# ChainBreak/denoising_diffusion_deep_fake

Measured on AMD Instinct MI355X. Metric: training images/sec (256x256 U-Net, bs=16/GPU), higher is better.
Workload: dtype f32; 1 GPU; d3f train_denoiser step: noise blend -> Unet(resnet34) fwd -> (MSE+1-SSIM)/2 -> bwd -> Adam, 256x256 synthetic face crops, bs=16/GPU, random-init weights, train-mode BatchNorm; image_size=256, batch_per_gpu=16, global_batch=16, parallelism=dp1, graph_step=False, adam_overlap_tail=False, adam_overlap_tail_steps=0, ranks_seen=1, csrc_digest=56899a78a27ce7a0

## Files before the change

denoising_diffusion_deep_fake_amd/_lib.py:

```python
import ctypes as C
import os
import re
from pathlib import Path

_HERE = Path(__file__).resolve().parent
LIB_PATH = Path(os.environ["D3F_LIB"]) if os.environ.get("D3F_LIB") else _HERE / "csrc" / "libd3f_hip.so"
HEADER_PATH = _HERE.parent / "include" / "d3f_hip.h"

F32, BF16, F32X3 = 0, 1, 2


class D3FError(RuntimeError):
    pass


class ConvDesc(C.Structure):
    _fields_ = [(n, C.c_int32) for n in
                ("B", "H", "W", "C0", "C1", "upsample0", "Cout", "KH", "KW", "stride", "pad", "CinReal")]


class BnDesc(C.Structure):
    _fields_ = [("dtype", C.c_int32), ("C", C.c_int32), ("Cpad", C.c_int32), ("rows", C.c_int64),
                ("apply", C.c_int32), ("relu", C.c_int32), ("res", C.c_int32), ("mask", C.c_int32),
                ("fwd_rows", C.c_int32), ("fused_rows", C.c_int32), ("allow_fused", C.c_int32), ("plan_nets", C.c_int32)]


class BnPlan(C.Structure):
    _fields_ = [("fwd_fused", C.c_int32), ("bwd_fused", C.c_int32), ("reduce_blocks", C.c_int32), ("bwd_rows", C.c_int32),
                ("rows_per_block", C.c_int64), ("stat_floats", C.c_uint64), ("part_floats", C.c_uint64)]


BN_COEF_ROWS = 7

_p, _i, _i64, _f, _sz, _dbl = C.c_void_p, C.c_int, C.c_int64, C.c_float, C.c_size_t, C.c_double
_u64, _u32p = C.c_uint64, C.POINTER(C.c_uint32)
_desc = C.POINTER(ConvDesc)
_bnd, _bnp = C.POINTER(BnDesc), C.POINTER(BnPlan)

PROTOTYPES = {
    "d3f_version": (_i, []),
    "d3f_last_error": (C.c_char_p, []),
    "d3f_source_digest": (C.c_char_p, []),
    "d3f_profile_enable": (_i, [_i]),
    "d3f_profile_classes": (_i, [_i]),
    "d3f_profile_collect": (_i, [C.POINTER(C.c_double), C.POINTER(C.c_int64), C.POINTER(C.c_double)]),
    "d3f_unet_create": (_i, [C.c_char_p, _i, _i, _i, _i, _i, _i, C.POINTER(_p)]),
    "d3f_unet_destroy": (_i, [_p]),
    "d3f_unet_create_nets": (_i, [C.c_char_p, _i, _i, _i, _i, _i, _i, _i, _i, C.POINTER(_p)]),
    "d3f_unet_nets": (_i, [_p]),
    "d3f_unet_net_workspace_stride": (_sz, [_p]),
    "d3f_unet_pair_pack_weights": (_i, [_p, C.POINTER(_p), _p, _p]),
    "d3f_unet_pair_forward": (_i, [_p, C.POINTER(_p), C.POINTER(_p), C.POINTER(_p), C.POINTER(_p), _p, _p]),
    "d3f_unet_pair_backward": (_i, [_p, C.POINTER(_p), C.POINTER(_p), C.POINTER(_p), _p, _i, _i, _i, _p]),
    "d3f_unet_num_params": (_i, [_p]),
    "d3f_unet_param_info": (_i, [_p, _i, C.c_char_p, _i, C.POINTER(C.c_int32), C.POINTER(_i), C.POINTER(_i64)]),
    "d3f_unet_param_floats": (_i64, [_p]),
    "d3f_unet_num_bn": (_i, [_p]),
    "d3f_unet_bn_info": (_i, [_p, _i, C.c_char_p, _i, C.POINTER(_i), C.POINTER(_i64), C.POINTER(_i64)]),
    "d3f_unet_bnstat_floats": (_i64, [_p]),
    "d3f_unet_workspace_bytes": (_sz, [_p]),
    "d3f_unet_forward_flops": (_dbl, [_p]),
    "d3f_unet_backward_flops": (_dbl, [_p]),
    "d3f_unet_pack_weights": (_i, [_p, _p, _p, _p]),
    "d3f_unet_forward": (_i, [_p, _p, _p, _p, _p, _p, _i, _p]),
    "d3f_unet_forward_graph": (_i, [_p, _p, _p, _p, _p, _p, _p]),
    "d3f_noise_blend_fixed": (_i, [_p, _p, _p, _p, _i, _i64, _p]),
    "d3f_l1_per_image_workspace_bytes": (_sz, [_i]),
    "d3f_l1_per_image": (_i, [_p, _p, _p, _p, _i, _i64, _p]),
    "d3f_affine_warp": (_i, [_p, _p, _p, _i, _i, _i, _i, _p]),
    "d3f_u8rgb_normalise": (_i, [_p, _p, _i, _i, _i, C.POINTER(_f), C.POINTER(_f), _p]),
    "d3f_unet_predict_u8": (_i, [_p, _p, _p, _p, _p, C.POINTER(_f), C.POINTER(_f), _p, _i, _p]),
    "d3f_unet_predict_frames_u8": (_i, [_p, _p, _p, _p, _i, _i, _i, _i, _i, _i, _p, C.POINTER(_f), C.POINTER(_f), _p, _i, _p]),
    "d3f_crop_resize_cubic_u8": (_i, [_p, _i, _i, _i, _i, _i, _i, _i, _p, _i, _i, _i64, _p]),
    "d3f_unet_num_segments": (_i, [_p]),
    "d3f_unet_plan_counts": (_i, [_p, C.POINTER(C.c_int32), C.POINTER(C.c_int32), C.POINTER(C.c_int32)]),
    "d3f_unet_segment_range": (_i, [_p, _i, C.POINTER(_i64), C.POINTER(_i64)]),
    "d3f_unet_backward": (_i, [_p, _p, _p, _p, _p, _i, _i, _p]),
    "d3f_unet_backward_nojoin": (_i, [_p, _p, _p, _p, _p, _i, _i, _p]),
    "d3f_unet_side_stream": (_i, [_p, C.POINTER(_p)]),
    "d3f_unet_backward_join": (_i, [_p, _p]),
    "d3f_adam_coefficients": (_i, [_f, _f, _f, _f, _i, _f, C.POINTER(_f)]),
    "d3f_unet_train_step": (_i, [_p, _p, _f, _f, _f, _p, _i, _p]),
    "d3f_unet_set_bn_sync": (_i, [_p, _p, _p, _i]),
    "d3f_unet_export": (_i, [_p, C.c_char_p, _p, _p, _p]),
    "d3f_unet_export_shape": (_i, [_p, C.c_char_p, C.POINTER(C.c_int32)]),
    "d3f_conv_upsample_folded": (_i, [_i, _p]),
    "d3f_conv_upsample_summed": (_i, [_i, _p]),
    "d3f_conv_packed_bytes": (_sz, [_i, _desc, _i]),
    "d3f_conv_pack_weights": (_i, [_i, _desc, _p, _p, _p, _p]),
    "d3f_conv_workspace_bytes": (_sz, [_i, _desc, _i]),
    "d3f_conv_stats_floats": (_sz, [_i, _desc, _i, C.POINTER(_i)]),
    "d3f_conv_forward": (_i, [_i, _desc, _p, _p, _p, _p, _p, _p, _p]),
    "d3f_conv_winograd_applies": (_i, [_i, _desc]),
    "d3f_conv_winograd_filter_bytes": (_sz, [_desc]),
    "d3f_conv_winograd_stats_floats": (_sz, [_desc, C.POINTER(_i)]),
    "d3f_conv_winograd_pack": (_i, [_desc, _p, _p, _p]),
    "d3f_conv_winograd_forward": (_i, [_desc, _p, _p, _p, _p, _p, _p, _p, _i, _p]),
    "d3f_conv_backward_data": (_i, [_i, _desc, _p, _p, _p, _p, _i, _i, _p, _p]),
    "d3f_conv_backward_weight_workspace_bytes": (_sz, [_i, _desc]),
    "d3f_conv_backward_weight": (_i, [_i, _desc, _p, _p, _p, _p, _p, _p]),
    "d3f_bn_finalize": (_i, [_p, _i, _i, _i64, _p, _p, _p, _p, _p, _p]),
    "d3f_bn_apply": (_i, [_i, _p, _p, _i, _i64, _p, _i, _p, _p]),
    "d3f_bn_backward_workspace_bytes": (_sz, [_i, _i, _i64]),
    "d3f_bn_backward": (_i, [_i, _p, _p, _p, _p, _p, _i, _i64, _p, _p, _p, _p, _p, _p]),
    "d3f_bn_layer_plan": (_i, [_bnd, _bnp]),
    "d3f_bn_layer_forward": (_i, [_bnd, _p, _p, _p, _p, _p, _p, _p, _p, _p, _p, _p]),
    "d3f_bn_layer_backward": (_i, [_bnd, _p, _p, _p, _p, _p, _p, _p, _p, _i, _p, _p, _p]),
    "d3f_unet_bn_layer": (_i, [_p, _i, _bnd, _bnp]),
    "d3f_maxpool3x3s2_forward": (_i, [_i, _p, _p, _p, _i, _i, _i, _i, _p]),
    "d3f_maxpool3x3s2_backward": (_i, [_i, _p, _p, _p, _i, _i, _i, _i, _i, _p]),
    "d3f_upsample2x_backward": (_i, [_i, _p, _p, _i, _i, _i, _i, _p]),
    "d3f_nchw_to_nhwc": (_i, [_i, _p, _p, _i, _i, _i, _i, _i, _p]),
    "d3f_nhwc_to_nchw": (_i, [_i, _p, _p, _i, _i, _i, _i, _i, _p]),
    "d3f_noise_blend": (_i, [_p, _p, _p, _f, _p, _p, _i, _i64, _p]),
    "d3f_mse_ssim_loss_workspace_bytes": (_sz, [_i, _i, _i]),
    "d3f_mse_ssim_loss": (_i, [_p, _p, _f, _f, _p, _p, _p, _i, _i, _i, _p]),
    "d3f_adam_step": (_i, [_p, _p, _p, _p, _i64, _f, _f, _f, _f, _i, _f, _p]),
    "d3f_ema_lerp": (_i, [_p, _p, _i64, _f, _p]),
    "d3f_philox4x32_10": (_i, [_u32p, _u32p, _u32p]),
    "d3f_noise_blend_rng": (_i, [_p, _u64, _u64, _f, _p, _p, _i, _i64, _p]),
    "d3f_noise_blend_fixed_rng": (_i, [_p, _u64, _u64, _p, _p, _i, _i64, _p]),
    "d3f_noise_draw": (_i, [_u64, _u64, _p, _p, _i, _i64, _p]),
    "d3f_affine_warp_rng": (_i, [_p, _p, _u64, _u64, _i, C.POINTER(_f), _i, _i, _i, _i, _p]),
    "d3f_affine_theta_draw": (_i, [_u64, _u64, _i, C.POINTER(_f), _p, _p, _i, _i, _i, _p]),
}

ALLREDUCE_FN = C.CFUNCTYPE(C.c_int, C.c_void_p, C.c_void_p, C.c_int64, C.c_void_p)

_lib = None


def header_symbols():
    text = HEADER_PATH.read_text()
    text = re.sub(r"/\*.*?\*/", "", text, flags=re.S)
    return sorted(set(re.findall(r"\b(d3f_[a-z0-9_]+)\s*\(", text)))


def sources_present():
    return HEADER_PATH.exists() and any((_HERE / "csrc").glob("*.hip"))


def source_digest():
    import hashlib
    h = hashlib.sha256()
    files = sorted((_HERE / "csrc").glob("*.hip")) + sorted((_HERE / "csrc").glob("*.h")) + [HEADER_PATH]
    for f in files:
        h.update(f.name.encode())
        h.update(f.read_bytes())
    return h.hexdigest()[:16]


def lib():
    global _lib
    if _lib is not None:
        return _lib
    if not LIB_PATH.exists():
        raise D3FError(
            f"{LIB_PATH} is missing: build it with `python -c 'import __graft_entry__ as g; g.build()'` "
            f"or `make -C {LIB_PATH.parent}` (hipcc, gfx950). There is no CPU fallback.")
    handle = C.CDLL(str(LIB_PATH))
    for name, (res, args) in PROTOTYPES.items():
        if os.environ.get("D3F_LIB") and not hasattr(handle, name):
            continue
        fn = getattr(handle, name)
        fn.restype = res
        fn.argtypes = args
    if not os.environ.get("D3F_LIB") and sources_present():
        built, here = handle.d3f_source_digest().decode(), source_digest()
        if built != here:
            raise D3FError(
                f"{LIB_PATH} was built from other sources (digest {built}) than the ones next to it ({here}): "
                f"rebuild it with `make -C {LIB_PATH.parent}`, or name a variant build explicitly through D3F_LIB")
    _lib = handle
    return _lib


def built_digest():
    handle = lib()
    return handle.d3f_source_digest().decode() if hasattr(handle, "d3f_source_digest") else None


def check(rc):
    if rc != 0:
        raise D3FError(lib().d3f_last_error().decode("utf-8", "replace"))


def stream_ptr():
    import torch
    return C.c_void_p(torch.cuda.current_stream().cuda_stream)


def ptr(t):
    if t is None:
        return None
    return C.c_void_p(t.data_ptr())


def ptr2(a, b):
    return (C.c_void_p * 2)(a.data_ptr(), b.data_ptr())
```

denoising_diffusion_deep_fake_amd/csrc/batchnorm.hip:

```cpp
#include "common.h"
#include "pointwise.h"
#include "vec16.h"

#include <algorithm>
#include <type_traits>

namespace d3f {

constexpr float BN_EPS = 1e-5f, BN_MOMENTUM = 0.1f;

constexpr int BNF_SC = 32;
constexpr int BNF_MAX_ROWS = 1024;
#ifndef BNF_FWD_U_F32
#define BNF_FWD_U_F32 4
#endif
#ifndef BNF_BWD_U
#define BNF_BWD_U 2
#endif

__device__ __forceinline__ float2 bn_fwd_coef(double s1, double s2, double count, int c, const float* __restrict__ gamma,
                                              const float* __restrict__ beta, float eps, float momentum, bool store,
                                              float* __restrict__ running_mean, float* __restrict__ running_var,
                                              float* __restrict__ mean_o, float* __restrict__ invstd_o,
                                              float* __restrict__ scale_o, float* __restrict__ shift_o) {
// ... 317 lines not shown
    const float4 v0 = *reinterpret_cast<const float4*>(base + (long)r * ld * 2);
    const float4 v1 = *reinterpret_cast<const float4*>(base + (long)(r + 16) * ld * 2);
    const float4 v2 = *reinterpret_cast<const float4*>(base + (long)(r + 32) * ld * 2);
    const float4 v3 = *reinterpret_cast<const float4*>(base + (long)(r + 48) * ld * 2);
    if (!hooked) { behind_first_loads(); hooked = true; }
    a0 += (double)v0.x; a1 += (double)v0.y; a2 += (double)v0.z; a3 += (double)v0.w;
    a0 += (double)v1.x; a1 += (double)v1.y; a2 += (double)v1.z; a3 += (double)v1.w;
    a0 += (double)v2.x; a1 += (double)v2.y; a2 += (double)v2.z; a3 += (double)v2.w;
    a0 += (double)v3.x; a1 += (double)v3.y; a2 += (double)v3.z; a3 += (double)v3.w;
  }
  if (!hooked) behind_first_loads();
  for (; r < rows; r += 16) {
    const float4 v = *reinterpret_cast<const float4*>(base + (long)r * ld * 2);
    a0 += (double)v.x; a1 += (double)v.y; a2 += (double)v.z; a3 += (double)v.w;
  }
  red[rl][q * 4 + 0] = a0;
  red[rl][q * 4 + 1] = a1;
  red[rl][q * 4 + 2] = a2;
  red[rl][q * 4 + 3] = a3;
  __syncthreads();
  if (tid < 64) {
    double s = 0.0;
#pragma unroll
    for (int k = 0; k < 16; ++k) s += red[k][tid];
    tot[tid] = s;
  }
  __syncthreads();
}

template <typename T, bool HAS2>
__global__ __launch_bounds__(256) void bn_finalize_apply_kernel(
    const float* __restrict__ stats, int stat_rows, int C, int Cpad, double count,
    const float* __restrict__ gamma, const float* __restrict__ beta, float eps, float momentum,
    float* __restrict__ running_mean, float* __restrict__ running_var, float* __restrict__ mean_o,
    float* __restrict__ invstd_o, float* __restrict__ scale_o, float* __restrict__ shift_o,
    const T* __restrict__ y, const T* __restrict__ res, const T* __restrict__ yr,
    const float* __restrict__ scale_r, const float* __restrict__ shift_r, int relu, T* __restrict__ out,
    long rows, long rows_per_block, NetSplit ns) {
  chain_priority();
  if (blockIdx.z != 0) {
    net_shift(stats, ns.ws); net_shift(gamma, ns.par); net_shift(beta, ns.par);
    net_shift(running_mean, ns.bn); net_shift(running_var, ns.bn);
    net_shift(mean_o, ns.ws); net_shift(invstd_o, ns.ws); net_shift(scale_o, ns.ws); net_shift(shift_o, ns.ws);
    net_shift(y, ns.ws); net_shift(res, ns.ws); net_shift(yr, ns.ws); net_shift(scale_r, ns.ws); net_shift(shift_r, ns.ws);
    net_shift(out, ns.ws);
  }
  __shared__ double red[16][64];
  __shared__ double tot[64];
  __shared__ float cf[2][BNF_SC];
  typedef typename Raw4<T>::type raw_t;
  constexpr int U = sizeof(T) == 4 ? BNF_FWD_U_F32 : 8;
  const int tid = threadIdx.x, c0 = blockIdx.y * BNF_SC;
  const int v = tid & 7, rr = tid >> 3, cc = c0 + v * 4;
  const long r0 = (long)blockIdx.x * rows_per_block;
  long r1 = r0 + rows_per_block;
  if (r1 > rows) r1 = rows;
  const T* __restrict__ second = res != nullptr ? res : yr;
  raw_t a[U], b[U], an[U], bn[U];
  auto load = [&](raw_t (&ya)[U], raw_t (&yb)[U], long r) {
#pragma unroll
    for (int u = 0; u < U; ++u) {
      const long row = r + 32 * u < r1 ? r + 32 * u : r1 - 1;
      ya[u] = ldraw(y + row * C + cc);
      if (HAS2) yb[u] = ldraw(second + row * C + cc);
    }
  };
  slab_reduce(stats, stat_rows, Cpad, c0, red, tot, [&]() { load(a, b, r0 + rr); });
  if (tid < BNF_SC) {
    const float2 f = bn_fwd_coef(tot[2 * tid], tot[2 * tid + 1], count, c0 + tid, gamma, beta, eps, momentum,
                                 blockIdx.x == 0, running_mean, running_var, mean_o, invstd_o, scale_o, shift_o);
    cf[0][tid] = f.x;
    cf[1][tid] = f.y;
  }
  __syncthreads();
  float sc[4], sf[4], scr[4] = {0.f, 0.f, 0.f, 0.f}, sfr[4] = {0.f, 0.f, 0.f, 0.f};
#pragma unroll
  for (int k = 0; k < 4; ++k) {
    sc[k] = cf[0][v * 4 + k];
    sf[k] = cf[1][v * 4 + k];
    if (HAS2 && res == nullptr) {
      scr[k] = scale_r[cc + k];
      sfr[k] = shift_r[cc + k];
    }
  }
  for (long r = r0 + rr; r < r1; r += 32 * U) {
    if (r + 32 * U < r1) load(an, bn, r + 32 * U);
#pragma unroll
    for (int u = 0; u < U; ++u) {
      const long row = r + 32 * u;
      if (row >= r1) continue;
      const float4 ya = cvt4(a[u]);
      float x[4] = {ya.x, ya.y, ya.z, ya.w};
#pragma unroll
      for (int k = 0; k < 4; ++k) x[k] = x[k] * sc[k] + sf[k];
      if (HAS2) {
        const float4 yb = cvt4(b[u]);
        if (res != nullptr) {
          x[0] += yb.x; x[1] += yb.y; x[2] += yb.z; x[3] += yb.w;
        } else {
          const float t[4] = {yb.x, yb.y, yb.z, yb.w};
#pragma unroll
          for (int k = 0; k < 4; ++k) x[k] += t[k] * scr[k] + sfr[k];
        }
      }
      if (relu) {
#pragma unroll
        for (int k = 0; k < 4; ++k) x[k] = fmaxf(x[k], 0.f);
      }
      st4<T>(out + row * C + cc, make_float4(x[0], x[1], x[2], x[3]));
    }
#pragma unroll
    for (int u = 0; u < U; ++u) {
      a[u] = an[u];
      if (HAS2) b[u] = bn[u];
    }
  }
}

static long rows_per_block_for(long rows, int slabs, int dtype, int plan_nets) {
  const long wgs = (dtype == D3F_F32 ? 256 : 512) / plan_nets_for(plan_nets, 64);
  long rb = std::max(1L, wgs / slabs);
  long rpb = (rows + rb - 1) / rb;
  rpb = (rpb + 31) / 32 * 32;
  return std::max(32L, rpb);
}

struct BnResidualOps {
  const void *res = nullptr, *yr = nullptr;
  const float *scale_r = nullptr, *shift_r = nullptr;
};
static BnResidualOps residual_ops(const BnLayer& L, const BnBufs& b) {
  if (L.res == BN_RES_TENSOR) return {b.res, nullptr, nullptr, nullptr};
  if (L.res == BN_RES_LAYER) return {nullptr, b.res, bn_coef(b.res_coef, L.C, BN_SCALE), bn_coef(b.res_coef, L.C, BN_SHIFT)};
  return {};
}

static int bn_finalize_apply_launch(const BnLayer& L, const BnBufs& b, hipStream_t stream, const NetSplit* ns) {
  if (L.rows == 0) return 0;
  const NetSplit nv = net_split_or_single(ns);
  const dim3 grid((unsigned)((L.rows + L.rows_per_block - 1) / L.rows_per_block), (unsigned)(L.C / BNF_SC),
                  (unsigned)nv.nets);
  const BnResidualOps r = residual_ops(L, b);
  by_dtype(L.dtype, [&](auto* typed) {
    typedef std::remove_pointer_t<decltype(typed)> T;
    auto go = [&](auto kernel) {
      hipLaunchKernelGGL(kernel, grid, dim3(256), 0, stream, b.stats, L.fwd_rows, L.C, L.Cpad, (double)L.rows, b.gamma,
                         b.beta, BN_EPS, BN_MOMENTUM, b.running_mean, b.running_var, bn_coef(b.coef, L.C, BN_MEAN),
                         bn_coef(b.coef, L.C, BN_INVSTD), bn_coef(b.coef, L.C, BN_SCALE), bn_coef(b.coef, L.C, BN_SHIFT),
                         (const T*)b.y, (const T*)r.res, (const T*)r.yr, r.scale_r, r.shift_r, L.relu ? 1 : 0, (T*)b.a,
                         L.rows, L.rows_per_block, nv);
    };
    if (L.res != BN_RES_NONE) go(bn_finalize_apply_kernel<T, true>);
    else go(bn_finalize_apply_kernel<T, false>);
  });
  D3F_HIP(hipGetLastError());
  return 0;
}

template <typename T, bool FROM_A, bool RD_DRES>
__global__ __launch_bounds__(256) void bn_bwd_finalize_apply_kernel(
    const float* __restrict__ partial, int nblocks, int C, double count, const float* __restrict__ gamma,
    const float* __restrict__ mean, const float* __restrict__ invstd, float* __restrict__ dgamma,
    float* __restrict__ dbeta, float* __restrict__ coef, const T* __restrict__ dA,
    const T* __restrict__ a, const T* __restrict__ y, T* __restrict__ dy, T* __restrict__ dres,
    long rows, long rows_per_block, const float* __restrict__ mask_scale,
    const float* __restrict__ mask_shift, NetSplit ns) {
  chain_priority();
  if (blockIdx.z != 0) {
    net_shift(partial, ns.ws); net_shift(gamma, ns.par); net_shift(mean, ns.ws); net_shift(invstd, ns.ws);
    net_shift(dgamma, ns.grad); net_shift(dbeta, ns.grad); net_shift(coef, ns.ws);
    net_shift(dA, ns.ws); net_shift(a, ns.ws); net_shift(y, ns.ws); net_shift(dy, ns.ws); net_shift(dres, ns.ws);
    net_shift(mask_scale, ns.ws); net_shift(mask_shift, ns.ws);
  }
  __shared__ double red[16][64];
  __shared__ double tot[64];
  __shared__ float cf[3][BNF_SC];
  typedef typename Raw4<T>::type raw_t;
  constexpr int U = BNF_BWD_U;
  const int tid = threadIdx.x, c0 = blockIdx.y * BNF_SC;
  const int v = tid & 7, rr = tid >> 3, cc = c0 + v * 4;
  const long r0 = (long)blockIdx.x * rows_per_block;
  long r1 = r0 + rows_per_block;
  if (r1 > rows) r1 = rows;
  raw_t g4[U], y4[U], a4[U], d4[U], g4n[U], y4n[U], a4n[U], d4n[U];
  auto load = [&](raw_t (&gg)[U], raw_t (&yy)[U], raw_t (&aa)[U], raw_t (&dd)[U], long r) {
#pragma unroll
    for (int u = 0; u < U; ++u) {
      const long row = r + 32 * u < r1 ? r + 32 * u : r1 - 1;
      gg[u] = ldraw(dA + row * C + cc);
      yy[u] = ldraw(y + row * C + cc);
      if (FROM_A) aa[u] = ldraw(a + row * C + cc);
      if (RD_DRES) dd[u] = ldraw(dres + row * C + cc);
    }
  };
  slab_reduce(partial, nblocks, C, c0, red, tot, [&]() { load(g4, y4, a4, d4, r0 + rr); });
  if (tid < BNF_SC) {
    const float3 k = bn_bwd_coef(tot[2 * tid], tot[2 * tid + 1], count, c0 + tid, C, gamma, invstd, blockIdx.x == 0,
                                 dgamma, dbeta, coef);
    cf[0][tid] = k.x;
    cf[1][tid] = k.y;
    cf[2][tid] = k.z;
  }
  __syncthreads();
  float k0[4], k1[4], k2[4], mu[4], is[4], msc[4] = {0.f, 0.f, 0.f, 0.f}, msf[4] = {0.f, 0.f, 0.f, 0.f};
#pragma unroll
  for (int k = 0; k < 4; ++k) {
    k0[k] = cf[0][v * 4 + k];
    k1[k] = cf[1][v * 4 + k];
    k2[k] = cf[2][v * 4 + k];
    mu[k] = mean[cc + k];
    is[k] = invstd[cc + k];
    if (!FROM_A && mask_scale != nullptr) {
      msc[k] = mask_scale[cc + k];
      msf[k] = mask_shift[cc + k];
    }
  }
  for (long r = r0 + rr; r < r1; r += 32 * U) {
    if (r + 32 * U < r1) load(g4n, y4n, a4n, d4n, r + 32 * U);
#pragma unroll
    for (int u = 0; u < U; ++u) {
      const long row = r + 32 * u;
      if (row >= r1) continue;
      const float4 gv = cvt4(g4[u]), yv = cvt4(y4[u]);
      float g[4] = {gv.x, gv.y, gv.z, gv.w};
      const float yy[4] = {yv.x, yv.y, yv.z, yv.w};
      if (FROM_A) {
        const float4 av = cvt4(a4[u]);
        const float aa[4] = {av.x, av.y, av.z, av.w};
#pragma unroll
        for (int k = 0; k < 4; ++k) g[k] = aa[k] > 0.f ? g[k] : 0.f;
      } else if (mask_scale != nullptr) {
#pragma unroll
        for (int k = 0; k < 4; ++k) g[k] = (yy[k] * msc[k] + msf[k]) > 0.f ? g[k] : 0.f;
      }
      float o[4];
#pragma unroll
      for (int k = 0; k < 4; ++k) {
        const float xhat = (yy[k] - mu[k]) * is[k];
        o[k] = k0[k] * (g[k] - k1[k] - xhat * k2[k]);
      }
      st4<T>(dy + row * C + cc, make_float4(o[0], o[1], o[2], o[3]));
      if (dres != nullptr) {
        if (RD_DRES) {
          const float4 dv = cvt4(d4[u]);
          g[0] += dv.x; g[1] += dv.y; g[2] += dv.z; g[3] += dv.w;
        }
        st4<T>(dres + row * C + cc, make_float4(g[0], g[1], g[2], g[3]));
      }
    }
#pragma unroll
    for (int u = 0; u < U; ++u) {
      g4[u] = g4n[u];
      y4[u] = y4n[u];
      if (FROM_A) a4[u] = a4n[u];
      if (RD_DRES) d4[u] = d4n[u];
    }
  }
}

struct BnBwdOps {
  const float *mean, *invstd;
  float* k;
  const void* a;
  const float *mask_scale, *mask_shift;
};
static BnBwdOps bwd_ops(const BnLayer& L, const BnBufs& b) {
  const bool from_y = L.mask == BN_MASK_FROM_Y;
  return {bn_coef(b.coef, L.C, BN_MEAN), bn_coef(b.coef, L.C, BN_INVSTD), b.k != nullptr ? b.k : bn_coef(b.coef, L.C, BN_K),
          L.mask == BN_MASK_FROM_A ? b.a : nullptr, from_y ? bn_coef(b.coef, L.C, BN_SCALE) : nullptr,
          from_y ? bn_coef(b.coef, L.C, BN_SHIFT) : nullptr};
}

static int bn_bwd_finalize_apply_launch(const BnLayer& L, const BnBufs& b, const BnBwdOps& o, hipStream_t stream,
                                        const NetSplit* ns) {
  if (L.rows == 0) return 0;
  const NetSplit nv = net_split_or_single(ns);
  const dim3 grid((unsigned)((L.rows + L.rows_per_block - 1) / L.rows_per_block), (unsigned)(L.C / BNF_SC),
                  (unsigned)nv.nets);
  const bool from_a = o.mask_scale == nullptr && o.a != nullptr;
  const bool rd_dres = b.dres != nullptr && b.dres_acc;
  by_dtype(L.dtype, [&](auto* typed) {
    typedef std::remove_pointer_t<decltype(typed)> T;
    auto go = [&](auto kernel) {
      hipLaunchKernelGGL(kernel, grid, dim3(256), 0, stream, b.stats, L.bwd_rows, L.C, (double)L.rows, b.gamma, o.mean,
                         o.invstd, b.dgamma, b.dbeta, o.k, (const T*)b.dA, (const T*)o.a, (const T*)b.y, (T*)b.dy,
                         (T*)b.dres, L.rows, L.rows_per_block, o.mask_scale, o.mask_shift, nv);
    };
    if (from_a && rd_dres) go(bn_bwd_finalize_apply_kernel<T, true, true>);
    else if (from_a) go(bn_bwd_finalize_apply_kernel<T, true, false>);
    else if (rd_dres) go(bn_bwd_finalize_apply_kernel<T, false, true>);
    else go(bn_bwd_finalize_apply_kernel<T, false, false>);
  });
  D3F_HIP(hipGetLastError());
  return 0;
}

void bn_layer_plan(BnLayer& L) {
  static const bool no_fused = getenv("D3F_NO_BN_FUSED_FINALIZE") != nullptr;
  auto fused_ok = [&](int rows) {
    return L.allow_fused && !no_fused && (L.dtype == D3F_F32 || L.dtype == D3F_BF16) && L.C % BNF_SC == 0 && rows >= 1 &&
           rows <= BNF_MAX_ROWS;
  };
  const long min_rows = std::max(16L, 4L * (256 / std::max(1, std::min(256, L.C / (L.dtype == D3F_F32 ? 4 : 8)))));
  L.reduce_blocks = (int)std::clamp((L.rows + min_rows - 1) / min_rows, 1L, 1024L);
  L.bwd_rows = L.fused_rows > 0 ? L.fused_rows : L.reduce_blocks;
  L.fwd_fused = L.apply && fused_ok(L.fwd_rows);
  L.bwd_fused = fused_ok(L.bwd_rows);
  L.rows_per_block = L.fwd_fused || L.bwd_fused ? rows_per_block_for(L.rows, L.C / BNF_SC, L.dtype, L.plan_nets) : 0;
  L.stat_floats = (size_t)L.fwd_rows * L.Cpad * 2;
  L.part_floats = (size_t)std::max(L.reduce_blocks, L.fused_rows) * L.C * 2;
}

int bn_layer_finalize(const BnLayer& L, const BnBufs& b, long count, hipStream_t stream, const NetSplit* ns) {
  const NetSplit nv = net_split_or_single(ns);
  hipLaunchKernelGGL(bn_finalize_kernel, dim3(L.C, 1, nv.nets), dim3(256), 0, stream, b.stats, L.fwd_rows, L.C, L.Cpad,
                     (double)count, b.gamma, b.beta, BN_EPS, BN_MOMENTUM, b.running_mean, b.running_var,
                     bn_coef(b.coef, L.C, BN_MEAN), bn_coef(b.coef, L.C, BN_INVSTD), bn_coef(b.coef, L.C, BN_SCALE),
                     bn_coef(b.coef, L.C, BN_SHIFT), nv);
  D3F_HIP(hipGetLastError());
  return 0;
}

int bn_layer_apply(const BnLayer& L, const BnBufs& b, hipStream_t stream, const NetSplit* ns) {
  const int ve = L.dtype == D3F_F32 ? 4 : 8;
  D3F_CHECK(L.C % ve == 0 && (256 * ve) % L.C == 0, "bn_apply: C=%d must divide %d", L.C, 256 * ve);
  const long nvec = L.rows * L.C / ve;
  if (nvec == 0) return 0;
  const NetSplit nv = net_split_or_single(ns);
  const BnResidualOps r = residual_ops(L, b);
  by_dtype(L.dtype, [&](auto* typed) {
    typedef std::remove_pointer_t<decltype(typed)> T;
    hipLaunchKernelGGL(bn_apply_kernel<T>, dim3(grid_for(nvec), 1, nv.nets), dim3(256), 0, stream, (const T*)b.y,
                       bn_coef(b.coef, L.C, BN_SCALE), bn_coef(b.coef, L.C, BN_SHIFT), (const T*)r.res, (const T*)r.yr,
                       r.scale_r, r.shift_r, L.relu ? 1 : 0, (T*)b.a, nvec, L.C, nv.ws);
  });
  D3F_HIP(hipGetLastError());
  return 0;
}

int bn_layer_forward(const BnLayer& L, const BnBufs& b, const BnSync* sync, hipStream_t stream, const NetSplit* ns) {
  long count = L.rows;
  if (sync != nullptr) {
    if (int rc = sync->fn(sync->ctx, b.stats, (int64_t)L.fwd_rows * L.Cpad * 2, (void*)stream))
      return set_error(rc, "BatchNorm statistics all-reduce failed in the forward pass (%s)", L.name.c_str());
    count *= sync->world;
  } else if (L.fwd_fused) {
    return bn_finalize_apply_launch(L, b, stream, ns);
  }
  if (int rc = bn_layer_finalize(L, b, count, stream, ns)) return rc;
  return L.apply ? bn_layer_apply(L, b, stream, ns) : 0;
}

int bn_layer_backward(const BnLayer& L, const BnBufs& b, const BnSync* sync, hipStream_t stream, const NetSplit* ns) {
  const int C = L.C, ve = L.dtype == D3F_F32 ? 4 : 8, vc = C / ve;
  const NetSplit nv = net_split_or_single(ns);
  const BnBwdOps o = bwd_ops(L, b);
  if (L.fused_rows == 0) {
    D3F_CHECK(C % ve == 0 && vc >= 1 && vc <= 256 && (256 % vc) == 0, "bn_bwd_reduce: unsupported channel count %d", C);
    by_dtype(L.dtype, [&](auto* typed) {
      typedef std::remove_pointer_t<decltype(typed)> T;
      hipLaunchKernelGGL(bn_bwd_reduce_kernel<T>, dim3(L.reduce_blocks, 1, nv.nets), dim3(256), 0, stream,
                         (const T*)b.dA, (const T*)o.a, (const T*)b.y, o.mean, o.invstd, b.stats, L.rows, C, o.mask_scale,
                         o.mask_shift, nv.ws);
    });
    D3F_HIP(hipGetLastError());
  }
  auto finalize = [&](long count, float* dgamma, float* dbeta) -> int {
    hipLaunchKernelGGL(bn_bwd_finalize_kernel, dim3(C, 1, nv.nets), dim3(256), 0, stream, b.stats, L.bwd_rows, C,
                       (double)count, b.gamma, o.invstd, dgamma, dbeta, o.k, nv);
    D3F_HIP(hipGetLastError());
    return 0;
  };
  if (sync != nullptr) {
    if (int rc = finalize(L.rows, b.dgamma, b.dbeta)) return rc;
    if (int rc = sync->fn(sync->ctx, b.stats, (int64_t)L.bwd_rows * C * 2, (void*)stream))
      return set_error(rc, "BatchNorm statistics all-reduce failed in the backward pass (%s)", L.name.c_str());
    if (int rc = finalize(L.rows * sync->world, nullptr, nullptr)) return rc;
  } else if (L.bwd_fused) {
    return bn_bwd_finalize_apply_launch(L, b, o, stream, ns);
  } else if (int rc = finalize(L.rows, b.dgamma, b.dbeta)) {
    return rc;
  }
  D3F_CHECK(C % ve == 0 && (256 * ve) % C == 0, "bn_bwd_apply: C=%d must divide %d", C, 256 * ve);
  const long nvec = L.rows * C / ve;
  if (nvec == 0) return 0;
  by_dtype(L.dtype, [&](auto* typed) {
    typedef std::remove_pointer_t<decltype(typed)> T;
    hipLaunchKernelGGL(bn_bwd_apply_kernel<T>, dim3(grid_for(nvec), 1, nv.nets), dim3(256), 0, stream, (const T*)b.dA,
                       (const T*)o.a, (const T*)b.y, o.mean, o.invstd, o.k, (T*)b.dy, (T*)b.dres, b.dres_acc, nvec, C,
                       o.mask_scale, o.mask_shift, nv.ws);
  });
  D3F_HIP(hipGetLastError());
  return 0;
}

}
```

denoising_diffusion_deep_fake_amd/csrc/c_api.hip:

```cpp
#include "../../include/d3f_hip.h"

#include <cstdarg>
#include <cstdio>
#include <cstring>
#include <new>
#include <vector>

#include "engine.h"
#include "philox.h"

namespace d3f {
static thread_local char g_err[1024] = "";
int set_error(int code, const char* fmt, ...) {
  va_list ap;
  va_start(ap, fmt);
  vsnprintf(g_err, sizeof(g_err), fmt, ap);
  va_end(ap);
  return code;
}
}

namespace d3f {
struct ProfRec {
  hipEvent_t a, b;
// ... 368 lines not shown
  if (int rc = plan(L, D3F_F32, d, PLAN_FWD)) return rc;
  D3F_CHECK(L.wu != 0,
            "conv_winograd: needs 3x3 / stride 1 / pad 1, one source, H and W multiples of 16, channels a multiple of 16, "
            "filters a multiple of 64 (got %dx%d k%d s%d p%d C0=%d C1=%d up=%d Cout=%d)",
            d->H, d->W, d->KH, d->stride, d->pad, d->C0, d->C1, d->upsample0, d->Cout);
  return 0;
}
int d3f_conv_winograd_applies(int dtype, const d3f_conv_desc* d) {
  ConvLayer L;
  return (d != nullptr && plan(L, dtype, d, PLAN_FWD) == 0 && L.wino) ? 1 : 0;
}
size_t d3f_conv_winograd_filter_bytes(const d3f_conv_desc* d) {
  ConvLayer L;
  return (d == nullptr || plan(L, D3F_F32, d, PLAN_FWD) != 0) ? 0 : L.wu;
}
size_t d3f_conv_winograd_stats_floats(const d3f_conv_desc* d, int* tiles) {
  ConvLayer L;
  if (d == nullptr || plan(L, D3F_F32, d, PLAN_FWD) != 0 || L.wu == 0) return 0;
  if (tiles) *tiles = L.wino_rows;
  return (size_t)L.wino_rows * L.CoutPad * 2;
}
int d3f_conv_winograd_pack(const d3f_conv_desc* d, const float* w, void* u, void* stream) {
  ConvLayer L;
  if (int rc = wino_plan(L, d)) return rc;
  D3F_CHECK(w && u && d->CinReal == d->C0, "conv_winograd_pack: null argument or padded input channels");
  return conv_winograd_pack_launch(w, reinterpret_cast<float*>(u), d->Cout, d->C0, (hipStream_t)stream);
}
int d3f_conv_winograd_forward(const d3f_conv_desc* d, const void* src0, const void* u, void* y, float* stats,
                              const float* scale, const float* shift, const void* residual, int relu, void* stream) {
  ConvLayer L;
  if (int rc = wino_plan(L, d)) return rc;
  if (d->B == 0) return 0;
  D3F_CHECK(src0 && u && y && ((scale == nullptr) == (shift == nullptr)), "conv_winograd_forward: null argument");
  D3F_CHECK(scale != nullptr || (residual == nullptr && relu == 0),
            "conv_winograd_forward: residual / ReLU belong to the eval epilogue (scale and shift)");
  ConvFwdBufs b;
  b.src0 = src0; b.w = u; b.out = y;
  if (scale != nullptr) {
    b.scale = scale; b.shift = shift; b.res = residual; b.relu = relu ? 1 : 0;
  } else {
    b.stats = stats;
  }
  return conv_layer_forward(L, b, true, (hipStream_t)stream);
}
int d3f_conv_backward_data(int dtype, const d3f_conv_desc* d, const void* dy, const void* w_dgrad,
                           void* dx0, void* dx1, int acc0, int acc1, void* workspace, void* stream) {
  ConvLayer L;
  const int sum2 = d != nullptr && d->upsample0 == 2 ? PLAN_SUM2 : 0;
  if (int rc = plan(L, dtype, d, PLAN_DGRAD | sum2 | (workspace ? PLAN_SPLITK : 0))) return rc;
  if (d->B == 0) return 0;
  D3F_CHECK(dy && w_dgrad && dx0 && (d->C1 == 0 || dx1), "conv_backward_data: null argument");
  ConvDgradBufs b;
  b.dy = dy; b.w = w_dgrad; b.dx0 = dx0; b.dx1 = dx1; b.acc0 = acc0; b.acc1 = acc1;
  b.w_skip = L.upfold ? reinterpret_cast<const char*>(w_dgrad) + L.wd4 : nullptr;
  b.slabs = reinterpret_cast<float*>(workspace);
  return conv_layer_dgrad(L, b, (hipStream_t)stream);
}
size_t d3f_conv_backward_weight_workspace_bytes(int dtype, const d3f_conv_desc* d) {
  ConvLayer L;
  return plan(L, dtype, d, PLAN_WGRAD) != 0 ? 0 : L.wslab_bytes;
}
int d3f_conv_backward_weight(int dtype, const d3f_conv_desc* d, const void* dy, const void* src0,
                             const void* src1, void* workspace, float* dw, void* stream) {
  ConvLayer L;
  if (int rc = plan(L, dtype, d, PLAN_WGRAD)) return rc;
  if (d->B == 0) {
    D3F_CHECK(dw, "conv_backward_weight: null argument");
    D3F_HIP(hipMemsetAsync(dw, 0, (size_t)d->Cout * d->CinReal * d->KH * d->KW * sizeof(float), (hipStream_t)stream));
    return 0;
  }
  D3F_CHECK(dy && src0 && workspace && dw && (d->C1 == 0 || src1), "conv_backward_weight: null argument");
  return wgrad_layer_launch(L.wl, dy, src0, src1, reinterpret_cast<float*>(workspace), dw, d->Cout, d->CinReal, dtype,
                            (hipStream_t)stream);
}

static BnLayer bn_layer(int dtype, int C, int64_t rows, int fwd_rows = 0) {
  BnLayer L;
  L.C = C; L.Cpad = (int)round_up(C, 16); L.rows = (long)rows; L.dtype = sdt(dtype); L.fwd_rows = fwd_rows;
  L.allow_fused = false;
  bn_layer_plan(L);
  return L;
}
int d3f_bn_finalize(const float* stats, int tiles, int C, int64_t count, const float* gamma,
                    const float* beta, float* running_mean, float* running_var, float* coef, void* stream) {
  D3F_CHECK(stats && gamma && beta && coef && C > 0 && tiles > 0 && count > 0, "bn_finalize: argument");
  const BnLayer L = bn_layer(D3F_F32, C, count, tiles);
  BnBufs b;
  b.stats = const_cast<float*>(stats);
  b.gamma = gamma; b.beta = beta; b.running_mean = running_mean; b.running_var = running_var; b.coef = coef;
  return bn_layer_finalize(L, b, (long)count, (hipStream_t)stream);
}
int d3f_bn_apply(int dtype, const void* y, const float* coef, int C, int64_t rows, const void* residual,
                 int relu, void* out, void* stream) {
  D3F_CHECK(y && coef && out, "bn_apply: null argument");
  BnLayer L = bn_layer(dtype, C, rows);
  L.relu = relu != 0;
  L.res = residual ? BN_RES_TENSOR : BN_RES_NONE;
  BnBufs b;
  b.coef = const_cast<float*>(coef);
  b.y = y; b.res = residual; b.a = out;
  return bn_layer_apply(L, b, (hipStream_t)stream);
}
size_t d3f_bn_backward_workspace_bytes(int dtype, int C, int64_t rows) {
  return ((size_t)bn_layer(dtype, C, rows).reduce_blocks * C * 2 + 3 * (size_t)C) * sizeof(float) + 256;
}
int d3f_bn_backward(int dtype, const void* dA, const void* a_or_null, const void* y, const float* coef,
                    const float* gamma, int C, int64_t rows, void* dy, void* dres, float* dgamma,
                    float* dbeta, void* workspace, void* stream) {
  D3F_CHECK(dA && y && coef && gamma && dy && dgamma && dbeta && workspace, "bn_backward: null argument");
  BnLayer L = bn_layer(dtype, C, rows);
  L.mask = a_or_null ? BN_MASK_FROM_A : BN_MASK_NONE;
  BnBufs b;
  b.stats = reinterpret_cast<float*>(workspace);
  b.k = b.stats + (size_t)round_up((long)L.reduce_blocks * C * 2, 4);
  b.coef = const_cast<float*>(coef);
  b.gamma = gamma; b.y = y; b.a = const_cast<void*>(a_or_null);
  b.dA = dA; b.dy = dy; b.dres = dres; b.dgamma = dgamma; b.dbeta = dbeta;
  return bn_layer_backward(L, b, nullptr, (hipStream_t)stream);
}

static_assert(D3F_BN_COEF_ROWS == BN_COEF_ROWS, "d3f_hip.h states the coefficient block's rows");
static int bn_plan(BnLayer& L, const d3f_bn_desc* d) {
  D3F_CHECK(d != nullptr, "bn_layer: null descriptor");
  D3F_CHECK(d->dtype == D3F_F32 || d->dtype == D3F_BF16 || d->dtype == D3F_F32X3, "bn_layer: dtype %d", d->dtype);
  D3F_CHECK(d->C > 0 && d->Cpad >= d->C && d->rows >= 0, "bn_layer: C=%d Cpad=%d rows=%lld", d->C, d->Cpad,
            (long long)d->rows);
  D3F_CHECK(d->res >= BN_RES_NONE && d->res <= BN_RES_LAYER && d->mask >= BN_MASK_NONE && d->mask <= BN_MASK_FROM_A,
            "bn_layer: res=%d mask=%d", d->res, d->mask);
  D3F_CHECK(d->fwd_rows >= 0 && d->fused_rows >= 0, "bn_layer: fwd_rows=%d fused_rows=%d", d->fwd_rows, d->fused_rows);
  D3F_CHECK(d->plan_nets == 1 || d->plan_nets == 2, "bn_layer: plan_nets=%d", d->plan_nets);
  L.name = "bn_layer";
  L.C = d->C; L.Cpad = d->Cpad; L.rows = (long)d->rows; L.dtype = sdt(d->dtype); L.plan_nets = d->plan_nets;
  L.apply = d->apply != 0; L.relu = d->relu != 0;
  L.res = (BnResidual)d->res; L.mask = (BnMask)d->mask;
  L.fwd_rows = d->fwd_rows; L.fused_rows = d->fused_rows; L.allow_fused = d->allow_fused != 0;
  bn_layer_plan(L);
  return 0;
}
static void bn_plan_out(const BnLayer& L, d3f_bn_plan* p) {
  p->fwd_fused = L.fwd_fused; p->bwd_fused = L.bwd_fused; p->reduce_blocks = L.reduce_blocks; p->bwd_rows = L.bwd_rows;
  p->rows_per_block = L.rows_per_block; p->stat_floats = L.stat_floats; p->part_floats = L.part_floats;
}
static bool bn_split_channels_ok(const BnLayer& L) {
  const int ve = L.dtype == D3F_F32 ? 4 : 8;
  return L.C % ve == 0 && (256 * ve) % L.C == 0;
}
int d3f_bn_layer_plan(const d3f_bn_desc* d, d3f_bn_plan* plan) {
  D3F_CHECK(plan != nullptr, "bn_layer_plan: null argument");
  BnLayer L;
  if (int rc = bn_plan(L, d)) return rc;
  bn_plan_out(L, plan);
  return 0;
}
int d3f_bn_layer_forward(const d3f_bn_desc* d, float* stats, const float* gamma, const float* beta, float* running_mean,
                         float* running_var, float* coef, const void* y, const void* res, const float* res_coef, void* a,
                         void* stream) {
  BnLayer L;
  if (int rc = bn_plan(L, d)) return rc;
  if (L.rows == 0) return 0;
  D3F_CHECK(L.fwd_rows >= 1, "bn_layer_forward: the forward pass reads fwd_rows >= 1 partial rows (fwd_rows=%d)", L.fwd_rows);
  D3F_CHECK(stats && gamma && beta && coef && y, "bn_layer_forward: null argument");
  D3F_CHECK((running_mean == nullptr) == (running_var == nullptr), "bn_layer_forward: one running statistic without the other");
  if (L.apply) {
    D3F_CHECK(a != nullptr, "bn_layer_forward: apply needs the output tensor");
    D3F_CHECK(L.res == BN_RES_NONE || res != nullptr, "bn_layer_forward: res=%d needs the residual tensor", (int)L.res);
    D3F_CHECK(L.res != BN_RES_LAYER || res_coef != nullptr, "bn_layer_forward: res=2 needs res_coef, the other layer's coefficient block");
  }
  if (L.fwd_fused)
    D3F_CHECK(L.Cpad % 2 == 0, "bn_layer_forward: the fused form needs an even Cpad (Cpad=%d)", L.Cpad);
  else if (L.apply)
    D3F_CHECK(bn_split_channels_ok(L), "bn_layer_forward: the split form needs C to divide %d (C=%d)",
              256 * (L.dtype == D3F_F32 ? 4 : 8), L.C);
  BnBufs b;
  b.stats = stats; b.gamma = gamma; b.beta = beta; b.running_mean = running_mean; b.running_var = running_var;
  b.coef = coef; b.y = y; b.a = a; b.res = res; b.res_coef = res_coef;
  return bn_layer_forward(L, b, nullptr, (hipStream_t)stream);
}
int d3f_bn_layer_backward(const d3f_bn_desc* d, float* partial, const float* gamma, float* coef, const void* y,
                          const void* a, const void* dA, void* dy, void* dres, int dres_acc, float* dgamma, float* dbeta,
                          void* stream) {
  BnLayer L;
  if (int rc = bn_plan(L, d)) return rc;
  if (L.rows == 0) return 0;
  D3F_CHECK(partial != nullptr, "bn_layer_backward: null partial rows (fused_rows=%d: %s)", L.fused_rows,
            L.fused_rows > 0 ? "the caller's sums" : "scratch of part_floats floats");
  D3F_CHECK(gamma && coef && y && dA && dy, "bn_layer_backward: null argument");
  D3F_CHECK(L.mask != BN_MASK_FROM_A || a != nullptr, "bn_layer_backward: mask=2 needs the activation a");
  D3F_CHECK((dgamma == nullptr) == (dbeta == nullptr), "bn_layer_backward: dgamma without dbeta or the reverse");
  if (L.fused_rows == 0 || !L.bwd_fused)
    D3F_CHECK(bn_split_channels_ok(L), "bn_layer_backward: the split kernels need C to divide %d (C=%d)",
              256 * (L.dtype == D3F_F32 ? 4 : 8), L.C);
  BnBufs b;
  b.stats = partial; b.gamma = gamma; b.coef = coef; b.y = y;
  b.a = const_cast<void*>(a);
  b.dA = dA; b.dy = dy; b.dres = dres; b.dres_acc = dres != nullptr && dres_acc ? 1 : 0;
  b.dgamma = dgamma; b.dbeta = dbeta;
  return bn_layer_backward(L, b, nullptr, (hipStream_t)stream);
}
int d3f_unet_bn_layer(d3f_unet_t h, int i, d3f_bn_desc* d, d3f_bn_plan* plan) {
  D3F_CHECK(h && d && plan && i >= 0 && i < (int)h->e.bns.size(), "bn_layer: index %d", i);
  int k = -1;
  for (const Unit& u : h->e.units) {
    if (!u.bn || ++k != i) continue;
    const BnLayer& L = u.norm;
    d->dtype = L.dtype; d->C = L.C; d->Cpad = L.Cpad; d->rows = L.rows; d->apply = L.apply; d->relu = L.relu;
    d->res = L.res; d->mask = L.mask; d->fwd_rows = L.fwd_rows; d->fused_rows = L.fused_rows;
    d->allow_fused = L.allow_fused; d->plan_nets = L.plan_nets;
    bn_plan_out(L, plan);
    return 0;
  }
  return set_error(-1, "bn_layer: index %d", i);
}

int d3f_maxpool3x3s2_forward(int dtype, const void* in, void* out, uint8_t* idx, int B, int H, int W,
                             int C, void* stream) {
  D3F_CHECK(in && out && idx, "maxpool: null argument");
  return maxpool3x3s2_fwd_launch(sdt(dtype), in, out, idx, B, H, W, C, (hipStream_t)stream);
}
int d3f_maxpool3x3s2_backward(int dtype, const void* dout, const uint8_t* idx, void* din, int accumulate,
                              int B, int H, int W, int C, void* stream) {
  D3F_CHECK(dout && idx && din, "maxpool: null argument");
  return maxpool3x3s2_bwd_launch(sdt(dtype), dout, idx, din, accumulate, B, H, W, C, (hipStream_t)stream);
}
int d3f_upsample2x_backward(int dtype, const void* dfull, void* dlow, int B, int Hlow, int Wlow, int C,
                            void* stream) {
  D3F_CHECK(dfull && dlow, "upsample2x_backward: null argument");
  return sum2x2_launch(sdt(dtype), dfull, dlow, B, Hlow, Wlow, C, (hipStream_t)stream);
}
int d3f_u8rgb_normalise(const uint8_t* in_hwc, float* out_nchw, int B, int H, int W, const float mean[3],
                        const float std[3], void* stream) {
  if (B == 0) return 0;
  D3F_CHECK(in_hwc && out_nchw && mean && std, "u8rgb_normalise: null argument");
  D3F_CHECK(B > 0 && H > 0 && W > 0, "u8rgb_normalise: bad shape");
  D3F_CHECK(std[0] != 0.f && std[1] != 0.f && std[2] != 0.f, "u8rgb_normalise: zero std");
  return u8rgb_to_nchw_launch(in_hwc, out_nchw, B, (long)H * W, mean, std, (hipStream_t)stream);
}

int d3f_crop_resize_cubic_u8(const uint8_t* src, int B, int src_h, int src_w, int x1, int y1, int cw, int ch, uint8_t* dst,
                             int H, int W, int64_t dst_row_stride_bytes, void* stream) {
  D3F_CHECK(src && dst, "crop_resize_cubic_u8: null argument");
  return crop_resize_cubic_u8_launch(src, B, src_h, src_w, x1, y1, cw, ch, dst, H, W, (long)dst_row_stride_bytes,
                                     (hipStream_t)stream);
}

int d3f_affine_warp(const float* in, const float* theta, float* out, int B, int C, int H, int W, void* stream) {
  if (B == 0) return 0;
  D3F_CHECK(in && theta && out && in != out, "affine_warp: null or aliased argument");
  D3F_CHECK(B >= 0 && C > 0 && H > 0 && W > 0, "affine_warp: bad shape");
  return affine_warp_launch(in, theta, out, B, C, H, W, (hipStream_t)stream);
}

int d3f_affine_warp_rng(const float* in, float* out, uint64_t seed, uint64_t offset, int kind, const float params[5],
                        int B, int C, int H, int W, void* stream) {
  if (B == 0) return 0;
  D3F_CHECK(in && out && params && in != out, "affine_warp_rng: null or aliased argument");
  D3F_CHECK(B >= 0 && C > 0 && H > 0 && W > 0, "affine_warp_rng: bad shape");
  AffineRngParams q;
  if (int rc = affine_rng_params(kind, params, H, W, q)) return rc;
  return affine_warp_rng_launch(in, out, seed, offset, q, B, C, H, W, (hipStream_t)stream);
}
int d3f_affine_theta_draw(uint64_t seed, uint64_t offset, int kind, const float params[5], float* theta, uint8_t* apply,
                          int B, int H, int W, void* stream) {
  if (B == 0) return 0;
  D3F_CHECK(params && theta && apply, "affine_theta_draw: null argument");
  D3F_CHECK(B >= 0, "affine_theta_draw: bad shape");
  AffineRngParams q;
  if (int rc = affine_rng_params(kind, params, H, W, q)) return rc;
  return affine_theta_draw_launch(seed, offset, q, theta, apply, B, (hipStream_t)stream);
}

int d3f_nchw_to_nhwc(int dtype, const float* in, void* out, int B, int C, int H, int W, int Cpad, void* stream) {
  D3F_CHECK(in && out && Cpad >= C, "nchw_to_nhwc: argument");
  return nchw_to_nhwc_launch(sdt(dtype), in, out, B, C, H, W, Cpad, (hipStream_t)stream);
}
int d3f_nhwc_to_nchw(int dtype, const void* in, float* out, int B, int C, int H, int W, int Cpad, void* stream) {
  D3F_CHECK(in && out && Cpad >= C, "nhwc_to_nchw: argument");
  return nhwc_to_nchw_launch(sdt(dtype), in, out, B, C, H, W, Cpad, (hipStream_t)stream);
}

int d3f_noise_blend(const float* x, const float* noise, const float* y_uniform, float lam, float* out,
                    float* r_out_or_null, int B, int64_t per_image, void* stream) {
  if (B == 0 || per_image == 0) return 0;
  D3F_CHECK(x && noise && y_uniform && out, "noise_blend: null argument");
  return noise_blend_launch(x, noise, y_uniform, lam, out, r_out_or_null, B, (long)per_image,
                            (hipStream_t)stream);
}
int d3f_noise_blend_fixed(const float* x, const float* noise, const float* r, float* out, int B, int64_t per_image,
                          void* stream) {
  if (B == 0 || per_image == 0) return 0;
  D3F_CHECK(x && noise && r && out, "noise_blend_fixed: null argument");
  return noise_blend_fixed_launch(x, noise, r, out, B, (long)per_image, (hipStream_t)stream);
}
int d3f_philox4x32_10(const uint32_t counter[4], const uint32_t key[2], uint32_t out[4]) {
  D3F_CHECK(counter && key && out, "philox4x32_10: null argument");
  const Philox4 p = philox4x32_10(counter[0], counter[1], counter[2], counter[3], key[0], key[1]);
  for (int i = 0; i < 4; ++i) out[i] = p.x[i];
  return 0;
}
int d3f_noise_blend_rng(const float* x, uint64_t seed, uint64_t offset, float lam, float* out, float* r_out_or_null,
                        int B, int64_t per_image, void* stream) {
  if (B == 0 || per_image == 0) return 0;
  D3F_CHECK(x && out && x != out, "noise_blend_rng: null or aliased argument");
  D3F_CHECK(B > 0 && per_image > 0, "noise_blend_rng: bad shape");
  return noise_blend_rng_launch(x, seed, offset, lam, out, r_out_or_null, B, (long)per_image, (hipStream_t)stream);
}
int d3f_noise_blend_fixed_rng(const float* x, uint64_t seed, uint64_t offset, const float* r, float* out, int B,
                              int64_t per_image, void* stream) {
  if (B == 0 || per_image == 0) return 0;
  D3F_CHECK(x && r && out && x != out, "noise_blend_fixed_rng: null or aliased argument");
  D3F_CHECK(B > 0 && per_image > 0, "noise_blend_fixed_rng: bad shape");
  return noise_blend_fixed_rng_launch(x, seed, offset, r, out, B, (long)per_image, (hipStream_t)stream);
}
int d3f_noise_draw(uint64_t seed, uint64_t offset, float* noise_or_null, float* y_or_null, int B, int64_t per_image,
                   void* stream) {
  if (B == 0) return 0;
  D3F_CHECK(B > 0 && per_image >= 0, "noise_draw: bad shape");
  return noise_draw_launch(seed, offset, noise_or_null, y_or_null, B, (long)per_image, (hipStream_t)stream);
}
size_t d3f_l1_per_image_workspace_bytes(int B) { return l1_per_image_workspace_bytes(B); }
int d3f_l1_per_image(const float* prediction, const float* target, float* out, void* workspace, int B,
                     int64_t per_image, void* stream) {
  if (B == 0) return 0;
  D3F_CHECK(prediction && target && out && workspace, "l1_per_image: null argument");
  return l1_per_image_launch(prediction, target, out, workspace, B, (long)per_image, (hipStream_t)stream);
}
size_t d3f_mse_ssim_loss_workspace_bytes(int B, int H, int W) {
  return loss_workspace_floats(B, H, W) * sizeof(float);
}
int d3f_mse_ssim_loss(const float* pred, const float* target, float input_min, float input_max,
// ... 18 lines not shown
```

denoising_diffusion_deep_fake_amd/csrc/engine.h:

```cpp
#pragma once
#include <string>
#include <vector>

#include "common.h"
#include "pointwise.h"

namespace d3f {

struct TensorD {
  size_t off = 0;
  int H = 0, W = 0, C = 0;
  long elems(int B) const { return (long)B * H * W * C; }
};

struct ParamInfo {
  std::string name;
  int shape[4];
  int ndim;
  long offset;
  long numel;
};

struct BnInfo {
  std::string prefix;
  int C;
  long rm_off, rv_off;
};

struct Unit : ConvLayer {
  std::string conv_name;
  int in0 = -1, in1 = -1, y = -1, a = -1;
  bool bn = true, bias = false;
  BnLayer norm;
  int res_tensor = -1, res_unit = -1;
  long w_off = -1, bias_off = -1, g_off = -1, b_off = -1, rm_off = -1, rv_off = -1;
  size_t wf_off = 0, wd_off = 0;
  size_t coef_off = 0;
  int segment = 0;
  size_t dy_off = 0;
  size_t wfc_off = 0, wd4_off = 0, wds_off = 0;
  size_t wu_off = 0;
  size_t wslab_off = 0;
};

enum BwdKind { BW_HEAD, BW_UNIT, BW_SUM2X2, BW_POOL };
struct BwdOp {
  BwdKind kind;
  int unit = -1;
  int dA = -1;
  int fuse_for_unit = -1;
  int fused_rows = 0;
  bool mask = true;
  int dres = -1;
  bool dres_acc = false;
  int dst0 = -1, dst1 = -1;
  bool acc0 = false, acc1 = false;
  bool dst0_is_full_scratch = false;
  int C = 0, Hl = 0, Wl = 0;
  int segment = 0;
};

struct NetIO {
  long params = 0, bnstats = 0, grads = 0, x = 0, out = 0, dout = 0;
};

class UnetEngine {
 public:
  ~UnetEngine();
  int build(const char* encoder, int in_channels, int classes, int B, int H, int W, int dtype, int nets = 1,
            int plan_nets = 1);

  int pack_weights(const float* params, void* ws, hipStream_t s, const NetIO* io = nullptr) const;
  int forward(const float* params, float* bnstats, const float* x, float* out, void* ws, int training,
              hipStream_t s, const NetIO* io = nullptr) const;
  int backward(const float* params, const float* dout, float* grads, void* ws, int seg_begin,
               int seg_end, hipStream_t s, int join = 1, const NetIO* io = nullptr) const;
  int backward_join(hipStream_t s) const;
  hipStream_t side_stream() const;
  int predict_u8(const float* params, float* bnstats, const uint8_t* bgr_in, uint8_t* bgr_out,
                 const float mean[3], const float stdv[3], void* ws, int use_graph, hipStream_t s) const;
  int predict_frames_u8(const float* params, float* bnstats, const uint8_t* raw_in, int src_h, int src_w, int x1, int y1,
                        int cw, int ch, uint8_t* pair_out, const float mean[3], const float stdv[3], void* ws,
                        int use_graph, hipStream_t s) const;
  int forward_graph(const float* params, float* bnstats, const float* x, float* out, void* ws, hipStream_t s) const;
  struct StepArgs {
    float* params; float* bnstats; float* grads; float* exp_avg; float* exp_avg_sq;
    const float* image; const float* noise; const float* y_uniform;
    float* noisy; float* pred; float* gpred; float* loss_out; float* loss_ws;
    const float* adam_coef;
    float lam, lo, hi;
  };
  int train_step(const StepArgs& a, void* ws, int use_graph, hipStream_t s) const;
  typedef int (*AllReduceFn)(void* ctx, float* data, int64_t count, void* stream);
  bool bn_sync_installed() const { return bn_sync_.fn != nullptr; }
  void set_bn_sync(AllReduceFn fn, void* ctx, int world) { bn_sync_ = BnSync{fn, ctx, world > 0 ? world : 1}; }
  int export_tensor(const char* name, const void* ws, float* out_nchw, hipStream_t s) const;
  int export_shape(const char* name, int32_t dims[3]) const;

  std::vector<ParamInfo> params;
  std::vector<BnInfo> bns;
  long param_floats = 0, bnstat_floats = 0;
  size_t workspace_bytes = 0;
  int num_segments = 4;
  long seg_grad_begin[8] = {0}, seg_grad_end[8] = {0};
  int B = 0, H = 0, W = 0, dtype = 0, in_channels = 3, classes = 3;
  int nets = 1, plan_nets = 1;
  size_t net_ws_stride = 0;
  int cdtype = 0;
  double fwd_flops = 0, bwd_flops = 0;
  std::vector<Unit> units;

 private:
  int esize() const { return dtype == D3F_F32 ? 4 : 2; }
  int wsize() const { return cdtype == D3F_F32X3 ? 6 : esize(); }
  int ve() const { return dtype == D3F_F32 ? 4 : 8; }
  const TensorD* find_export(const char* name) const;
  int new_tensor(int H_, int W_, int C_);
  int new_grad(int tensor_id);
  size_t alloc(size_t bytes);
  int add_unit(const std::string& conv_name, const std::string& bn_name, int in0, int in1, int up0,
               int Cout, int k, int stride, int pad, bool bn, bool bias, bool relu, bool apply,
               int segment);

  std::vector<TensorD> tensors;
  std::vector<TensorD> gtensors;
  std::vector<int> grad_of;
  std::vector<bool> grad_init;
  std::vector<BwdOp> bwd_ops;
  std::vector<int> fwd_order_;
  mutable hipStream_t side_ = nullptr;
  mutable std::vector<hipEvent_t> ev_dy_;
  mutable hipEvent_t ev_join_ = nullptr;
  mutable hipEvent_t ev_seg_ = nullptr;
  mutable bool side_dirty_ = false;
  int ensure_streams() const;
  mutable hipEvent_t ev_pack_in_ = nullptr, ev_pack_done_ = nullptr, ev_pack_mid_ = nullptr;
  mutable bool pack_pending_ = false, pack_mid_pending_ = false;
  int first_mid_unit_ = -1;
  int first_late_unit_ = -1;
  int forward_body(const float* params, float* bnstats, float* out, char* ws, int training, hipStream_t s,
                   const NetSplit* ns = nullptr) const;
  bool make_split(const NetIO* io, long in_delta, NetSplit* ns) const;
  int predict_u8_launches(const float* params, float* bnstats, const uint8_t* bgr_in, uint8_t* bgr_out,
                          const float mean255[3], const float std255[3], char* ws, hipStream_t s) const;
  int predict_frames_u8_launches(const float* params, float* bnstats, const uint8_t* raw_in, const int geo[6],
                                 uint8_t* pair_out, const float mean255[3], const float std255[3], char* ws,
                                 hipStream_t s) const;
  struct GraphKey {
    const void* ptr[5];
    float cst[6];
    int geo[6];
  };
  struct GraphSlot {
    hipGraphExec_t exec = nullptr;
    GraphKey key = {};
  };
  template <typename F>
  int graph_replay(GraphSlot& slot, const GraphKey& key, hipStream_t s, F&& launches) const;
  int wait_for_packed_weights(hipStream_t s) const;
  mutable hipStream_t gstream_ = nullptr;
  mutable GraphSlot g_predict_, g_eval_, g_frames_;
  BnSync bn_sync_{nullptr, nullptr, 1};
  const BnSync* bn_sync() const { return bn_sync_.fn != nullptr ? &bn_sync_ : nullptr; }
  int train_step_launches(const StepArgs& a, void* ws, hipStream_t s) const;
  mutable hipGraphExec_t g_step_ = nullptr;
  mutable StepArgs g_step_key_{};
  mutable const void* g_step_ws_ = nullptr;
  mutable hipEvent_t ev_gin_ = nullptr, ev_gout_ = nullptr;
  size_t head_nchw_off = 0;
  size_t ws_top = 0;
  int t_x = -1, t_pool = -1, head = -1, conv1 = -1;
  size_t pool_idx_off = 0, stats_off = 0, bnpart_off = 0, dz_off = 0, dfull_off = 0,
         bsum_off = 0, splitk_off = 0;
  size_t stats_bytes = 0, bnpart_bytes = 0, dy_bytes = 0, dz_bytes = 0, dfull_bytes = 0, splitk_bytes = 0;
};

int channel_sum_nchw_launch(const float* x, int B, int C, long HW, float* partial, float* out,
                            hipStream_t stream, const NetSplit* ns = nullptr);

}
```

denoising_diffusion_deep_fake_amd/csrc/engine.hip:

```cpp
#include "engine.h"
#include <vector>

#include <cstdio>
#include <cstdlib>
#include <cstring>

namespace d3f {

constexpr int CS_PP = 16;
__global__ __launch_bounds__(256) void channel_sum_partial_kernel(const float* __restrict__ x, int C, long HW,
                                                                  float* __restrict__ partial, int nb, long net_in,
                                                                  long net_ws) {
  __shared__ float red[256];
  const int seg = blockIdx.x, c = blockIdx.y, b = (int)blockIdx.z % nb;
  if ((int)blockIdx.z >= nb) {
    net_shift(x, net_in); net_shift(partial, net_ws);
  }
  const float* __restrict__ plane = x + ((long)b * C + c) * HW;
  const long per = (HW + CS_PP - 1) / CS_PP, lo = (long)seg * per, hi = lo + per < HW ? lo + per : HW;
  float s = 0.f;
  if ((HW & 3) == 0 && (per & 3) == 0) {
    for (long i = lo + 4 * threadIdx.x; i < hi; i += 4 * 256) {
      const float4 v = *reinterpret_cast<const float4*>(plane + i);
      s += (v.x + v.y) + (v.z + v.w);
// ... 253 lines not shown
        if (u.in1 >= 0) op.dst1 = grad_dst(u.in1, &op.acc1);
      } else {
        op.dst0 = grad_dst(u.in0, &op.acc0);
      }
    }
    bwd_ops.push_back(op);
    if (u.need_dgrad && u.up0 && !u.upfold && !u.dgrad.sum2) {
      BwdOp s;
      s.kind = BW_SUM2X2; s.unit = ui; s.C = u.C0; s.Hl = u.Hv / 2; s.Wl = u.Wv / 2; s.segment = u.segment;
      bool acc;
      s.dst0 = grad_dst(u.in0, &acc);
      D3F_CHECK(!acc, "plan: up-sampled tensor has two consumers");
      bwd_ops.push_back(s);
    }
    return 0;
  };
  {
    BwdOp h;
    h.kind = BW_HEAD; h.unit = head; h.segment = 0;
    h.dst0 = grad_dst(units[head].in0, &h.acc0);
    bwd_ops.push_back(h);
  }
  for (int i = 4; i >= 0; --i) {
    const DBlk& d = dec_blocks[i];
    if (int rc = emit_unit(d.u2, grad_of[units[d.u2].a], true, -1, false)) return rc;
    if (int rc = emit_unit(d.u1, grad_of[units[d.u1].a], true, -1, false)) return rc;
  }
  for (int bi = (int)enc_blocks.size() - 1; bi >= 0; --bi) {
    const Blk& b = enc_blocks[bi];
    const Unit& u2 = units[b.u2];
    D3F_CHECK(grad_of[u2.a] >= 0, "plan: block output without gradient");
    int dres;
    bool dres_acc = false;
    if (b.ud >= 0) dres = -2;
    else dres = grad_dst(u2.res_tensor, &dres_acc);
    if (int rc = emit_unit(b.u2, grad_of[u2.a], true, dres, dres_acc)) return rc;
    if (int rc = emit_unit(b.u1, grad_of[units[b.u1].a], true, -1, false)) return rc;
    if (b.ud >= 0)
      if (int rc = emit_unit(b.ud, -2, false, -1, false)) return rc;
  }
  {
    BwdOp p;
    p.kind = BW_POOL; p.segment = 3;
    p.dA = grad_of[t_pool];
    D3F_CHECK(p.dA >= 0, "plan: pool output without gradient");
    p.dst0 = grad_dst(f1, &p.acc0);
    bwd_ops.push_back(p);
  }
  if (int rc = emit_unit(conv1, grad_of[f1], true, -1, false)) return rc;

  static const bool no_fused_reduce = getenv("D3F_NO_FUSED_BN_REDUCE") != nullptr;
  if (!no_fused_reduce) {
    auto writes = [&](const BwdOp& o, int gid) {
      if (o.kind == BW_UNIT || o.kind == BW_HEAD) {
        if (units[o.unit].need_dgrad && !o.dst0_is_full_scratch && o.dst0 == gid) return true;
        if (o.dst1 == gid) return true;
        if (o.kind == BW_UNIT && o.dres == gid) return true;
      }
      return (o.kind == BW_SUM2X2 || o.kind == BW_POOL) && o.dst0 == gid;
    };
    for (size_t j = 0; j + 1 < bwd_ops.size(); ++j) {
      BwdOp& pj = bwd_ops[j];
      if (!(pj.kind == BW_UNIT || pj.kind == BW_HEAD)) continue;
      const Unit& up = units[pj.unit];
      const ConvParams& pd = up.upfold ? up.dgrad_lo : up.dgrad;
      if (!up.need_dgrad || pd.par || pj.dst0_is_full_scratch || (pj.dst1 >= 0 && !up.upfold) || pj.dst0 < 0) continue;
      BwdOp& ck = bwd_ops[j + 1];
      if (ck.kind != BW_UNIT || ck.dA != pj.dst0) continue;
      bool last = true;
      for (size_t k = j + 1; k < bwd_ops.size(); ++k) last = last && !writes(bwd_ops[k], pj.dst0);
      const Unit& uc = units[ck.unit];
      if (!last || !(uc.bn && ck.mask)) continue;
      D3F_CHECK(pd.Cout == uc.Cout && pd.M == (pd.sum2 ? 4 : 1) * B * uc.Ho * uc.Wo && pd.out_c0 == pd.Cout,
                "plan: fused BatchNorm reduce shape mismatch (%s -> %s)", up.conv_name.c_str(), uc.conv_name.c_str());
      pj.fuse_for_unit = ck.unit;
      ck.fused_rows = pd.splitk > 1 ? pd.stat_rows : pd.tiles_m;
    }
  }

  for (const BwdOp& op : bwd_ops) {
    if (op.kind != BW_UNIT) continue;
    Unit& u = units[op.unit];
    u.norm.res = u.res_tensor >= 0 ? BN_RES_TENSOR : u.res_unit >= 0 ? BN_RES_LAYER : BN_RES_NONE;
    u.norm.mask = !op.mask ? BN_MASK_NONE : u.norm.res == BN_RES_NONE ? BN_MASK_FROM_Y : BN_MASK_FROM_A;
    u.norm.fused_rows = op.fused_rows;
  }
  for (Unit& u : units) {
    if (!u.bn) continue;
    bn_layer_plan(u.norm);
    stats_bytes = std::max(stats_bytes, u.norm.stat_floats * sizeof(float));
    bnpart_bytes = std::max(bnpart_bytes, u.norm.part_floats * sizeof(float));
  }

  stats_off = alloc(stats_bytes);
  bnpart_off = alloc(bnpart_bytes);
  dz_off = alloc(dz_bytes);
  dfull_off = alloc(dfull_bytes);
  bsum_off = alloc(channel_sum_partial_floats(B, classes) * sizeof(float));
  splitk_off = alloc(splitk_bytes);
  head_nchw_off = alloc((size_t)B * classes * H * W * sizeof(float));
  net_ws_stride = nets > 1 ? (size_t)round_up((long)ws_top, 4096) : 0;
  workspace_bytes = nets > 1 ? net_ws_stride * nets : ws_top;

  long layer3_start = -1, layer4_start = -1, dec_start = -1;
  for (const auto& p : params) {
    if (layer3_start < 0 && p.name.rfind("encoder.layer3.", 0) == 0) layer3_start = p.offset;
    if (layer4_start < 0 && p.name.rfind("encoder.layer4.", 0) == 0) layer4_start = p.offset;
    if (dec_start < 0 && p.name.rfind("decoder.", 0) == 0) dec_start = p.offset;
  }
  num_segments = 4;
  seg_grad_begin[0] = dec_start;     seg_grad_end[0] = param_floats;
  seg_grad_begin[1] = layer4_start;  seg_grad_end[1] = dec_start;
  seg_grad_begin[2] = layer3_start;  seg_grad_end[2] = layer4_start;
  seg_grad_begin[3] = 0;             seg_grad_end[3] = layer3_start;
  fwd_order_.clear();
  fwd_order_.push_back(conv1);
  fwd_order_.push_back(-1);
  for (const auto& b : enc_blocks) {
    fwd_order_.push_back(b.u1);
    if (b.ud >= 0) fwd_order_.push_back(b.ud);
    fwd_order_.push_back(b.u2);
  }
  for (const auto& d : dec_blocks) {
    fwd_order_.push_back(d.u1);
    fwd_order_.push_back(d.u2);
  }
  fwd_order_.push_back(head);
  return 0;
}

static int shared_side_stream(hipStream_t* out) {
  constexpr int MAXDEV = 64;
  static hipStream_t streams[MAXDEV] = {};
  int dev = 0;
  D3F_HIP(hipGetDevice(&dev));
  D3F_CHECK(dev >= 0 && dev < MAXDEV, "side stream: device index %d", dev);
  if (streams[dev] == nullptr) {
    int least = 0, greatest = 0;
    D3F_HIP(hipDeviceGetStreamPriorityRange(&least, &greatest));
    D3F_HIP(hipStreamCreateWithPriority(&streams[dev], hipStreamNonBlocking, least));
  }
  *out = streams[dev];
  return 0;
}

int UnetEngine::ensure_streams() const {
  if (side_ != nullptr) return 0;
  if (int rc = shared_side_stream(&side_)) return rc;
  D3F_HIP(hipEventCreateWithFlags(&ev_join_, hipEventDisableTiming));
  D3F_HIP(hipEventCreateWithFlags(&ev_seg_, hipEventDisableTiming));
  D3F_HIP(hipEventCreateWithFlags(&ev_pack_in_, hipEventDisableTiming));
  D3F_HIP(hipEventCreateWithFlags(&ev_pack_done_, hipEventDisableTiming));
  D3F_HIP(hipEventCreateWithFlags(&ev_pack_mid_, hipEventDisableTiming));
  return 0;
}

bool UnetEngine::make_split(const NetIO* io, long in_delta, NetSplit* ns) const {
  if (nets <= 1) return false;
  ns->nets = nets;
  ns->ws = (long)net_ws_stride;
  ns->par = io->params;
  ns->grad = io->grads;
  ns->bn = io->bnstats;
  ns->in = in_delta;
  ns->out = io->out;
  return true;
}

int UnetEngine::pack_weights(const float* params0_, void* ws0_, hipStream_t s, const NetIO* io) const {
  D3F_CHECK((int)units.size() <= PACK_MAX_LAYERS, "pack_weights: %d layers exceed the table", (int)units.size());
  D3F_CHECK(nets == 1 || io != nullptr, "pack_weights: a pair engine needs the second network's offsets");
  static const bool sync_pack = getenv("D3F_NO_ASYNC_PACK") != nullptr;
  const bool async = !sync_pack && first_late_unit_ > 0;
  const int mid = async ? first_mid_unit_ : -1;
  auto params_of = [&](int n) { return reinterpret_cast<const float*>(reinterpret_cast<const char*>(params0_) + (n ? io->params : 0)); };
  auto ws_of = [&](int n) { return reinterpret_cast<char*>(ws0_) + (size_t)n * net_ws_stride; };
  auto part_of = [&](int ui) { return ui >= first_late_unit_ ? 2 : (mid > 0 && ui >= mid) ? 1 : 0; };
  for (int part = 0; part < 3; ++part) {
    if (part == 1 && mid <= 0) continue;
    PackTable t;
    t.n = 0;
    uint32_t blocks = 0;
    for (int ui = 0; ui < (int)units.size(); ++ui) {
      const Unit& u = units[ui];
      if (first_late_unit_ > 0 && part_of(ui) != part) continue;
      if (first_late_unit_ <= 0 && part != 0) continue;
      if (u.upfold) continue;
      const int nb = conv_pack_entry(u, u.w_off, u.wf_off, u.wd_off, true, u.need_dgrad, blocks, t.e[t.n++]);
      if (nb < 0) return nb;
      blocks += (uint32_t)nb;
    }
    hipStream_t ps = s;
    if (part >= 1 && async) {
      if (int rc = ensure_streams()) return rc;
      if (part == 1 || mid <= 0) {
        D3F_HIP(hipEventRecord(ev_pack_in_, s));
        D3F_HIP(hipStreamWaitEvent(side_, ev_pack_in_, 0));
      }
      ps = side_;
    }
    for (int n = 0; n < nets; ++n) {
      const float* params_ = params_of(n);
      char* ws = ws_of(n);
      if (t.n > 0)
        if (int rc = pack_all_launch(cdtype, params_, ws, t, (int)blocks, ps)) return rc;
      for (int ui = 0; ui < (int)units.size(); ++ui) {
        const Unit& u = units[ui];
        if (!u.wino) continue;
        if (first_late_unit_ > 0 ? part_of(ui) != part : part != 0) continue;
        if (int rc = conv_winograd_pack_launch(params_ + u.w_off, reinterpret_cast<float*>(ws + u.wu_off), u.Cout, u.Cin, ps))
          return rc;
      }
    }
    if (part == 1 && async) {
      D3F_HIP(hipEventRecord(ev_pack_mid_, side_));
      pack_mid_pending_ = true;
    }
    if (part == 2 || (first_late_unit_ <= 0 && part == 0)) {
      for (int n = 0; n < nets; ++n) {
        const float* params_ = params_of(n);
        char* ws = ws_of(n);
        for (const Unit& u : units)
          if (u.upfold)
            if (int rc = pack_up_launch(cdtype, params_ + u.w_off, u.Cout, u.C0, u.C1, ws + u.wfc_off, u.CoutPad,
                                        u.need_dgrad ? ws + u.wd4_off : nullptr, u.C0Rows,
                                        (u.need_dgrad && u.C1 > 0) ? ws + u.wds_off : nullptr, u.C1Rows, ps))
              return rc;
      }
    }
    if (part == 2 && async) {
      D3F_HIP(hipEventRecord(ev_pack_done_, side_));
      pack_pending_ = true;
    }
  }
  return 0;
}

int UnetEngine::forward(const float* params_, float* bnstats, const float* x, float* out, void* ws_,
                        int training, hipStream_t s, const NetIO* io) const {
  char* ws = reinterpret_cast<char*>(ws_);
  D3F_CHECK(nets == 1 || (io != nullptr && training), "unet: the pair engine runs train-mode passes and needs the second "
            "network's offsets");
  NetSplit split{};
  const NetSplit* ns = make_split(io, io ? io->x : 0, &split) ? &split : nullptr;
  if (int rc = nchw_to_nhwc_launch(dtype, x, ws + tensors[t_x].off, B, in_channels, H, W, tensors[t_x].C, s, ns))
    return rc;
  return forward_body(params_, bnstats, out, ws, training, s, ns);
}

int UnetEngine::forward_body(const float* params_, float* bnstats, float* out, char* ws, int training,
                             hipStream_t s, const NetSplit* ns) const {
  auto T = [&](int tid) { return ws + tensors[tid].off; };
  auto coef = [&](const Unit& u) { return reinterpret_cast<float*>(ws + u.coef_off); };
  D3F_CHECK(ns == nullptr || (training && bn_sync() == nullptr), "unet: the pair engine runs train-mode passes with "
            "per-GPU BatchNorm statistics");
  if (!training) {
    BnEvalTable t;
    t.n = 0;
    for (const Unit& u : units)
      if (u.bn) {
        D3F_CHECK(t.n < PACK_MAX_LAYERS && u.coef_off % 16 == 0, "eval coefficients: table overflow");
        BnEvalEntry& e = t.e[t.n++];
        e.g_off = (uint32_t)u.g_off; e.b_off = (uint32_t)u.b_off;
        e.rm_off = (uint32_t)u.rm_off; e.rv_off = (uint32_t)u.rv_off;
        e.coef_off16 = (uint32_t)(u.coef_off >> 4);
        e.C = u.Cout;
      }
    if (int rc = bn_eval_coeff_all_launch(params_, bnstats, ws, t, s)) return rc;
  }
  for (int ui : fwd_order_) {
    if (ui < 0) {
      const TensorD& f1 = tensors[units[conv1].a];
      if (int rc = maxpool3x3s2_fwd_launch(dtype, T(units[conv1].a), T(t_pool),
                                           reinterpret_cast<uint8_t*>(ws + pool_idx_off), B, f1.H, f1.W,
                                           f1.C, s, ns))
        return rc;
      continue;
    }
    const Unit& u = units[ui];
    if (pack_mid_pending_ && ui >= first_mid_unit_) {
      D3F_HIP(hipStreamWaitEvent(s, ev_pack_mid_, 0));
      pack_mid_pending_ = false;
    }
    if (pack_pending_ && ui >= first_late_unit_) {
      D3F_HIP(hipStreamWaitEvent(s, ev_pack_done_, 0));
      pack_pending_ = false;
    }
    ConvFwdBufs b;
    b.src0 = T(u.in0);
    b.src1 = u.in1 >= 0 ? T(u.in1) : nullptr;
    b.w = ws + (u.wino ? u.wu_off : u.upfold ? u.wfc_off : u.wf_off);
    b.slabs = reinterpret_cast<float*>(ws + splitk_off);
    if (!u.bn) {
      b.out = out;
      b.bias = params_ + u.bias_off;
      if (int rc = conv_layer_forward(u, b, false, s, ns)) return rc;
      continue;
    }
    const Unit* ds = u.res_unit >= 0 ? &units[u.res_unit] : nullptr;
    if (training) {
      b.out = T(u.y);
      b.stats = reinterpret_cast<float*>(ws + stats_off);
      if (int rc = conv_layer_forward(u, b, u.wino, s, ns)) return rc;
      BnBufs n;
      n.stats = b.stats;
      n.gamma = params_ + u.g_off; n.beta = params_ + u.b_off;
      n.running_mean = bnstats + u.rm_off; n.running_var = bnstats + u.rv_off;
      n.coef = coef(u);
      n.y = T(u.y); n.a = u.a >= 0 ? T(u.a) : nullptr;
      n.res = u.res_tensor >= 0 ? T(u.res_tensor) : (ds ? T(ds->y) : nullptr);
      n.res_coef = ds ? coef(*ds) : nullptr;
      if (int rc = bn_layer_forward(u.norm, n, bn_sync(), s, ns)) return rc;
    } else {
      b.scale = bn_coef(coef(u), u.Cout, BN_SCALE);
      b.shift = bn_coef(coef(u), u.Cout, BN_SHIFT);
      b.relu = u.norm.relu ? 1 : 0;
      if (u.norm.apply) {
        b.out = T(u.a);
        b.res = u.res_tensor >= 0 ? T(u.res_tensor) : (ds ? T(ds->y) : nullptr);
      } else {
        b.out = T(u.y);
      }
      if (int rc = conv_layer_forward(u, b, u.wino, s, ns)) return rc;
    }
  }
  return 0;
}

int UnetEngine::predict_u8_launches(const float* params_, float* bnstats, const uint8_t* bgr_in, uint8_t* bgr_out,
                                    const float mean255[3], const float std255[3], char* ws, hipStream_t s) const {
  if (int rc = u8bgr_to_nhwc_launch(dtype, bgr_in, ws + tensors[t_x].off, (long)B * H * W, tensors[t_x].C, mean255,
                                    std255, s))
    return rc;
  float* head_out = reinterpret_cast<float*>(ws + head_nchw_off);
  if (int rc = forward_body(params_, bnstats, head_out, ws, 0, s)) return rc;
  return nchw_to_u8bgr_launch(head_out, bgr_out, B, H, W, 3L * W, mean255, std255, s);
}

int UnetEngine::predict_u8(const float* params_, float* bnstats, const uint8_t* bgr_in, uint8_t* bgr_out,
                           const float mean[3], const float stdv[3], void* ws_, int use_graph,
                           hipStream_t s) const {
  D3F_CHECK(in_channels == 3 && classes == 3, "predict_u8: 3-channel frames only (in %d, out %d)", in_channels, classes);
  char* ws = reinterpret_cast<char*>(ws_);
  float m255[3], s255[3];
  for (int c = 0; c < 3; ++c) {
    m255[c] = mean[c] * 255.0f;
    s255[c] = stdv[c] * 255.0f;
  }
  if (!use_graph) return predict_u8_launches(params_, bnstats, bgr_in, bgr_out, m255, s255, ws, s);
  const GraphKey key = {{params_, bnstats, bgr_in, bgr_out, ws_}, {m255[0], m255[1], m255[2], s255[0], s255[1], s255[2]}, {}};
  return graph_replay(g_predict_, key, s, [&](hipStream_t gs) {
    return predict_u8_launches(params_, bnstats, bgr_in, bgr_out, m255, s255, ws, gs);
  });
}

int UnetEngine::predict_frames_u8_launches(const float* params_, float* bnstats, const uint8_t* raw_in, const int geo[6],
                                           uint8_t* pair_out, const float mean255[3], const float std255[3], char* ws,
                                           hipStream_t s) const {
  if (int rc = crop_resize_cubic_u8_nhwc_launch(dtype, raw_in, B, geo[0], geo[1], geo[2], geo[3], geo[4], geo[5], pair_out,
                                                H, W, 6L * W, ws + tensors[t_x].off, tensors[t_x].C, mean255, std255, s))
    return rc;
  float* head_out = reinterpret_cast<float*>(ws + head_nchw_off);
  if (int rc = forward_body(params_, bnstats, head_out, ws, 0, s)) return rc;
  return nchw_to_u8bgr_launch(head_out, pair_out + 3L * W, B, H, W, 6L * W, mean255, std255, s);
}

int UnetEngine::predict_frames_u8(const float* params_, float* bnstats, const uint8_t* raw_in, int src_h, int src_w, int x1,
                                  int y1, int cw, int ch, uint8_t* pair_out, const float mean[3], const float stdv[3],
                                  void* ws_, int use_graph, hipStream_t s) const {
  D3F_CHECK(in_channels == 3 && classes == 3, "predict_frames_u8: 3-channel frames only (in %d, out %d)", in_channels,
            classes);
  char* ws = reinterpret_cast<char*>(ws_);
  float m255[3], s255[3];
  for (int c = 0; c < 3; ++c) {
    m255[c] = mean[c] * 255.0f;
    s255[c] = stdv[c] * 255.0f;
  }
  if (int rc = crop_resize_cubic_check(B, src_h, src_w, x1, y1, cw, ch, H, W, 6L * W)) return rc;
  const int geo[6] = {src_h, src_w, x1, y1, cw, ch};
  if (!use_graph) return predict_frames_u8_launches(params_, bnstats, raw_in, geo, pair_out, m255, s255, ws, s);
  const GraphKey key = {{params_, bnstats, raw_in, pair_out, ws_},
                        {m255[0], m255[1], m255[2], s255[0], s255[1], s255[2]},
                        {src_h, src_w, x1, y1, cw, ch}};
  return graph_replay(g_frames_, key, s, [&](hipStream_t gs) {
    return predict_frames_u8_launches(params_, bnstats, raw_in, geo, pair_out, m255, s255, ws, gs);
  });
}

int UnetEngine::forward_graph(const float* params_, float* bnstats, const float* x, float* out, void* ws_,
                              hipStream_t s) const {
  const GraphKey key = {{params_, bnstats, x, out, ws_}, {}, {}};
  return graph_replay(g_eval_, key, s, [&](hipStream_t gs) { return forward(params_, bnstats, x, out, ws_, 0, gs); });
}

int UnetEngine::train_step_launches(const StepArgs& a, void* ws_, hipStream_t s) const {
  const long per_image = (long)in_channels * H * W;
  if (int rc = pack_weights(a.params, ws_, s)) return rc;
  if (int rc = noise_blend_launch(a.image, a.noise, a.y_uniform, a.lam, a.noisy, nullptr, B, per_image, s)) return rc;
  if (int rc = forward(a.params, a.bnstats, a.noisy, a.pred, ws_, 1, s)) return rc;
  if (int rc = mse_ssim_loss_launch(a.pred, a.image, a.lo, a.hi, a.loss_out, a.gpred, a.loss_ws, B, H, W, s)) return rc;
  if (int rc = backward(a.params, a.gpred, a.grads, ws_, 0, num_segments, s, 1)) return rc;
  return adam_step_dev_launch(a.params, a.grads, a.exp_avg, a.exp_avg_sq, param_floats, a.adam_coef, s);
}

int UnetEngine::train_step(const StepArgs& a, void* ws_, int use_graph, hipStream_t s) const {
  D3F_CHECK(in_channels == 3 && classes == 3, "train_step: the (MSE + 1 - SSIM) / 2 objective is defined on 3-channel images");
  if (!use_graph) return train_step_launches(a, ws_, s);
  if (int rc = wait_for_packed_weights(s)) return rc;
  if (int rc = ensure_streams()) return rc;
  if (gstream_ == nullptr) {
    D3F_HIP(hipStreamCreateWithFlags(&gstream_, hipStreamNonBlocking));
    D3F_HIP(hipEventCreateWithFlags(&ev_gin_, hipEventDisableTiming));
    D3F_HIP(hipEventCreateWithFlags(&ev_gout_, hipEventDisableTiming));
  }
  const bool same = g_step_ != nullptr && g_step_ws_ == ws_ && memcmp(&a, &g_step_key_, sizeof(StepArgs)) == 0;
  if (!same) {
    if (g_step_) {
      (void)hipGraphExecDestroy(g_step_);
      g_step_ = nullptr;
    }
    hipGraph_t graph = nullptr;
    D3F_HIP(hipStreamBeginCapture(gstream_, hipStreamCaptureModeThreadLocal));
    const int rc = train_step_launches(a, ws_, gstream_);
    const hipError_t e = hipStreamEndCapture(gstream_, &graph);
    pack_pending_ = pack_mid_pending_ = false;
    side_dirty_ = false;
    if (rc != 0) {
      if (graph) (void)hipGraphDestroy(graph);
      return rc;
    }
    D3F_HIP(e);
    const hipError_t ei = hipGraphInstantiate(&g_step_, graph, nullptr, nullptr, 0);
    (void)hipGraphDestroy(graph);
    D3F_HIP(ei);
    g_step_key_ = a;
    g_step_ws_ = ws_;
  }
  D3F_HIP(hipGraphLaunch(g_step_, s));
  return 0;
}

int UnetEngine::wait_for_packed_weights(hipStream_t s) const {
  if (pack_mid_pending_) {
    D3F_HIP(hipStreamWaitEvent(s, ev_pack_mid_, 0));
    pack_mid_pending_ = false;
  }
  if (pack_pending_) {
    D3F_HIP(hipStreamWaitEvent(s, ev_pack_done_, 0));
    pack_pending_ = false;
  }
  return 0;
}

template <typename F>
int UnetEngine::graph_replay(GraphSlot& slot, const GraphKey& key, hipStream_t s, F&& launches) const {
  if (int rc = wait_for_packed_weights(s)) return rc;
  if (gstream_ == nullptr) {
    D3F_HIP(hipStreamCreateWithFlags(&gstream_, hipStreamNonBlocking));
    D3F_HIP(hipEventCreateWithFlags(&ev_gin_, hipEventDisableTiming));
    D3F_HIP(hipEventCreateWithFlags(&ev_gout_, hipEventDisableTiming));
  }
  static_assert(sizeof(GraphKey) == 5 * sizeof(void*) + 6 * sizeof(float) + 6 * sizeof(int), "GraphKey is compared bytewise");
  const bool same = slot.exec != nullptr && memcmp(&key, &slot.key, sizeof(GraphKey)) == 0;
  if (!same) {
    if (slot.exec) {
      (void)hipGraphExecDestroy(slot.exec);
      slot.exec = nullptr;
    }
    hipGraph_t graph = nullptr;
    D3F_HIP(hipStreamBeginCapture(gstream_, hipStreamCaptureModeThreadLocal));
    const int rc = launches(gstream_);
    const hipError_t e = hipStreamEndCapture(gstream_, &graph);
    if (rc != 0) {
      if (graph) (void)hipGraphDestroy(graph);
      return rc;
    }
    D3F_HIP(e);
    const hipError_t ei = hipGraphInstantiate(&slot.exec, graph, nullptr, nullptr, 0);
    (void)hipGraphDestroy(graph);
    D3F_HIP(ei);
    slot.key = key;
  }
  D3F_HIP(hipEventRecord(ev_gin_, s));
  D3F_HIP(hipStreamWaitEvent(gstream_, ev_gin_, 0));
  D3F_HIP(hipGraphLaunch(slot.exec, gstream_));
  D3F_HIP(hipEventRecord(ev_gout_, gstream_));
  D3F_HIP(hipStreamWaitEvent(s, ev_gout_, 0));
  return 0;
}

UnetEngine::~UnetEngine() {
  if (g_predict_.exec) (void)hipGraphExecDestroy(g_predict_.exec);
  if (g_eval_.exec) (void)hipGraphExecDestroy(g_eval_.exec);
  if (g_frames_.exec) (void)hipGraphExecDestroy(g_frames_.exec);
  if (g_step_) (void)hipGraphExecDestroy(g_step_);
  if (ev_gin_) (void)hipEventDestroy(ev_gin_);
  if (ev_gout_) (void)hipEventDestroy(ev_gout_);
  if (gstream_) (void)hipStreamDestroy(gstream_);
  for (hipEvent_t e : ev_dy_)
    if (e) (void)hipEventDestroy(e);
  if (ev_join_) (void)hipEventDestroy(ev_join_);
  if (ev_seg_) (void)hipEventDestroy(ev_seg_);
  if (ev_pack_in_) (void)hipEventDestroy(ev_pack_in_);
  if (ev_pack_done_) (void)hipEventDestroy(ev_pack_done_);
  if (ev_pack_mid_) (void)hipEventDestroy(ev_pack_mid_);
}

static bool serial_backward() {
  static const bool serial = getenv("D3F_SERIAL_BACKWARD") != nullptr;
  return serial;
}

hipStream_t UnetEngine::side_stream() const {
  if (serial_backward() || ensure_streams() != 0) return nullptr;
  return side_;
}

int UnetEngine::backward_join(hipStream_t s) const {
  if (side_ != nullptr && side_dirty_) {
    D3F_HIP(hipEventRecord(ev_join_, side_));
    D3F_HIP(hipStreamWaitEvent(s, ev_join_, 0));
    side_dirty_ = false;
  }
  return 0;
}

int UnetEngine::backward(const float* params_, const float* dout, float* grads, void* ws_,
                         int seg_begin, int seg_end, hipStream_t s, int join, const NetIO* io) const {
  char* ws = reinterpret_cast<char*>(ws_);
  D3F_CHECK(nets == 1 || (io != nullptr && bn_sync() == nullptr), "unet: the pair engine needs the second network's "
            "offsets and runs with per-GPU BatchNorm statistics");
  NetSplit split{};
  const NetSplit* ns = make_split(io, io ? io->dout : 0, &split) ? &split : nullptr;
  auto T = [&](int tid) { return ws + tensors[tid].off; };
  auto G = [&](int gid) { return gid == -2 ? ws + dz_off : ws + gtensors[gid].off; };
  auto coef = [&](const Unit& u) { return reinterpret_cast<float*>(ws + u.coef_off); };
  const bool serial = serial_backward();
#ifdef D3F_PROFILING
  static const char* abl = getenv("D3F_ABLATE_BACKWARD");
  const bool skip_w = abl && strchr(abl, 'w'), skip_d = abl && strchr(abl, 'd'), skip_b = abl && strchr(abl, 'b');
  const bool skip_r = abl && strchr(abl, 'r');
#else
  constexpr bool skip_w = false, skip_d = false, skip_b = false, skip_r = false;
#endif
  if (!serial)
    if (int rc = ensure_streams()) return rc;
  hipStream_t ws_stream = serial ? s : side_;
  size_t next_event = 0;
  bool side_used = false;
  constexpr int defer = 3;
  std::vector<int> pending;
  int pending_segment = -1;
  bool head_bias_pending = false;
  auto flush_pending = [&]() -> int {
    if (pending.empty()) return 0;
    if (!serial) {
      if (next_event == ev_dy_.size()) {
        hipEvent_t e = nullptr;
        D3F_HIP(hipEventCreateWithFlags(&e, hipEventDisableTiming));
        ev_dy_.push_back(e);
      }
      D3F_HIP(hipEventRecord(ev_dy_[next_event], s));
      D3F_HIP(hipStreamWaitEvent(side_, ev_dy_[next_event], 0));
      ++next_event;
      side_used = true;
    }
    if (head_bias_pending) {
      const Unit& uh = units[head];
      if (int rc = channel_sum_nchw_launch(dout, B, uh.Cout, (long)uh.Ho * uh.Wo, reinterpret_cast<float*>(ws + bsum_off),
                                           grads + uh.bias_off, ws_stream, ns))
        return rc;
      head_bias_pending = false;
    }
    for (int ui : pending) {
      const Unit& u = units[ui];
      WgradReduceBatch red;
      if (int rc = wgrad_layer_launch_deferred(u.wl, ws + u.dy_off, T(u.in0), u.in1 >= 0 ? T(u.in1) : nullptr,
                                               reinterpret_cast<float*>(ws + u.wslab_off), grads + u.w_off, u.Cout,
                                               u.CinReal, cdtype, red, ws_stream, ns))
        return rc;
      if (!skip_r)
        if (int rc = wgrad_reduce_batch_launch(red, ws_stream)) return rc;
    }
    pending.clear();
    return 0;
  };
  for (const BwdOp& op : bwd_ops) {
    if (op.segment < seg_begin || op.segment >= seg_end) continue;
    if (op.segment != pending_segment) {
      if (int rc = flush_pending()) return rc;
      pending_segment = op.segment;
    }
    if (op.kind == BW_SUM2X2) {
      if (int rc = sum2x2_launch(dtype, ws + dfull_off, G(op.dst0), B, op.Hl, op.Wl, op.C, s, ns)) return rc;
      continue;
    }
    if (op.kind == BW_POOL) {
      const TensorD& f1 = tensors[units[conv1].a];
      if (int rc = maxpool3x3s2_bwd_launch(dtype, G(op.dA), reinterpret_cast<uint8_t*>(ws + pool_idx_off),
                                           G(op.dst0), op.acc0 ? 1 : 0, B, f1.H, f1.W, f1.C, s, ns))
        return rc;
      continue;
    }
    const Unit& u = units[op.unit];
    char* dy = ws + u.dy_off;
    if (op.kind == BW_HEAD) {
      if (int rc = nchw_to_nhwc_launch(dtype, dout, dy, B, u.Cout, u.Ho, u.Wo, u.CoutD, s, ns)) return rc;
      if (skip_w) {
        if (int rc = channel_sum_nchw_launch(dout, B, u.Cout, (long)u.Ho * u.Wo,
                                             reinterpret_cast<float*>(ws + bsum_off), grads + u.bias_off, s, ns))
          return rc;
      } else {
        head_bias_pending = true;
      }
    } else if (!skip_b) {
      BnBufs n;
      n.stats = reinterpret_cast<float*>(ws + bnpart_off);
      n.gamma = params_ + u.g_off;
      n.coef = coef(u);
      n.y = T(u.y); n.a = u.a >= 0 ? T(u.a) : nullptr;
      n.dA = G(op.dA); n.dy = dy;
      n.dres = op.dres == -1 ? nullptr : G(op.dres); n.dres_acc = op.dres_acc ? 1 : 0;
      n.dgamma = grads + u.g_off; n.dbeta = grads + u.b_off;
      if (int rc = bn_layer_backward(u.norm, n, bn_sync(), s, ns)) return rc;
    }
    if (!skip_w) {
      pending.push_back(op.unit);
      if ((int)pending.size() >= defer)
        if (int rc = flush_pending()) return rc;
    }
    if (u.need_dgrad && !skip_d) {
      ConvDgradBufs d;
      d.dy = dy;
      d.w = ws + (u.upfold ? u.wd4_off : u.wd_off);
      d.w_skip = ws + u.wds_off;
      if (op.dst0_is_full_scratch) {
        d.dx0 = ws + dfull_off;
      } else {
        d.dx0 = G(op.dst0);
        d.acc0 = op.acc0 ? 1 : 0;
      }
      d.dx1 = op.dst1 >= 0 ? G(op.dst1) : nullptr;
      d.acc1 = op.acc1 ? 1 : 0;
      d.slabs = reinterpret_cast<float*>(ws + splitk_off);
      if (op.fuse_for_unit >= 0) {
        const Unit& uc = units[op.fuse_for_unit];
        d.bn_y = T(uc.y);
        d.bn_coef = bn_coef(coef(uc), uc.Cout, BN_MEAN);
        d.bn_partial = reinterpret_cast<float*>(ws + bnpart_off);
        d.bn_a = uc.norm.mask == BN_MASK_FROM_A ? T(uc.a) : nullptr;
      }
      if (int rc = conv_layer_dgrad(u, d, s, ns)) return rc;
    }
  }
  if (int rc = flush_pending()) return rc;
  if (!serial && side_used) side_dirty_ = true;
  if (!serial && !join) {
    D3F_HIP(hipEventRecord(ev_seg_, s));
    D3F_HIP(hipStreamWaitEvent(side_, ev_seg_, 0));
    side_dirty_ = true;
  } else if (!serial) {
    if (int rc = backward_join(s)) return rc;
  }
  return 0;
}

const TensorD* UnetEngine::find_export(const char* name) const {
  const std::string n(name);
  const size_t colon = n.rfind(':');
  if (colon == std::string::npos) return nullptr;
  const std::string un = n.substr(0, colon), kind = n.substr(colon + 1);
  if (kind != "y" && kind != "a" && kind != "da") return nullptr;
  for (const Unit& u : units) {
    if (u.conv_name != un) continue;
    const int tid = kind == "y" ? u.y : u.a;
    if (tid < 0) return nullptr;
    if (kind == "da") return grad_of[tid] >= 0 ? &gtensors[grad_of[tid]] : nullptr;
    return &tensors[tid];
  }
  return nullptr;
}

int UnetEngine::export_tensor(const char* name, const void* ws_, float* out_nchw, hipStream_t s) const {
  const TensorD* t = find_export(name);
  D3F_CHECK(t != nullptr, "export: no tensor named '%s' (expected '<conv name>:y|a|da')", name);
  return nhwc_to_nchw_launch(dtype, reinterpret_cast<const char*>(ws_) + t->off, out_nchw, B, t->C, t->H, t->W, t->C, s);
}

int UnetEngine::export_shape(const char* name, int32_t dims[3]) const {
  const TensorD* t = find_export(name);
  D3F_CHECK(t != nullptr, "export: no tensor named '%s' (expected '<conv name>:y|a|da')", name);
  dims[0] = t->C; dims[1] = t->H; dims[2] = t->W;
  return 0;
}

}
```

denoising_diffusion_deep_fake_amd/csrc/loss.hip:

```cpp
#include "pointwise.h"
#include "philox.h"

namespace d3f {

constexpr int SS_T = 32;
constexpr int SS_K = 11;
constexpr int SS_IN = SS_T + SS_K - 1;
constexpr int SS_LD = SS_IN + 1;

struct GaussK {
  float g[SS_K];
};

static GaussK make_gauss() {
  GaussK k;
  float s = 0.f;
  for (int i = 0; i < SS_K; ++i) {
    const float d = (float)i - (float)(SS_K - 1) / 2.f;
    k.g[i] = expf(-(d * d) / (2.f * 1.5f * 1.5f));
    s += k.g[i];
  }
  for (int i = 0; i < SS_K; ++i) k.g[i] /= s;
  return k;
}

__device__ __forceinline__ float norm01(float v, float lo, float range) {
  const float t = (v - lo) / range;
  return fminf(fmaxf(t, 0.f), 1.f);
}

__global__ __launch_bounds__(256) void ssim_fwd_kernel(const float* __restrict__ pred,
                                                       const float* __restrict__ target, float lo,
                                                       float range, GaussK gk, int H, int W,
                                                       float* __restrict__ dA, float* __restrict__ dB,
                                                       float* __restrict__ dC,
                                                       float* __restrict__ partial) {
  chain_priority();
  __shared__ float tx[SS_IN * SS_LD], ty[SS_IN * SS_LD];
  __shared__ float vv[5][SS_T * SS_LD];
  __shared__ float wsum[4];
  const int Hv = H - (SS_K - 1), Wv = W - (SS_K - 1);
  const int plane = blockIdx.z;
  const int oy0 = blockIdx.y * SS_T, ox0 = blockIdx.x * SS_T;
  const float* __restrict__ px = pred + (long)plane * H * W;
  const float* __restrict__ py = target + (long)plane * H * W;
  const int tid = threadIdx.x;
  for (int e = tid; e < SS_IN * SS_IN; e += 256) {
    const int r = e / SS_IN, c = e - r * SS_IN;
    const int iy = oy0 + r, ix = ox0 + c;
    float a = 0.f, b = 0.f;
    if (iy < H && ix < W) {
      a = norm01(px[(long)iy * W + ix], lo, range);
      b = norm01(py[(long)iy * W + ix], lo, range);
    }
    tx[r * SS_LD + c] = a;
    ty[r * SS_LD + c] = b;
  }
  __syncthreads();
  constexpr int RB = 8;
  if (tid < SS_IN * (SS_T / RB)) {
    const int c = tid % SS_IN, r0 = (tid / SS_IN) * RB;
    float a[RB + SS_K - 1], b[RB + SS_K - 1], aa[RB + SS_K - 1], bb[RB + SS_K - 1], ab[RB + SS_K - 1];
#pragma unroll
    for (int i = 0; i < RB + SS_K - 1; ++i) {
      a[i] = tx[(r0 + i) * SS_LD + c];
      b[i] = ty[(r0 + i) * SS_LD + c];
      aa[i] = a[i] * a[i];
      bb[i] = b[i] * b[i];
      ab[i] = a[i] * b[i];
    }
#pragma unroll
    for (int r = 0; r < RB; ++r) {
      float s0 = 0.f, s1 = 0.f, s2 = 0.f, s3 = 0.f, s4 = 0.f;
#pragma unroll
      for (int i = 0; i < SS_K; ++i) {
        const float g = gk.g[i];
        s0 += g * a[r + i];
        s1 += g * b[r + i];
        s2 += g * aa[r + i];
        s3 += g * bb[r + i];
        s4 += g * ab[r + i];
      }
      vv[0][(r0 + r) * SS_LD + c] = s0;
      vv[1][(r0 + r) * SS_LD + c] = s1;
      vv[2][(r0 + r) * SS_LD + c] = s2;
      vv[3][(r0 + r) * SS_LD + c] = s3;
      vv[4][(r0 + r) * SS_LD + c] = s4;
    }
  }
  __syncthreads();
  const float c1 = 0.01f * 0.01f, c2 = 0.03f * 0.03f;
  float local = 0.f;
  constexpr int CBk = 4;
  const int rr = tid / (SS_T / CBk), cq = (tid % (SS_T / CBk)) * CBk;
  float win[5][CBk + SS_K - 1];
#pragma unroll
  for (int q = 0; q < 5; ++q)
#pragma unroll
    for (int j = 0; j < CBk + SS_K - 1; ++j) win[q][j] = vv[q][rr * SS_LD + cq + j];
#pragma unroll
  for (int cc = 0; cc < CBk; ++cc) {
    const int r = rr, c = cq + cc;
    const int oy = oy0 + r, ox = ox0 + c;
    if (oy >= Hv || ox >= Wv) continue;
    float m[5];
#pragma unroll
    for (int q = 0; q < 5; ++q) {
      float s = 0.f;
#pragma unroll
      for (int j = 0; j < SS_K; ++j) s += gk.g[j] * win[q][cc + j];
      m[q] = s;
    }
    const float mux = m[0], muy = m[1];
    const float sxx = m[2] - mux * mux, syy = m[3] - muy * muy, sxy = m[4] - mux * muy;
    const float a1 = 2.f * mux * muy + c1, b1 = mux * mux + muy * muy + c1;
    const float a2 = 2.f * sxy + c2, b2 = sxx + syy + c2;
    const float l = a1 / b1, cs = a2 / b2;
    const float ss = l * cs;
    local += ss;
    const long o = ((long)plane * Hv + oy) * Wv + ox;
    const float dl_dmux = 2.f * (muy - l * mux) / b1;
    const float dcs_dmux = (2.f * mux * cs - 2.f * muy) / b2;
    dA[o] = cs * dl_dmux + l * dcs_dmux;
    dB[o] = -l * cs / b2;
    dC[o] = 2.f * l / b2;
  }
#pragma unroll
  for (int o = 32; o > 0; o >>= 1) local += __shfl_xor(local, o);
  if ((tid & 63) == 0) wsum[tid >> 6] = local;
  __syncthreads();
  if (tid == 0)
    partial[((long)blockIdx.z * gridDim.y + blockIdx.y) * gridDim.x + blockIdx.x] =
        (wsum[0] + wsum[1]) + (wsum[2] + wsum[3]);
}

__global__ __launch_bounds__(256) void ssim_mse_bwd_kernel(
    const float* __restrict__ pred, const float* __restrict__ target, float lo, float range, GaussK gk,
    int H, int W, const float* __restrict__ dA, const float* __restrict__ dB,
    const float* __restrict__ dC, float ssim_coef, float mse_coef, float* __restrict__ grad,
    float* __restrict__ partial_mse) {
  chain_priority();
  __shared__ float t3[3][SS_IN * SS_LD];
  __shared__ float vv[3][SS_T * SS_LD];
  __shared__ float wsum[4];
  const int Hv = H - (SS_K - 1), Wv = W - (SS_K - 1);
  const int plane = blockIdx.z;
  const int py0 = blockIdx.y * SS_T, px0 = blockIdx.x * SS_T;
  const int tid = threadIdx.x;
  for (int e = tid; e < SS_IN * SS_IN; e += 256) {
    const int r = e / SS_IN, c = e - r * SS_IN;
    const int oy = py0 - (SS_K - 1) + r, ox = px0 - (SS_K - 1) + c;
    float a = 0.f, b = 0.f, d = 0.f;
    if (oy >= 0 && oy < Hv && ox >= 0 && ox < Wv) {
      const long o = ((long)plane * Hv + oy) * Wv + ox;
      a = dA[o];
      b = dB[o];
      d = dC[o];
    }
    t3[0][r * SS_LD + c] = a;
    t3[1][r * SS_LD + c] = b;
    t3[2][r * SS_LD + c] = d;
  }
  __syncthreads();
  constexpr int RB = 8;
  if (tid < SS_IN * (SS_T / RB)) {
    const int c = tid % SS_IN, r0 = (tid / SS_IN) * RB;
    float v0[RB + SS_K - 1], v1[RB + SS_K - 1], v2[RB + SS_K - 1];
#pragma unroll
    for (int i = 0; i < RB + SS_K - 1; ++i) {
      v0[i] = t3[0][(r0 + i) * SS_LD + c];
      v1[i] = t3[1][(r0 + i) * SS_LD + c];
      v2[i] = t3[2][(r0 + i) * SS_LD + c];
    }
#pragma unroll
    for (int r = 0; r < RB; ++r) {
      float s0 = 0.f, s1 = 0.f, s2 = 0.f;
#pragma unroll
      for (int i = 0; i < SS_K; ++i) {
        const float g = gk.g[SS_K - 1 - i];
        s0 += g * v0[r + i];
        s1 += g * v1[r + i];
        s2 += g * v2[r + i];
      }
      vv[0][(r0 + r) * SS_LD + c] = s0;
      vv[1][(r0 + r) * SS_LD + c] = s1;
      vv[2][(r0 + r) * SS_LD + c] = s2;
    }
  }
  __syncthreads();
  const float inv_range = 1.f / range;
  float local = 0.f;
  constexpr int CBk = 4;
  const int rr = tid / (SS_T / CBk), cq = (tid % (SS_T / CBk)) * CBk;
  float win[3][CBk + SS_K - 1];
#pragma unroll
  for (int q = 0; q < 3; ++q)
#pragma unroll
    for (int j = 0; j < CBk + SS_K - 1; ++j) win[q][j] = vv[q][rr * SS_LD + cq + j];
#pragma unroll
  for (int cc = 0; cc < CBk; ++cc) {
    const int r = rr, c = cq + cc;
    const int iy = py0 + r, ix = px0 + c;
    if (iy >= H || ix >= W) continue;
    float ga = 0.f, gb = 0.f, gc = 0.f;
#pragma unroll
    for (int j = 0; j < SS_K; ++j) {
      const float g = gk.g[SS_K - 1 - j];
      ga += g * win[0][cc + j];
      gb += g * win[1][cc + j];
      gc += g * win[2][cc + j];
    }
    const long p = (long)plane * H * W + (long)iy * W + ix;
    const float pv = pred[p], tv = target[p];
    const float rawx = (pv - lo) / range;
    const float xh = fminf(fmaxf(rawx, 0.f), 1.f);
    const float yh = norm01(tv, lo, range);
    float gx = ga + 2.f * xh * gb + yh * gc;
    gx = (rawx >= 0.f && rawx <= 1.f) ? gx * inv_range : 0.f;
    const float diff = pv - tv;
    local += diff * diff;
    grad[p] = ssim_coef * gx + mse_coef * diff;
  }
#pragma unroll
  for (int o = 32; o > 0; o >>= 1) local += __shfl_xor(local, o);
  if ((tid & 63) == 0) wsum[tid >> 6] = local;
  __syncthreads();
  if (tid == 0)
    partial_mse[((long)blockIdx.z * gridDim.y + blockIdx.y) * gridDim.x + blockIdx.x] =
        (wsum[0] + wsum[1]) + (wsum[2] + wsum[3]);
}

__global__ __launch_bounds__(256) void loss_finalize_kernel(const float* __restrict__ part_ss, int n_ss,
                                                            const float* __restrict__ part_mse,
                                                            int n_mse, double n_ssim_elems,
                                                            double n_elems, float* __restrict__ out) {
  chain_priority();
  __shared__ double red[2][256];
  double a = 0.0, b = 0.0;
  for (int i = threadIdx.x; i < n_ss; i += 256) a += (double)part_ss[i];
  for (int i = threadIdx.x; i < n_mse; i += 256) b += (double)part_mse[i];
  red[0][threadIdx.x] = a;
  red[1][threadIdx.x] = b;
  __syncthreads();
  for (int s = 128; s > 0; s >>= 1) {
    if (threadIdx.x < s) {
      red[0][threadIdx.x] += red[0][threadIdx.x + s];
      red[1][threadIdx.x] += red[1][threadIdx.x + s];
    }
    __syncthreads();
  }
  if (threadIdx.x == 0) {
    const float ssim = (float)(red[0][0] / n_ssim_elems);
    const float mse = (float)(red[1][0] / n_elems);
    out[0] = (mse + (1.0f - ssim)) / 2.0f;
    out[1] = mse;
    out[2] = ssim;
  }
}

static inline int tiles(int n) { return (n + SS_T - 1) / SS_T; }

size_t loss_workspace_floats(int B, int H, int W) {
  if (H < SS_K || W < SS_K) return 0;
  const long planes = (long)B * 3;
  const long maps = 3 * planes * (H - SS_K + 1) * (W - SS_K + 1);
  const long p1 = planes * tiles(H - SS_K + 1) * tiles(W - SS_K + 1);
  const long p2 = planes * tiles(H) * tiles(W);
  return (size_t)(maps + p1 + p2 + 16);
}

int mse_ssim_loss_launch(const float* pred, const float* target, float in_min, float in_max,
                         float* loss_out, float* grad_pred, float* workspace, int B, int H, int W,
                         hipStream_t stream) {
  D3F_CHECK(H >= SS_K && W >= SS_K, "loss: image %dx%d smaller than the 11x11 SSIM window", H, W);
  D3F_CHECK(in_max > in_min, "loss: input range");
  static const GaussK gk = make_gauss();
  const int Hv = H - SS_K + 1, Wv = W - SS_K + 1;
  const long planes = (long)B * 3;
  const long map = planes * Hv * Wv;
  float* dA = workspace;
  float* dB = dA + map;
  float* dC = dB + map;
  float* part_ss = dC + map;
  const int n_ss = (int)(planes * tiles(Hv) * tiles(Wv));
  float* part_mse = part_ss + n_ss;
  const int n_mse = (int)(planes * tiles(H) * tiles(W));
  const float range = in_max - in_min;
  hipLaunchKernelGGL(ssim_fwd_kernel, dim3(tiles(Wv), tiles(Hv), (unsigned)planes), dim3(256), 0, stream,
                     pred, target, in_min, range, gk, H, W, dA, dB, dC, part_ss);
  D3F_HIP(hipGetLastError());
  const double n_elems = (double)planes * H * W;
  const double n_ssim = (double)planes * Hv * Wv;
  const float ssim_coef = (float)(-0.5 / n_ssim);
  const float mse_coef = (float)(1.0 / n_elems);
  hipLaunchKernelGGL(ssim_mse_bwd_kernel, dim3(tiles(W), tiles(H), (unsigned)planes), dim3(256), 0,
                     stream, pred, target, in_min, range, gk, H, W, dA, dB, dC, ssim_coef, mse_coef,
                     grad_pred, part_mse);
  D3F_HIP(hipGetLastError());
  hipLaunchKernelGGL(loss_finalize_kernel, dim3(1), dim3(256), 0, stream, part_ss, n_ss, part_mse, n_mse,
                     n_ssim, n_elems, loss_out);
  D3F_HIP(hipGetLastError());
  return 0;
}

struct BlendCoef {
  float r, sa, sb;
};
__device__ __forceinline__ BlendCoef blend_coef(float y, float c, float one_minus_c, float inv_lam) {
  const float t = __fadd_rn(__fmul_rn(y, one_minus_c), c);
  const float r = inv_lam > 0.f ? __fmul_rn(inv_lam, (float)log((double)__fdiv_rn(1.0f, t))) : y;
  return BlendCoef{r, __fsqrt_rn(__fsub_rn(1.0f, r)), __fsqrt_rn(r)};
}
__device__ __forceinline__ float4 blend4(const BlendCoef k, const float4 a, const float4 n) {
  float4 o;
  o.x = __fadd_rn(__fmul_rn(k.sa, a.x), __fmul_rn(k.sb, n.x));
  o.y = __fadd_rn(__fmul_rn(k.sa, a.y), __fmul_rn(k.sb, n.y));
  o.z = __fadd_rn(__fmul_rn(k.sa, a.z), __fmul_rn(k.sb, n.z));
  o.w = __fadd_rn(__fmul_rn(k.sa, a.w), __fmul_rn(k.sb, n.w));
  return o;
}

__global__ __launch_bounds__(256) void noise_blend_kernel(const float* __restrict__ x,
                                                          const float* __restrict__ noise,
                                                          const float* __restrict__ y_uniform,
                                                          float c, float one_minus_c, float inv_lam,
                                                          float* __restrict__ out,
                                                          float* __restrict__ r_out, long per_image) {
  const int b = blockIdx.y;
  const BlendCoef k = blend_coef(y_uniform[b], c, one_minus_c, inv_lam);
  if (r_out != nullptr && blockIdx.x == 0 && threadIdx.x == 0) r_out[b] = k.r;
  const long nvec = per_image / 4;
  const float4* __restrict__ xv = reinterpret_cast<const float4*>(x + (long)b * per_image);
  const float4* __restrict__ nv = reinterpret_cast<const float4*>(noise + (long)b * per_image);
  float4* __restrict__ ov = reinterpret_cast<float4*>(out + (long)b * per_image);
  for (long i = (long)blockIdx.x * 256 + threadIdx.x; i < nvec; i += (long)gridDim.x * 256) ov[i] = blend4(k, xv[i], nv[i]);
}

int noise_blend_launch(const float* x, const float* noise, const float* y_uniform, float lam,
                       float* out, float* r_out, int B, long per_image, hipStream_t stream) {
  D3F_CHECK(per_image % 4 == 0, "noise_blend: per-image element count %ld not a multiple of 4", per_image);
  D3F_CHECK(lam > 0.f, "noise_blend: lambda must be positive");
  if (B == 0 || per_image == 0) return 0;
  const double c = 1.0 / exp((double)lam);
  long bx = (per_image / 4 + 255) / 256;
  if (bx > 256) bx = 256;
  hipLaunchKernelGGL(noise_blend_kernel, dim3((unsigned)bx, (unsigned)B), dim3(256), 0, stream, x, noise,
                     y_uniform, (float)c, (float)(1.0 - c), (float)(1.0 / (double)lam), out, r_out,
                     per_image);
  D3F_HIP(hipGetLastError());
  return 0;
}

int noise_blend_fixed_launch(const float* x, const float* noise, const float* r, float* out, int B, long per_image,
                             hipStream_t stream) {
  D3F_CHECK(per_image % 4 == 0, "noise_blend: per-image element count %ld not a multiple of 4", per_image);
  if (B == 0 || per_image == 0) return 0;
  long bx = (per_image / 4 + 255) / 256;
  if (bx > 256) bx = 256;
  hipLaunchKernelGGL(noise_blend_kernel, dim3((unsigned)bx, (unsigned)B), dim3(256), 0, stream, x, noise, r, 0.f, 0.f,
                     -1.f, out, (float*)nullptr, per_image);
  D3F_HIP(hipGetLastError());
  return 0;
}

__global__ __launch_bounds__(256) void noise_blend_rng_kernel(const float* __restrict__ x, uint64_t seed, uint64_t offset,
                                                              const float* __restrict__ y_or_r, float c,
                                                              float one_minus_c, float inv_lam, float* __restrict__ out,
                                                              float* __restrict__ r_out, long per_image) {
  chain_priority();
  const int b = blockIdx.y;
  const BlendCoef k = blend_coef(y_or_r != nullptr ? y_or_r[b] : rng_y(seed, offset, b), c, one_minus_c, inv_lam);
  if (r_out != nullptr && blockIdx.x == 0 && threadIdx.x == 0) r_out[b] = k.r;
  const long nvec = per_image / 4;
  const float4* __restrict__ xv = reinterpret_cast<const float4*>(x + (long)b * per_image);
// ... 100 lines not shown
```

denoising_diffusion_deep_fake_amd/csrc/pointwise.h:

```cpp
#pragma once
#include <string>

#include "common.h"

namespace d3f {

constexpr int PACK_MAX_LAYERS = 64;

enum BnCoefRow { BN_MEAN, BN_INVSTD, BN_SCALE, BN_SHIFT, BN_K, BN_COEF_ROWS = BN_K + 3 };
inline float* bn_coef(float* block, int C, BnCoefRow row) { return block + (long)row * C; }
inline const float* bn_coef(const float* block, int C, BnCoefRow row) { return block + (long)row * C; }

struct BnEvalEntry {
  uint32_t g_off, b_off, rm_off, rv_off;
  uint32_t coef_off16;
  int32_t C;
};
struct BnEvalTable {
  int n;
  BnEvalEntry e[PACK_MAX_LAYERS];
};
int bn_eval_coeff_all_launch(const float* params, const float* bnstats, void* ws, const BnEvalTable& t,
                             hipStream_t stream);

enum BnResidual { BN_RES_NONE, BN_RES_TENSOR, BN_RES_LAYER };
enum BnMask { BN_MASK_NONE, BN_MASK_FROM_Y, BN_MASK_FROM_A };
struct BnLayer {
  std::string name;
  int C = 0, Cpad = 0;
  long rows = 0;
  int dtype = D3F_F32;
  int plan_nets = 1;
  bool apply = true, relu = true;
  BnResidual res = BN_RES_NONE;
  BnMask mask = BN_MASK_NONE;
  int fwd_rows = 0;
  int fused_rows = 0;
  bool allow_fused = false;
  bool fwd_fused = false, bwd_fused = false;
  int reduce_blocks = 0;
  int bwd_rows = 0;
  long rows_per_block = 0;
  size_t stat_floats = 0;
  size_t part_floats = 0;
};
void bn_layer_plan(BnLayer& L);
struct BnBufs {
  float* stats = nullptr;
  const float *gamma = nullptr, *beta = nullptr;
  float *running_mean = nullptr, *running_var = nullptr;
  float* coef = nullptr;
  float* k = nullptr;
  const void* y = nullptr;
  void* a = nullptr;
  const void* res = nullptr;
  const float* res_coef = nullptr;
  const void* dA = nullptr;
  void* dy = nullptr;
  void* dres = nullptr;
  int dres_acc = 0;
  float *dgamma = nullptr, *dbeta = nullptr;
};
struct BnSync {
  int (*fn)(void* ctx, float* data, int64_t count, void* stream);
  void* ctx;
  int world;
};
int bn_layer_forward(const BnLayer& L, const BnBufs& b, const BnSync* sync, hipStream_t stream,
                     const NetSplit* ns = nullptr);
int bn_layer_backward(const BnLayer& L, const BnBufs& b, const BnSync* sync, hipStream_t stream,
                      const NetSplit* ns = nullptr);
int bn_layer_finalize(const BnLayer& L, const BnBufs& b, long count, hipStream_t stream, const NetSplit* ns = nullptr);
int bn_layer_apply(const BnLayer& L, const BnBufs& b, hipStream_t stream, const NetSplit* ns = nullptr);

int maxpool3x3s2_fwd_launch(int dtype, const void* in, void* out, uint8_t* idx, int B, int H, int W,
                            int C, hipStream_t stream, const NetSplit* ns = nullptr);
int maxpool3x3s2_bwd_launch(int dtype, const void* dout, const uint8_t* idx, void* din, int accumulate,
                            int B, int H, int W, int C, hipStream_t stream, const NetSplit* ns = nullptr);
int sum2x2_launch(int dtype, const void* dfull, void* dlow, int B, int Hl, int Wl, int C,
                  hipStream_t stream, const NetSplit* ns = nullptr);
int nchw_to_nhwc_launch(int dtype, const float* in, void* out, int B, int C, int H, int W, int Cpad,
                        hipStream_t stream, const NetSplit* ns = nullptr);
int nhwc_to_nchw_launch(int dtype, const void* in, float* out, int B, int C, int H, int W, int Cpad,
                        hipStream_t stream);

int u8bgr_to_nhwc_launch(int dtype, const uint8_t* in, void* out, long npix, int Cpad, const float mean255[3],
                         const float std255[3], hipStream_t stream);
int nchw_to_u8bgr_launch(const float* in, uint8_t* out, int B, int H, int W, long out_row_stride, const float mean255[3],
                         const float std255[3], hipStream_t stream);

int crop_resize_cubic_check(int B, int src_h, int src_w, int x1, int y1, int cw, int ch, int H, int W, long dst_row_stride);
int crop_resize_cubic_u8_launch(const uint8_t* src, int B, int src_h, int src_w, int x1, int y1, int cw, int ch,
                                uint8_t* dst, int H, int W, long dst_row_stride, hipStream_t stream);
int crop_resize_cubic_u8_nhwc_launch(int dtype, const uint8_t* src, int B, int src_h, int src_w, int x1, int y1, int cw,
                                     int ch, uint8_t* dst, int H, int W, long dst_row_stride, void* act, int Cpad,
                                     const float mean255[3], const float std255[3], hipStream_t stream);

int u8rgb_to_nchw_launch(const uint8_t* in, float* out, int B, long HW, const float mean[3], const float stdv[3],
                         hipStream_t stream);

int affine_warp_launch(const float* in, const float* theta, float* out, int B, int C, int H, int W,
                       hipStream_t stream);
struct AffineRngParams {
  int kind;
  float angle_unit;
  float deg2rad;
  float scale_lo, scale_span;
  float shift_x, shift_y;
  float p;
  float h_over_w, w_over_h;
};
int affine_rng_params(int kind, const float params[5], int H, int W, AffineRngParams& q);
int affine_warp_rng_launch(const float* in, float* out, uint64_t seed, uint64_t offset, const AffineRngParams& q, int B,
                           int C, int H, int W, hipStream_t stream);
int affine_theta_draw_launch(uint64_t seed, uint64_t offset, const AffineRngParams& q, float* theta, uint8_t* apply, int B,
                             hipStream_t stream);

int pack_up_launch(int dtype, const float* w, int Cout, int C0, int C1, void* wfc, int CoutPad, void* wd4,
                   int C0Rows, void* wds, int C1Rows, hipStream_t stream);

constexpr int PACK_NT = 32;
constexpr int PACK_LDS_ROW = 288;
struct PackEntry {
  uint32_t w_off;
  uint32_t wf_off16, wd_off16;
  uint32_t block0;
  uint16_t Cout, CinReal, Cin, taps, CoutPad, Kpad, CinRows, CoutD, KpadD, has_d, CT, ctiles;
  uint16_t conv_stride;
  uint16_t has_f;
  uint16_t taps_shr, ct_log2;
  uint32_t taps_mul;
};
struct PackTable {
  int n;
  PackEntry e[PACK_MAX_LAYERS];
};
static_assert(sizeof(PackEntry) == 52, "PackTable travels as a kernel argument: keep its entries small");
int pack_all_launch(int dtype, const float* params, void* ws, const PackTable& t, int blocks,
                    hipStream_t stream);

int noise_blend_launch(const float* x, const float* noise, const float* y_uniform, float lam,
                       float* out, float* r_out, int B, long per_image, hipStream_t stream);
int noise_blend_fixed_launch(const float* x, const float* noise, const float* r, float* out, int B, long per_image,
                             hipStream_t stream);
int noise_blend_rng_launch(const float* x, uint64_t seed, uint64_t offset, float lam, float* out, float* r_out, int B,
                           long per_image, hipStream_t stream);
int noise_blend_fixed_rng_launch(const float* x, uint64_t seed, uint64_t offset, const float* r, float* out, int B,
                                 long per_image, hipStream_t stream);
int noise_draw_launch(uint64_t seed, uint64_t offset, float* noise, float* y, int B, long per_image,
                      hipStream_t stream);
size_t l1_per_image_workspace_bytes(int B);
int l1_per_image_launch(const float* pred, const float* target, float* out, void* workspace, int B, long per_image,
                        hipStream_t stream);
size_t loss_workspace_floats(int B, int H, int W);
int mse_ssim_loss_launch(const float* pred, const float* target, float in_min, float in_max,
                         float* loss_out , float* grad_pred, float* workspace,
                         int B, int H, int W, hipStream_t stream);
int adam_step_launch(float* p, const float* g, float* m, float* v, long n, float lr, float beta1,
                     float beta2, float eps, int step, float grad_scale, hipStream_t stream);
void adam_coefficients(float lr, float beta1, float beta2, float eps, int step, float grad_scale, float coef[8]);
int adam_step_dev_launch(float* p, const float* g, float* m, float* v, long n, const float* coef_dev,
                         hipStream_t stream);
int ema_lerp_launch(float* ema, const float* online, long n, float weight, hipStream_t stream);

}
```

denoising_diffusion_deep_fake_amd/ops.py:

```python
import ctypes as C

import torch

from . import _lib
from ._lib import ConvDesc, check, ptr, stream_ptr

F32, BF16, F32X3 = _lib.F32, _lib.BF16, _lib.F32X3


def _tdtype(dtype):
    return torch.bfloat16 if dtype == BF16 else torch.float32


def _dev(t):
    if t.device.type != "cuda":
        raise _lib.D3FError("libd3f_hip ops need tensors on the HIP device (no CPU fallback)")
    return t.device


def make_desc(B, H, W, C0, C1, Cout, k, stride, pad, upsample0=False, cin_real=None):
    return ConvDesc(B, H, W, C0, C1, 1 if upsample0 else 0, Cout, k, k, stride, pad,
                    cin_real if cin_real is not None else C0 + C1)


# ... 7 lines not shown
    check(_lib.lib().d3f_nchw_to_nhwc(dtype, ptr(x.contiguous().float()), ptr(out), B, Cc, H, W, cpad, stream_ptr()))
    return out


def nhwc_to_nchw(x, c, dtype=F32):
    B, H, W, cpad = x.shape
    out = torch.empty((B, c, H, W), dtype=torch.float32, device=_dev(x))
    check(_lib.lib().d3f_nhwc_to_nchw(dtype, ptr(x.contiguous()), ptr(out), B, c, H, W, cpad, stream_ptr()))
    return out


def pack_weights(d, w, dtype=F32, dgrad=True):
    L = _lib.lib()
    dev = _dev(w)
    wf = torch.empty(L.d3f_conv_packed_bytes(dtype, C.byref(d), 0), dtype=torch.uint8, device=dev)
    wd = torch.empty(L.d3f_conv_packed_bytes(dtype, C.byref(d), 1), dtype=torch.uint8, device=dev) if dgrad else None
    check(L.d3f_conv_pack_weights(dtype, C.byref(d), ptr(w.contiguous().float()), ptr(wf), ptr(wd), stream_ptr()))
    return wf, wd


def _conv_ws(d, dtype, which, dev, splitk):
    if not splitk:
        return None
    n = _lib.lib().d3f_conv_workspace_bytes(dtype, C.byref(d), which)
    return torch.empty(max(n, 16), dtype=torch.uint8, device=dev)


def conv_forward(d, src0, src1, wf, dtype=F32, want_stats=True, splitk=False):
    L = _lib.lib()
    ho, wo = out_hw(d)
    y = torch.empty((d.B, ho, wo, d.Cout), dtype=_tdtype(dtype), device=_dev(src0))
    ws = _conv_ws(d, dtype, 0, y.device, splitk)
    tiles = C.c_int()
    n = L.d3f_conv_stats_floats(dtype, C.byref(d), int(splitk), C.byref(tiles))
    stats = torch.zeros(n, dtype=torch.float32, device=y.device) if want_stats else None
    check(L.d3f_conv_forward(dtype, C.byref(d), ptr(src0), ptr(src1), ptr(wf), ptr(y), ptr(stats), ptr(ws),
                             stream_ptr()))
    return y, stats, tiles.value


def conv_winograd_applies(d, dtype=F32):
    return bool(_lib.lib().d3f_conv_winograd_applies(dtype, C.byref(d)))


def conv_winograd_pack(d, w):
    L = _lib.lib()
    n = L.d3f_conv_winograd_filter_bytes(C.byref(d))
    if n == 0:
        raise _lib.D3FError("conv_winograd_pack: the layer does not fit the Winograd kernel")
    u = torch.empty(n, dtype=torch.uint8, device=_dev(w))
    check(L.d3f_conv_winograd_pack(C.byref(d), ptr(w.contiguous().float()), ptr(u), stream_ptr()))
    return u


def conv_winograd_forward(d, src0, u, want_stats=True, scale=None, shift=None, residual=None, relu=False):
    L = _lib.lib()
    y = torch.empty((d.B, d.H, d.W, d.Cout), dtype=torch.float32, device=_dev(src0))
    tiles = C.c_int()
    n = L.d3f_conv_winograd_stats_floats(C.byref(d), C.byref(tiles))
    stats = torch.zeros(n, dtype=torch.float32, device=y.device) if (want_stats and scale is None) else None
    check(L.d3f_conv_winograd_forward(C.byref(d), ptr(src0), ptr(u), ptr(y), ptr(stats), ptr(scale), ptr(shift),
                                      ptr(residual), int(relu), stream_ptr()))
    return y, stats, tiles.value


def conv_upsample_folded(d, dtype=F32):
    return bool(d.upsample0) and bool(_lib.lib().d3f_conv_upsample_folded(dtype, C.byref(d)))


def conv_backward_data(d, dy, wd, dtype=F32, dx0=None, dx1=None, acc0=False, acc1=False, splitk=False, summed=None):
    dev = _dev(dy)
    ws = _conv_ws(d, dtype, 1, dev, splitk)
    folded = bool(d.upsample0) and bool(_lib.lib().d3f_conv_upsample_folded(dtype, C.byref(d)))
    if bool(d.upsample0) and not folded and summed is not False and \
            bool(_lib.lib().d3f_conv_upsample_summed(dtype, C.byref(d))):
        d = ConvDesc(*[getattr(d, n) for n, _ in ConvDesc._fields_])
        d.upsample0 = 2
        folded = True
    low = (d.B, d.H // 2, d.W // 2, d.C0)
    if d.upsample0 and not folded:
        if acc0 or dx0 is not None:
            raise ValueError("conv_backward_data: an up-sampled source that is not folded takes no dx0 / acc0")
        full = torch.empty((d.B, d.H, d.W, d.C0), dtype=_tdtype(dtype), device=dev)
    elif dx0 is None:
        full = None
        dx0 = torch.empty(low if d.upsample0 else (d.B, d.H, d.W, d.C0), dtype=_tdtype(dtype), device=dev)
    else:
        full = None
    if dx1 is None and d.C1 > 0:
        dx1 = torch.empty((d.B, d.H, d.W, d.C1), dtype=_tdtype(dtype), device=dev)
    check(_lib.lib().d3f_conv_backward_data(dtype, C.byref(d), ptr(dy), ptr(wd), ptr(full if full is not None else dx0),
                                            ptr(dx1), int(acc0), int(acc1), ptr(ws), stream_ptr()))
    if full is not None:
        dx0 = upsample2x_backward(full, dtype)
    return dx0, dx1


def conv_backward_weight(d, dy, src0, src1, dtype=F32):
    L = _lib.lib()
    ws = torch.empty(L.d3f_conv_backward_weight_workspace_bytes(dtype, C.byref(d)), dtype=torch.uint8, device=_dev(dy))
    dw = torch.empty((d.Cout, d.CinReal, d.KH, d.KW), dtype=torch.float32, device=dy.device)
    check(L.d3f_conv_backward_weight(dtype, C.byref(d), ptr(dy), ptr(src0), ptr(src1), ptr(ws), ptr(dw), stream_ptr()))
    return dw


def bn_finalize(stats, tiles, Cc, count, gamma, beta, running_mean=None, running_var=None):
    coef = torch.empty(4 * Cc, dtype=torch.float32, device=_dev(stats))
    check(_lib.lib().d3f_bn_finalize(ptr(stats), tiles, Cc, count, ptr(gamma), ptr(beta), ptr(running_mean),
                                     ptr(running_var), ptr(coef), stream_ptr()))
    return coef


def bn_apply(y, coef, residual=None, relu=True, dtype=F32):
    Cc = y.shape[-1]
    out = torch.empty_like(y)
    check(_lib.lib().d3f_bn_apply(dtype, ptr(y), ptr(coef), Cc, y.numel() // Cc, ptr(residual), int(relu),
                                  ptr(out), stream_ptr()))
    return out


def bn_backward(dA, a, y, coef, gamma, want_dres=False, dtype=F32):
    L = _lib.lib()
    Cc = y.shape[-1]
    rows = y.numel() // Cc
    ws = torch.empty(L.d3f_bn_backward_workspace_bytes(dtype, Cc, rows), dtype=torch.uint8, device=_dev(y))
    dy = torch.empty_like(y)
    dres = torch.empty_like(y) if want_dres else None
    dgamma = torch.empty(Cc, dtype=torch.float32, device=y.device)
    dbeta = torch.empty(Cc, dtype=torch.float32, device=y.device)
    check(L.d3f_bn_backward(dtype, ptr(dA), ptr(a), ptr(y), ptr(coef), ptr(gamma), Cc, rows, ptr(dy), ptr(dres),
                            ptr(dgamma), ptr(dbeta), ptr(ws), stream_ptr()))
    return dy, dres, dgamma, dbeta


def bn_desc(C_, rows, dtype=F32, cpad=None, apply=True, relu=True, res=0, mask=0, fwd_rows=0, fused_rows=0,
            allow_fused=True, plan_nets=1):
    return _lib.BnDesc(dtype, C_, C_ if cpad is None else cpad, rows, int(apply), int(relu), res, mask, fwd_rows,
                       fused_rows, int(allow_fused), plan_nets)


def bn_layer_plan(d):
    p = _lib.BnPlan()
    check(_lib.lib().d3f_bn_layer_plan(C.byref(d), C.byref(p)))
    return p


def bn_layer_forward(d, stats, gamma, beta, coef, y, a=None, res=None, res_coef=None, running_mean=None,
                     running_var=None):
    check(_lib.lib().d3f_bn_layer_forward(C.byref(d), ptr(stats), ptr(gamma), ptr(beta), ptr(running_mean),
                                          ptr(running_var), ptr(coef), ptr(y), ptr(res), ptr(res_coef), ptr(a),
                                          stream_ptr()))


def bn_layer_backward(d, partial, gamma, coef, y, dA, dy, a=None, dres=None, dres_acc=False, dgamma=None, dbeta=None):
    check(_lib.lib().d3f_bn_layer_backward(C.byref(d), ptr(partial), ptr(gamma), ptr(coef), ptr(y), ptr(a), ptr(dA),
                                           ptr(dy), ptr(dres), int(dres_acc), ptr(dgamma), ptr(dbeta), stream_ptr()))


def maxpool_forward(x, dtype=F32):
    B, H, W, Cc = x.shape
    out = torch.empty((B, H // 2, W // 2, Cc), dtype=x.dtype, device=_dev(x))
    idx = torch.empty((B, H // 2, W // 2, Cc), dtype=torch.uint8, device=x.device)
    check(_lib.lib().d3f_maxpool3x3s2_forward(dtype, ptr(x), ptr(out), ptr(idx), B, H, W, Cc, stream_ptr()))
    return out, idx


def maxpool_backward(dout, idx, H, W, dtype=F32, din=None):
    B, _, _, Cc = dout.shape
    acc = din is not None
    if din is None:
        din = torch.empty((B, H, W, Cc), dtype=dout.dtype, device=_dev(dout))
    check(_lib.lib().d3f_maxpool3x3s2_backward(dtype, ptr(dout), ptr(idx), ptr(din), int(acc), B, H, W, Cc, stream_ptr()))
    return din


def upsample2x_backward(dfull, dtype=F32):
    B, H, W, Cc = dfull.shape
    out = torch.empty((B, H // 2, W // 2, Cc), dtype=dfull.dtype, device=_dev(dfull))
    check(_lib.lib().d3f_upsample2x_backward(dtype, ptr(dfull), ptr(out), B, H // 2, W // 2, Cc, stream_ptr()))
    return out


def affine_warp(x, theta):
    x = x.contiguous().float()
    B, Cc, H, W = x.shape
    theta = theta.to(device=_dev(x), dtype=torch.float32).contiguous()
    if theta.shape != (B, 2, 3):
        raise ValueError(f"theta must be [{B}, 2, 3], got {list(theta.shape)}")
    out = torch.empty_like(x)
    check(_lib.lib().d3f_affine_warp(ptr(x), ptr(theta), ptr(out), B, Cc, H, W, stream_ptr()))
    return out


def _affine_rng_params(kind, params):
    kinds = {"random_affine": 0, "shift_scale_rotate": 1}
    kind = kinds.get(kind, kind)
    if kind not in (0, 1):
        raise ValueError(f"kind must be one of {sorted(kinds)} (or 0 / 1), got {kind!r}")
    params = [float(v) for v in params]
    if len(params) != (5 if kind == 0 else 4):
        raise ValueError("params: (degrees, translate_x, translate_y, scale_lo, scale_hi) for random_affine, "
                         "(shift_limit, scale_limit, rotate_limit, p) for shift_scale_rotate")
    return kind, (C.c_float * 5)(*(params + [0.0] * (5 - len(params))))


def affine_warp_rng(x, seed, offset, kind, params):
    x = x.contiguous().float()
    B, Cc, H, W = x.shape
    kind, cparams = _affine_rng_params(kind, params)
    out = torch.empty_like(x)
    check(_lib.lib().d3f_affine_warp_rng(ptr(x), ptr(out), int(seed), int(offset), kind, cparams, B, Cc, H, W,
                                         stream_ptr()))
    return out


def affine_theta_draw(seed, offset, kind, params, B, H, W, device="cuda"):
    kind, cparams = _affine_rng_params(kind, params)
    theta = torch.empty((B, 2, 3), dtype=torch.float32, device=device)
    apply = torch.empty(B, dtype=torch.uint8, device=device)
    _dev(theta)
    check(_lib.lib().d3f_affine_theta_draw(int(seed), int(offset), kind, cparams, ptr(theta), ptr(apply), B, H, W,
                                           stream_ptr()))
    return theta, apply.bool()


def u8rgb_normalise(frames, mean, std):
    if frames.dtype != torch.uint8 or frames.dim() != 4 or frames.shape[-1] != 3:
        raise ValueError("u8rgb_normalise expects uint8 frames [B, H, W, 3] (RGB)")
    frames = frames.contiguous()
    B, H, W, _ = frames.shape
    out = torch.empty((B, 3, H, W), dtype=torch.float32, device=_dev(frames))
    m = (C.c_float * 3)(*[float(v) for v in mean])
    s = (C.c_float * 3)(*[float(v) for v in std])
    check(_lib.lib().d3f_u8rgb_normalise(ptr(frames), ptr(out), B, H, W, m, s, stream_ptr()))
    return out


def noise_blend(x, noise, y_uniform, lam, return_r=False):
    x = x.contiguous().float()
    out = torch.empty_like(x)
    B = x.shape[0]
    r = torch.empty(B, dtype=torch.float32, device=_dev(x)) if return_r else None
    check(_lib.lib().d3f_noise_blend(ptr(x), ptr(noise.contiguous().float()), ptr(y_uniform.contiguous().float()),
                                     float(lam), ptr(out), ptr(r), B, x.numel() // max(B, 1), stream_ptr()))
    return (out, r) if return_r else out


def noise_blend_fixed(x, noise, ratio):
    x = x.contiguous().float()
    B = x.shape[0]
    r = ratio if torch.is_tensor(ratio) else torch.ones(B, device=_dev(x)) * float(ratio)
    r = r.to(device=_dev(x), dtype=torch.float32).reshape(-1).contiguous()
    out = torch.empty_like(x)
    check(_lib.lib().d3f_noise_blend_fixed(ptr(x), ptr(noise.contiguous().float()), ptr(r), ptr(out), B,
                                           x.numel() // max(B, 1), stream_ptr()))
    return out


def noise_blend_rng(x, seed, offset, lam, return_r=False):
    x = x.contiguous().float()
    out = torch.empty_like(x)
    B = x.shape[0]
    r = torch.empty(B, dtype=torch.float32, device=_dev(x)) if return_r else None
    check(_lib.lib().d3f_noise_blend_rng(ptr(x), int(seed), int(offset), float(lam), ptr(out), ptr(r), B,
                                         x.numel() // max(B, 1), stream_ptr()))
    return (out, r) if return_r else out


def noise_blend_fixed_rng(x, seed, offset, ratio):
    x = x.contiguous().float()
    B = x.shape[0]
    r = ratio if torch.is_tensor(ratio) else torch.ones(B, device=_dev(x)) * float(ratio)
    r = r.to(device=_dev(x), dtype=torch.float32).reshape(-1).contiguous()
    out = torch.empty_like(x)
    check(_lib.lib().d3f_noise_blend_fixed_rng(ptr(x), int(seed), int(offset), ptr(r), ptr(out), B,
                                               x.numel() // max(B, 1), stream_ptr()))
    return out


def noise_draw(seed, offset, shape, device="cuda", noise=True, y=True):
    shape = tuple(int(v) for v in shape)
    B = shape[0]
    per_image = 1
    for v in shape[1:]:
        per_image *= v
    n = torch.empty(shape, dtype=torch.float32, device=device) if noise else None
    yy = torch.empty(B, dtype=torch.float32, device=device) if y else None
    _dev(n if n is not None else yy)
    check(_lib.lib().d3f_noise_draw(int(seed), int(offset), ptr(n), ptr(yy), B, per_image, stream_ptr()))
    return n, yy


def philox4x32_10(counter, key):
    c = (C.c_uint32 * 4)(*[int(v) & 0xFFFFFFFF for v in counter])
    k = (C.c_uint32 * 2)(*[int(v) & 0xFFFFFFFF for v in key])
    out = (C.c_uint32 * 4)()
    check(_lib.lib().d3f_philox4x32_10(c, k, out))
    return tuple(int(v) for v in out)


def l1_per_image(pred, target):
    L = _lib.lib()
    pred, target = pred.contiguous().float(), target.contiguous().float()
    B = pred.shape[0]
    ws = torch.empty(L.d3f_l1_per_image_workspace_bytes(B), dtype=torch.uint8, device=_dev(pred))
    out = torch.empty(B, dtype=torch.float32, device=pred.device)
# ... 57 lines not shown
```

include/d3f_hip.h:

```cpp
#ifndef D3F_HIP_H
#define D3F_HIP_H
#include <stddef.h>
#include <stdint.h>

#ifdef __cplusplus
extern "C" {
#endif

#define D3F_F32 0
#define D3F_BF16 1
#define D3F_F32X3 2

int d3f_version(void);
const char* d3f_last_error(void);
const char* d3f_source_digest(void);

int d3f_profile_enable(int max_launches);
int d3f_profile_classes(int mask);
int d3f_profile_collect(double ms[3], int64_t launches[3], double flops[3]);

typedef struct d3f_unet* d3f_unet_t;

int d3f_unet_create(const char* encoder_name, int in_channels, int classes, int B, int H, int W,
                    int dtype, d3f_unet_t* out);
int d3f_unet_destroy(d3f_unet_t h);

int d3f_unet_create_nets(const char* encoder_name, int in_channels, int classes, int B, int H, int W, int dtype,
                         int nets, int plan_nets, d3f_unet_t* out);
int d3f_unet_nets(d3f_unet_t h);
size_t d3f_unet_net_workspace_stride(d3f_unet_t h);
int d3f_unet_pair_pack_weights(d3f_unet_t h, const float* const params[2], void* workspace, void* stream);
int d3f_unet_pair_forward(d3f_unet_t h, const float* const params[2], float* const bnstats[2], const float* const x[2],
                          float* const out[2], void* workspace, void* stream);
int d3f_unet_pair_backward(d3f_unet_t h, const float* const params[2], const float* const grad_out[2],
                           float* const grads[2], void* workspace, int seg_begin, int seg_end, int join, void* stream);

int d3f_unet_num_params(d3f_unet_t h);
int d3f_unet_param_info(d3f_unet_t h, int i, char* name, int name_cap, int32_t shape[4], int* ndim,
                        int64_t* offset);
int64_t d3f_unet_param_floats(d3f_unet_t h);
int d3f_unet_num_bn(d3f_unet_t h);
int d3f_unet_bn_info(d3f_unet_t h, int i, char* prefix, int prefix_cap, int* C, int64_t* rm_offset,
                     int64_t* rv_offset);
int64_t d3f_unet_bnstat_floats(d3f_unet_t h);
size_t d3f_unet_workspace_bytes(d3f_unet_t h);
double d3f_unet_forward_flops(d3f_unet_t h);
double d3f_unet_backward_flops(d3f_unet_t h);

int d3f_unet_pack_weights(d3f_unet_t h, const float* params, void* workspace, void* stream);
int d3f_unet_forward(d3f_unet_t h, const float* params, float* bnstats, const float* x, float* out,
                     void* workspace, int training, void* stream);
int d3f_unet_forward_graph(d3f_unet_t h, const float* params, float* bnstats, const float* x, float* out,
                           void* workspace, void* stream);
int d3f_unet_predict_u8(d3f_unet_t h, const float* params, float* bnstats, const uint8_t* bgr_in, uint8_t* bgr_out,
                        const float mean[3], const float std[3], void* workspace, int use_graph, void* stream);
int d3f_unet_predict_frames_u8(d3f_unet_t h, const float* params, float* bnstats, const uint8_t* raw_in, int src_h,
                               int src_w, int x1, int y1, int cw, int ch, uint8_t* pair_out, const float mean[3],
                               const float std[3], void* workspace, int use_graph, void* stream);
int d3f_unet_num_segments(d3f_unet_t h);
int d3f_unet_plan_counts(d3f_unet_t h, int32_t fwd[16], int32_t dgrad[16], int32_t wgrad[16]);
int d3f_unet_segment_range(d3f_unet_t h, int segment, int64_t* begin, int64_t* end);
int d3f_unet_backward(d3f_unet_t h, const float* params, const float* grad_out, float* grads,
                      void* workspace, int seg_begin, int seg_end, void* stream);
int d3f_unet_backward_nojoin(d3f_unet_t h, const float* params, const float* grad_out, float* grads,
                             void* workspace, int seg_begin, int seg_end, void* stream);
int d3f_unet_side_stream(d3f_unet_t h, void** stream_out);
int d3f_unet_backward_join(d3f_unet_t h, void* stream);
typedef struct d3f_step_buffers {
  float* params; float* bnstats; float* grads; float* exp_avg; float* exp_avg_sq;
  const float* image;
  const float* noise;
  const float* y_uniform;
  float* noisy;
  float* pred;
  float* grad_pred;
  float* loss_out;
  void* loss_workspace;
  const float* adam_coef;
} d3f_step_buffers;
int d3f_adam_coefficients(float lr, float beta1, float beta2, float eps, int step, float grad_scale, float coef[8]);
int d3f_unet_train_step(d3f_unet_t h, const d3f_step_buffers* buffers, float lambda, float input_min, float input_max,
                        void* workspace, int use_graph, void* stream);
typedef int (*d3f_allreduce_fn)(void* ctx, float* data, int64_t count, void* stream);
int d3f_unet_set_bn_sync(d3f_unet_t h, d3f_allreduce_fn fn, void* ctx, int world_size);
int d3f_unet_export(d3f_unet_t h, const char* name, const void* workspace, float* out_nchw, void* stream);
int d3f_unet_export_shape(d3f_unet_t h, const char* name, int32_t dims[3]);

typedef struct d3f_conv_desc {
  int32_t B, H, W;
  int32_t C0, C1;
  int32_t upsample0;
  int32_t Cout, KH, KW, stride, pad;
  int32_t CinReal;
} d3f_conv_desc;

size_t d3f_conv_packed_bytes(int dtype, const d3f_conv_desc* d, int which);
int d3f_conv_pack_weights(int dtype, const d3f_conv_desc* d, const float* w, void* w_fwd, void* w_dgrad,
                          void* stream);
size_t d3f_conv_workspace_bytes(int dtype, const d3f_conv_desc* d, int which);
size_t d3f_conv_stats_floats(int dtype, const d3f_conv_desc* d, int with_workspace, int* tiles);
int d3f_conv_forward(int dtype, const d3f_conv_desc* d, const void* src0, const void* src1,
                     const void* w_fwd, void* y, float* stats, void* workspace, void* stream);
int d3f_conv_winograd_applies(int dtype, const d3f_conv_desc* d);
size_t d3f_conv_winograd_filter_bytes(const d3f_conv_desc* d);
size_t d3f_conv_winograd_stats_floats(const d3f_conv_desc* d, int* tiles);
int d3f_conv_winograd_pack(const d3f_conv_desc* d, const float* w, void* u, void* stream);
int d3f_conv_winograd_forward(const d3f_conv_desc* d, const void* src0, const void* u, void* y, float* stats,
                              const float* scale, const float* shift, const void* residual, int relu, void* stream);
int d3f_conv_upsample_folded(int dtype, const d3f_conv_desc* d);
int d3f_conv_upsample_summed(int dtype, const d3f_conv_desc* d);
int d3f_conv_backward_data(int dtype, const d3f_conv_desc* d, const void* dy, const void* w_dgrad,
                           void* dx0, void* dx1, int acc0, int acc1, void* workspace, void* stream);
size_t d3f_conv_backward_weight_workspace_bytes(int dtype, const d3f_conv_desc* d);
int d3f_conv_backward_weight(int dtype, const d3f_conv_desc* d, const void* dy, const void* src0,
                             const void* src1, void* workspace, float* dw, void* stream);

int d3f_bn_finalize(const float* stats, int tiles, int C, int64_t count, const float* gamma,
                    const float* beta, float* running_mean, float* running_var, float* coef, void* stream);
int d3f_bn_apply(int dtype, const void* y, const float* coef, int C, int64_t rows, const void* residual,
                 int relu, void* out, void* stream);
size_t d3f_bn_backward_workspace_bytes(int dtype, int C, int64_t rows);
int d3f_bn_backward(int dtype, const void* dA, const void* a_or_null, const void* y, const float* coef,
                    const float* gamma, int C, int64_t rows, void* dy, void* dres, float* dgamma,
                    float* dbeta, void* workspace, void* stream);

typedef struct d3f_bn_desc {
  int32_t dtype, C, Cpad;
  int64_t rows;
  int32_t apply, relu;
  int32_t res;
  int32_t mask;
  int32_t fwd_rows;
  int32_t fused_rows;
  int32_t allow_fused, plan_nets;
} d3f_bn_desc;
typedef struct d3f_bn_plan {
  int32_t fwd_fused, bwd_fused;
  int32_t reduce_blocks;
  int32_t bwd_rows;
  int64_t rows_per_block;
  uint64_t stat_floats;
  uint64_t part_floats;
} d3f_bn_plan;
#define D3F_BN_COEF_ROWS 7
int d3f_bn_layer_plan(const d3f_bn_desc* d, d3f_bn_plan* plan);
int d3f_bn_layer_forward(const d3f_bn_desc* d, float* stats, const float* gamma, const float* beta, float* running_mean,
                         float* running_var, float* coef, const void* y, const void* res, const float* res_coef, void* a,
                         void* stream);
int d3f_bn_layer_backward(const d3f_bn_desc* d, float* partial, const float* gamma, float* coef, const void* y,
                          const void* a, const void* dA, void* dy, void* dres, int dres_acc, float* dgamma, float* dbeta,
                          void* stream);
int d3f_unet_bn_layer(d3f_unet_t h, int i, d3f_bn_desc* d, d3f_bn_plan* plan);

int d3f_maxpool3x3s2_forward(int dtype, const void* in, void* out, uint8_t* idx, int B, int H, int W, int C, void* stream);
int d3f_maxpool3x3s2_backward(int dtype, const void* dout, const uint8_t* idx, void* din, int accumulate,
                              int B, int H, int W, int C, void* stream);
int d3f_upsample2x_backward(int dtype, const void* dfull, void* dlow, int B, int Hlow, int Wlow, int C, void* stream);
int d3f_nchw_to_nhwc(int dtype, const float* in, void* out, int B, int C, int H, int W, int Cpad, void* stream);
int d3f_nhwc_to_nchw(int dtype, const void* in, float* out, int B, int C, int H, int W, int Cpad, void* stream);
int d3f_u8rgb_normalise(const uint8_t* in_hwc, float* out_nchw, int B, int H, int W, const float mean[3],
                        const float std[3], void* stream);

int d3f_crop_resize_cubic_u8(const uint8_t* src, int B, int src_h, int src_w, int x1, int y1, int cw, int ch, uint8_t* dst,
                             int H, int W, int64_t dst_row_stride_bytes, void* stream);

int d3f_affine_warp(const float* in, const float* theta, float* out, int B, int C, int H, int W, void* stream);

int d3f_philox4x32_10(const uint32_t counter[4], const uint32_t key[2], uint32_t out[4]);

int d3f_affine_warp_rng(const float* in, float* out, uint64_t seed, uint64_t offset, int kind,
                        const float params[5], int B, int C, int H, int W, void* stream);
int d3f_affine_theta_draw(uint64_t seed, uint64_t offset, int kind, const float params[5],
                          float* theta, uint8_t* apply, int B, int H, int W, void* stream);

int d3f_noise_blend(const float* x, const float* noise, const float* y_uniform, float lam, float* out,
                    float* r_out_or_null, int B, int64_t per_image, void* stream);
int d3f_noise_blend_fixed(const float* x, const float* noise, const float* r, float* out, int B, int64_t per_image,
                          void* stream);
int d3f_noise_blend_rng(const float* x, uint64_t seed, uint64_t offset, float lam, float* out,
                        float* r_out_or_null, int B, int64_t per_image, void* stream);
int d3f_noise_blend_fixed_rng(const float* x, uint64_t seed, uint64_t offset, const float* r, float* out, int B,
                              int64_t per_image, void* stream);
int d3f_noise_draw(uint64_t seed, uint64_t offset, float* noise_or_null, float* y_or_null, int B, int64_t per_image,
                   void* stream);
size_t d3f_l1_per_image_workspace_bytes(int B);
int d3f_l1_per_image(const float* prediction, const float* target, float* out, void* workspace, int B,
                     int64_t per_image, void* stream);
size_t d3f_mse_ssim_loss_workspace_bytes(int B, int H, int W);
int d3f_mse_ssim_loss(const float* pred, const float* target, float input_min, float input_max,
                      float* loss_out, float* grad_pred, void* workspace, int B, int H, int W, void* stream);
int d3f_adam_step(float* params, const float* grads, float* exp_avg, float* exp_avg_sq, int64_t n,
                  float lr, float beta1, float beta2, float eps, int step, float grad_scale, void* stream);
int d3f_ema_lerp(float* ema, const float* online, int64_t n, float weight, void* stream);

#ifdef __cplusplus
}
#endif
#endif
```

Measured before the change: 2042 images/sec.

## Fuse stem BN apply with maxpool, split weight packing, vectorise SSIM backward

Adds a fused kernel that finalizes the stem BatchNorm, applies it with ReLU, writes the activation and computes the 3x3 stride-2 maxpool with its indices in one pass. This avoids a separate maxpool launch and a full re-read of the stem activation. It also gives the first part of weight packing on the side stream its own event so the forward can start earlier, reworks the conv1 weight-gradient scheduling, and rewrites the SSIM/MSE loss backward to use paired-float shared tiles and vector loads. These bring more code paths and extra event dependencies, and the fused kernel's banded grid may occupy the GPU less well than the separate kernels did.

```diff
diff --git a/denoising_diffusion_deep_fake_amd/_lib.py b/denoising_diffusion_deep_fake_amd/_lib.py
--- a/denoising_diffusion_deep_fake_amd/_lib.py
+++ b/denoising_diffusion_deep_fake_amd/_lib.py
@@ -105,6 +105,7 @@
     "d3f_bn_backward": (_i, [_i, _p, _p, _p, _p, _p, _i, _i64, _p, _p, _p, _p, _p, _p]),
     "d3f_bn_layer_plan": (_i, [_bnd, _bnp]),
     "d3f_bn_layer_forward": (_i, [_bnd, _p, _p, _p, _p, _p, _p, _p, _p, _p, _p, _p]),
+    "d3f_bn_layer_forward_pool": (_i, [_bnd, _p, _p, _p, _p, _p, _p, _p, _p, _p, _p, _i, _i, _p]),
     "d3f_bn_layer_backward": (_i, [_bnd, _p, _p, _p, _p, _p, _p, _p, _p, _i, _p, _p, _p]),
     "d3f_unet_bn_layer": (_i, [_p, _i, _bnd, _bnp]),
     "d3f_maxpool3x3s2_forward": (_i, [_i, _p, _p, _p, _i, _i, _i, _i, _p]),
diff --git a/denoising_diffusion_deep_fake_amd/csrc/batchnorm.hip b/denoising_diffusion_deep_fake_amd/csrc/batchnorm.hip
--- a/denoising_diffusion_deep_fake_amd/csrc/batchnorm.hip
+++ b/denoising_diffusion_deep_fake_amd/csrc/batchnorm.hip
@@ -493,6 +493,129 @@
     };
     if (L.res != BN_RES_NONE) go(bn_finalize_apply_kernel<T, true>);
     else go(bn_finalize_apply_kernel<T, false>);
+  });
+  D3F_HIP(hipGetLastError());
+  return 0;
+}
+
+template <typename T>
+__global__ __launch_bounds__(256) void bn_finalize_apply_pool_kernel(
+    const float* __restrict__ stats, int stat_rows, int C, int Cpad, double count,
+    const float* __restrict__ gamma, const float* __restrict__ beta, float eps, float momentum,
+    float* __restrict__ running_mean, float* __restrict__ running_var, float* __restrict__ mean_o,
+    float* __restrict__ invstd_o, float* __restrict__ scale_o, float* __restrict__ shift_o,
+    const T* __restrict__ y, int relu, T* __restrict__ out, T* __restrict__ pool, uint8_t* __restrict__ idx,
+    int H, int W, int bands_per_image, int band_rows, NetSplit ns) {
+  chain_priority();
+  if (blockIdx.z != 0) {
+    net_shift(stats, ns.ws); net_shift(gamma, ns.par); net_shift(beta, ns.par);
+    net_shift(running_mean, ns.bn); net_shift(running_var, ns.bn);
+    net_shift(mean_o, ns.ws); net_shift(invstd_o, ns.ws); net_shift(scale_o, ns.ws); net_shift(shift_o, ns.ws);
+    net_shift(y, ns.ws); net_shift(out, ns.ws); net_shift(pool, ns.ws); net_shift(idx, ns.ws);
+  }
+  __shared__ double red[16][64];
+  __shared__ double tot[64];
+  __shared__ float cf[2][BNF_SC];
+  typedef typename Raw4<T>::type raw_t;
+  const int tid = threadIdx.x, c0 = blockIdx.y * BNF_SC;
+  const int v = tid & 7, cc = c0 + v * 4;
+  const int Ho = H / 2, Wo = W / 2;
+  const int b = (int)blockIdx.x / bands_per_image, band = (int)blockIdx.x - b * bands_per_image;
+  const int p0 = band * band_rows, p1 = p0 + band_rows < Ho ? p0 + band_rows : Ho;
+  const T* __restrict__ yb = y + (long)b * H * W * C + cc;
+  T* __restrict__ ab = out + (long)b * H * W * C + cc;
+  auto load = [&](raw_t (&t)[9], int oy, int ox) {
+#pragma unroll
+    for (int kh = 0; kh < 3; ++kh)
+#pragma unroll
+      for (int kw = 0; kw < 3; ++kw) {
+        int iy = 2 * oy - 1 + kh, ix = 2 * ox - 1 + kw;
+        if (iy < 0) iy = 2 * oy;
+        if (ix < 0) ix = 2 * ox;
+        t[kh * 3 + kw] = ldraw(yb + ((long)iy * W + ix) * C);
+      }
+  };
+  const int items = (p1 - p0) * Wo;
+  int it = tid >> 3;
+  int oy = p0 + it / Wo, ox = it % Wo;
+  auto step = [&](int& r, int& c) {
+    c += 32;
+    while (c >= Wo) { c -= Wo; ++r; }
+  };
+  raw_t cur[9], nxt[9];
+  slab_reduce(stats, stat_rows, Cpad, c0, red, tot, [&]() {
+    if (it < items) load(cur, oy, ox);
+  });
+  if (tid < BNF_SC) {
+    const float2 f = bn_fwd_coef(tot[2 * tid], tot[2 * tid + 1], count, c0 + tid, gamma, beta, eps, momentum,
+                                 blockIdx.x == 0, running_mean, running_var, mean_o, invstd_o, scale_o, shift_o);
+    cf[0][tid] = f.x;
+    cf[1][tid] = f.y;
+  }
+  __syncthreads();
+  float sc[4], sf[4];
+#pragma unroll
+  for (int k = 0; k < 4; ++k) {
+    sc[k] = cf[0][v * 4 + k];
+    sf[k] = cf[1][v * 4 + k];
+  }
+  for (; it < items; it += 32) {
+    int oyn = oy, oxn = ox;
+    step(oyn, oxn);
+    if (it + 32 < items) load(nxt, oyn, oxn);
+    float best[4];
+    int bi[4];
+    bool first = true;
+#pragma unroll
+    for (int kh = 0; kh < 3; ++kh) {
+      const int iy = 2 * oy - 1 + kh;
+      if (iy < 0) continue;
+#pragma unroll
+      for (int kw = 0; kw < 3; ++kw) {
+        const int ix = 2 * ox - 1 + kw;
+        if (ix < 0) continue;
+        const float4 yv = cvt4(cur[kh * 3 + kw]);
+        float x[4] = {yv.x, yv.y, yv.z, yv.w};
+#pragma unroll
+        for (int k = 0; k < 4; ++k) {
+          x[k] = x[k] * sc[k] + sf[k];
+          if (relu) x[k] = fmaxf(x[k], 0.f);
+        }
+        if (kh >= 1 && kw >= 1) st4<T>(ab + ((long)iy * W + ix) * C, make_float4(x[0], x[1], x[2], x[3]));
+#pragma unroll
+        for (int k = 0; k < 4; ++k) {
+          const float r = to_f32<T>(from_f32<T>(x[k]));
+          if (first || r > best[k] || r != r) { best[k] = r; bi[k] = kh * 3 + kw; }
+        }
+        first = false;
+      }
+    }
+    const long o = (((long)b * Ho + oy) * Wo + ox) * C + cc;
+    st4<T>(pool + o, make_float4(best[0], best[1], best[2], best[3]));
+    *reinterpret_cast<uint32_t*>(idx + o) = (uint32_t)bi[0] | ((uint32_t)bi[1] << 8) | ((uint32_t)bi[2] << 16) |
+                                            ((uint32_t)bi[3] << 24);
+#pragma unroll
+    for (int k = 0; k < 9; ++k) cur[k] = nxt[k];
+    oy = oyn;
+    ox = oxn;
+  }
+}
+
+static int bn_finalize_apply_pool_launch(const BnLayer& L, const BnBufs& b, hipStream_t stream, const NetSplit* ns) {
+  const int H = b.pool_H, W = b.pool_W;
+  const long B = L.rows / ((long)H * W);
+  const int band_rows = (int)std::clamp(L.rows_per_block / (2L * W), 1L, (long)(H / 2));
+  const int bands = (H / 2 + band_rows - 1) / band_rows;
+  D3F_CHECK(B * bands <= 0x7fffffffL, "bn_layer_forward: %ld pool bands exceed the grid", B * bands);
+  const NetSplit nv = net_split_or_single(ns);
+  const dim3 grid((unsigned)(B * bands), (unsigned)(L.C / BNF_SC), (unsigned)nv.nets);
+  by_dtype(L.dtype, [&](auto* typed) {
+    typedef std::remove_pointer_t<decltype(typed)> T;
+    hipLaunchKernelGGL(bn_finalize_apply_pool_kernel<T>, grid, dim3(256), 0, stream, b.stats, L.fwd_rows, L.C, L.Cpad,
+                       (double)L.rows, b.gamma, b.beta, BN_EPS, BN_MOMENTUM, b.running_mean, b.running_var,
+                       bn_coef(b.coef, L.C, BN_MEAN), bn_coef(b.coef, L.C, BN_INVSTD), bn_coef(b.coef, L.C, BN_SCALE),
+                       bn_coef(b.coef, L.C, BN_SHIFT), (const T*)b.y, L.relu ? 1 : 0, (T*)b.a, (T*)b.pool_out, b.pool_idx, H,
+                       W, bands, band_rows, nv);
   });
   D3F_HIP(hipGetLastError());
   return 0;
@@ -681,6 +804,19 @@
 
 int bn_layer_forward(const BnLayer& L, const BnBufs& b, const BnSync* sync, hipStream_t stream, const NetSplit* ns) {
   long count = L.rows;
+  if (b.pool_out != nullptr) {
+    const int H = b.pool_H, W = b.pool_W;
+    D3F_CHECK(b.pool_idx != nullptr && L.apply && L.res == BN_RES_NONE && b.a != nullptr,
+              "bn_layer_forward: the pool outputs go with an applied layer without a residual (%s)", L.name.c_str());
+    D3F_CHECK(H > 0 && W > 0 && H % 2 == 0 && W % 2 == 0 && L.rows % ((long)H * W) == 0,
+              "bn_layer_forward: pool extents %dx%d for %ld rows (%s)", H, W, L.rows, L.name.c_str());
+    if (sync == nullptr && L.fwd_fused && L.rows > 0) return bn_finalize_apply_pool_launch(L, b, stream, ns);
+    BnBufs plain = b;
+    plain.pool_out = nullptr;
+    if (int rc = bn_layer_forward(L, plain, sync, stream, ns)) return rc;
+    return maxpool3x3s2_fwd_launch(L.dtype, b.a, b.pool_out, b.pool_idx, (int)(L.rows / ((long)H * W)), H, W, L.C, stream,
+                                   ns);
+  }
   if (sync != nullptr) {
     if (int rc = sync->fn(sync->ctx, b.stats, (int64_t)L.fwd_rows * L.Cpad * 2, (void*)stream))
       return set_error(rc, "BatchNorm statistics all-reduce failed in the forward pass (%s)", L.name.c_str());
diff --git a/denoising_diffusion_deep_fake_amd/csrc/c_api.hip b/denoising_diffusion_deep_fake_amd/csrc/c_api.hip
--- a/denoising_diffusion_deep_fake_amd/csrc/c_api.hip
+++ b/denoising_diffusion_deep_fake_amd/csrc/c_api.hip
@@ -544,9 +544,9 @@
   bn_plan_out(L, plan);
   return 0;
 }
-int d3f_bn_layer_forward(const d3f_bn_desc* d, float* stats, const float* gamma, const float* beta, float* running_mean,
-                         float* running_var, float* coef, const void* y, const void* res, const float* res_coef, void* a,
-                         void* stream) {
+static int bn_forward_with(const d3f_bn_desc* d, float* stats, const float* gamma, const float* beta, float* running_mean,
+                           float* running_var, float* coef, const void* y, const void* res, const float* res_coef, void* a,
+                           void* pool_out, uint8_t* pool_idx, int H, int W, void* stream) {
   BnLayer L;
   if (int rc = bn_plan(L, d)) return rc;
   if (L.rows == 0) return 0;
@@ -566,7 +566,21 @@
   BnBufs b;
   b.stats = stats; b.gamma = gamma; b.beta = beta; b.running_mean = running_mean; b.running_var = running_var;
   b.coef = coef; b.y = y; b.a = a; b.res = res; b.res_coef = res_coef;
+  b.pool_out = pool_out; b.pool_idx = pool_idx; b.pool_H = H; b.pool_W = W;
   return bn_layer_forward(L, b, nullptr, (hipStream_t)stream);
+}
+int d3f_bn_layer_forward(const d3f_bn_desc* d, float* stats, const float* gamma, const float* beta, float* running_mean,
+                         float* running_var, float* coef, const void* y, const void* res, const float* res_coef, void* a,
+                         void* stream) {
+  return bn_forward_with(d, stats, gamma, beta, running_mean, running_var, coef, y, res, res_coef, a, nullptr, nullptr, 0, 0,
+                         stream);
+}
+int d3f_bn_layer_forward_pool(const d3f_bn_desc* d, float* stats, const float* gamma, const float* beta,
+                              float* running_mean, float* running_var, float* coef, const void* y, void* a, void* pool_out,
+                              uint8_t* pool_idx, int H, int W, void* stream) {
+  D3F_CHECK(pool_out && pool_idx, "bn_layer_forward_pool: null argument");
+  return bn_forward_with(d, stats, gamma, beta, running_mean, running_var, coef, y, nullptr, nullptr, a, pool_out, pool_idx,
+                         H, W, stream);
 }
 int d3f_bn_layer_backward(const d3f_bn_desc* d, float* partial, const float* gamma, float* coef, const void* y,
                           const void* a, const void* dA, void* dy, void* dres, int dres_acc, float* dgamma, float* dbeta,
diff --git a/denoising_diffusion_deep_fake_amd/csrc/engine.h b/denoising_diffusion_deep_fake_amd/csrc/engine.h
--- a/denoising_diffusion_deep_fake_amd/csrc/engine.h
+++ b/denoising_diffusion_deep_fake_amd/csrc/engine.h
@@ -134,8 +134,8 @@
   mutable hipEvent_t ev_seg_ = nullptr;
   mutable bool side_dirty_ = false;
   int ensure_streams() const;
-  mutable hipEvent_t ev_pack_in_ = nullptr, ev_pack_done_ = nullptr, ev_pack_mid_ = nullptr;
-  mutable bool pack_pending_ = false, pack_mid_pending_ = false;
+  mutable hipEvent_t ev_pack_in_ = nullptr, ev_pack_done_ = nullptr, ev_pack_mid_ = nullptr, ev_pack_first_ = nullptr;
+  mutable bool pack_pending_ = false, pack_mid_pending_ = false, pack_first_pending_ = false;
   int first_mid_unit_ = -1;
   int first_late_unit_ = -1;
   int forward_body(const float* params, float* bnstats, float* out, char* ws, int training, hipStream_t s,
diff --git a/denoising_diffusion_deep_fake_amd/csrc/engine.hip b/denoising_diffusion_deep_fake_amd/csrc/engine.hip
--- a/denoising_diffusion_deep_fake_amd/csrc/engine.hip
+++ b/denoising_diffusion_deep_fake_amd/csrc/engine.hip
@@ -429,6 +429,7 @@
   D3F_HIP(hipEventCreateWithFlags(&ev_pack_in_, hipEventDisableTiming));
   D3F_HIP(hipEventCreateWithFlags(&ev_pack_done_, hipEventDisableTiming));
   D3F_HIP(hipEventCreateWithFlags(&ev_pack_mid_, hipEventDisableTiming));
+  D3F_HIP(hipEventCreateWithFlags(&ev_pack_first_, hipEventDisableTiming));
   return 0;
 }
 
@@ -468,9 +469,9 @@
       blocks += (uint32_t)nb;
     }
     hipStream_t ps = s;
-    if (part >= 1 && async) {
+    if ((part >= 1 || mid > 0) && async) {
       if (int rc = ensure_streams()) return rc;
-      if (part == 1 || mid <= 0) {
+      if (part == 0 || (part == 2 && mid <= 0)) {
         D3F_HIP(hipEventRecord(ev_pack_in_, s));
         D3F_HIP(hipStreamWaitEvent(side_, ev_pack_in_, 0));
       }
@@ -488,6 +489,10 @@
         if (int rc = conv_winograd_pack_launch(params_ + u.w_off, reinterpret_cast<float*>(ws + u.wu_off), u.Cout, u.Cin, ps))
           return rc;
       }
+    }
+    if (part == 0 && ps != s) {
+      D3F_HIP(hipEventRecord(ev_pack_first_, side_));
+      pack_first_pending_ = true;
     }
     if (part == 1 && async) {
       D3F_HIP(hipEventRecord(ev_pack_mid_, side_));
@@ -545,8 +550,12 @@
       }
     if (int rc = bn_eval_coeff_all_launch(params_, bnstats, ws, t, s)) return rc;
   }
-  for (int ui : fwd_order_) {
+  static const bool no_stem_pool = getenv("D3F_NO_FUSED_STEM_POOL") != nullptr;
+  bool pool_done = false;
+  for (size_t fi = 0; fi < fwd_order_.size(); ++fi) {
+    const int ui = fwd_order_[fi];
     if (ui < 0) {
+      if (pool_done) continue;
       const TensorD& f1 = tensors[units[conv1].a];
       if (int rc = maxpool3x3s2_fwd_launch(dtype, T(units[conv1].a), T(t_pool),
                                            reinterpret_cast<uint8_t*>(ws + pool_idx_off), B, f1.H, f1.W,
@@ -555,6 +564,10 @@
       continue;
     }
     const Unit& u = units[ui];
+    if (pack_first_pending_) {
+      D3F_HIP(hipStreamWaitEvent(s, ev_pack_first_, 0));
+      pack_first_pending_ = false;
+    }
     if (pack_mid_pending_ && ui >= first_mid_unit_) {
       D3F_HIP(hipStreamWaitEvent(s, ev_pack_mid_, 0));
       pack_mid_pending_ = false;
@@ -587,6 +600,13 @@
       n.y = T(u.y); n.a = u.a >= 0 ? T(u.a) : nullptr;
       n.res = u.res_tensor >= 0 ? T(u.res_tensor) : (ds ? T(ds->y) : nullptr);
       n.res_coef = ds ? coef(*ds) : nullptr;
+      if (ui == conv1 && !no_stem_pool && fi + 1 < fwd_order_.size() && fwd_order_[fi + 1] < 0) {
+        const TensorD& f1 = tensors[u.a];
+        n.pool_out = T(t_pool);
+        n.pool_idx = reinterpret_cast<uint8_t*>(ws + pool_idx_off);
+        n.pool_H = f1.H; n.pool_W = f1.W;
+        pool_done = true;
+      }
       if (int rc = bn_layer_forward(u.norm, n, bn_sync(), s, ns)) return rc;
     } else {
       b.scale = bn_coef(coef(u), u.Cout, BN_SCALE);
@@ -700,7 +720,7 @@
     D3F_HIP(hipStreamBeginCapture(gstream_, hipStreamCaptureModeThreadLocal));
     const int rc = train_step_launches(a, ws_, gstream_);
     const hipError_t e = hipStreamEndCapture(gstream_, &graph);
-    pack_pending_ = pack_mid_pending_ = false;
+    pack_pending_ = pack_mid_pending_ = pack_first_pending_ = false;
     side_dirty_ = false;
     if (rc != 0) {
       if (graph) (void)hipGraphDestroy(graph);
@@ -718,6 +738,10 @@
 }
 
 int UnetEngine::wait_for_packed_weights(hipStream_t s) const {
+  if (pack_first_pending_) {
+    D3F_HIP(hipStreamWaitEvent(s, ev_pack_first_, 0));
+    pack_first_pending_ = false;
+  }
   if (pack_mid_pending_) {
     D3F_HIP(hipStreamWaitEvent(s, ev_pack_mid_, 0));
     pack_mid_pending_ = false;
@@ -781,6 +805,7 @@
   if (ev_pack_in_) (void)hipEventDestroy(ev_pack_in_);
   if (ev_pack_done_) (void)hipEventDestroy(ev_pack_done_);
   if (ev_pack_mid_) (void)hipEventDestroy(ev_pack_mid_);
+  if (ev_pack_first_) (void)hipEventDestroy(ev_pack_first_);
 }
 
 static bool serial_backward() {
@@ -829,6 +854,17 @@
   std::vector<int> pending;
   int pending_segment = -1;
   bool head_bias_pending = false;
+  auto wgrad_on = [&](int ui, hipStream_t st) -> int {
+    const Unit& u = units[ui];
+    WgradReduceBatch red;
+    if (int rc = wgrad_layer_launch_deferred(u.wl, ws + u.dy_off, T(u.in0), u.in1 >= 0 ? T(u.in1) : nullptr,
+                                             reinterpret_cast<float*>(ws + u.wslab_off), grads + u.w_off, u.Cout,
+                                             u.CinReal, cdtype, red, st, ns))
+      return rc;
+    if (!skip_r)
+      if (int rc = wgrad_reduce_batch_launch(red, st)) return rc;
+    return 0;
+  };
   auto flush_pending = [&]() -> int {
     if (pending.empty()) return 0;
     if (!serial) {
@@ -849,16 +885,8 @@
         return rc;
       head_bias_pending = false;
     }
-    for (int ui : pending) {
-      const Unit& u = units[ui];
-      WgradReduceBatch red;
-      if (int rc = wgrad_layer_launch_deferred(u.wl, ws + u.dy_off, T(u.in0), u.in1 >= 0 ? T(u.in1) : nullptr,
-                                               reinterpret_cast<float*>(ws + u.wslab_off), grads + u.w_off, u.Cout,
-                                               u.CinReal, cdtype, red, ws_stream, ns))
-        return rc;
-      if (!skip_r)
-        if (int rc = wgrad_reduce_batch_launch(red, ws_stream)) return rc;
-    }
+    for (int ui : pending)
+      if (int rc = wgrad_on(ui, ws_stream)) return rc;
     pending.clear();
     return 0;
   };
@@ -901,7 +929,10 @@
       n.dgamma = grads + u.g_off; n.dbeta = grads + u.b_off;
       if (int rc = bn_layer_backward(u.norm, n, bn_sync(), s, ns)) return rc;
     }
-    if (!skip_w) {
+    if (!skip_w && op.unit == conv1 && !u.need_dgrad) {
+      if (int rc = flush_pending()) return rc;
+      if (int rc = wgrad_on(op.unit, s)) return rc;
+    } else if (!skip_w) {
       pending.push_back(op.unit);
       if ((int)pending.size() >= defer)
         if (int rc = flush_pending()) return rc;
diff --git a/denoising_diffusion_deep_fake_amd/csrc/loss.hip b/denoising_diffusion_deep_fake_amd/csrc/loss.hip
--- a/denoising_diffusion_deep_fake_amd/csrc/loss.hip
+++ b/denoising_diffusion_deep_fake_amd/csrc/loss.hip
@@ -29,6 +29,32 @@
   return fminf(fmaxf(t, 0.f), 1.f);
 }
 
+typedef float ss2 __attribute__((ext_vector_type(2)));
+
+constexpr int SS_RG = 6;
+constexpr int SS_RBMAX = 6;
+__device__ __forceinline__ int ss_group_row0(int g) { return g * 5 + (g < 2 ? g : 2); }
+__device__ __forceinline__ int ss_group_rows(int g) { return g < 2 ? 6 : 5; }
+
+__device__ __forceinline__ void ss_load4(const float* __restrict__ row, int x, int n, float (&v)[4]) {
+  if (x >= 0 && x + 3 < n && (reinterpret_cast<uintptr_t>(row + x) & 15) == 0) {
+    const float4 t = *reinterpret_cast<const float4*>(row + x);
+    v[0] = t.x; v[1] = t.y; v[2] = t.z; v[3] = t.w;
+  } else {
+#pragma unroll
+    for (int e = 0; e < 4; ++e) v[e] = (x + e >= 0 && x + e < n) ? row[x + e] : 0.f;
+  }
+}
+__device__ __forceinline__ void ss_store4(float* __restrict__ out, const float (&v)[4], int valid) {
+  if (valid == 4 && (reinterpret_cast<uintptr_t>(out) & 15) == 0) {
+    *reinterpret_cast<float4*>(out) = make_float4(v[0], v[1], v[2], v[3]);
+  } else {
+#pragma unroll
+    for (int e = 0; e < 4; ++e)
+      if (e < valid) out[e] = v[e];
+  }
+}
+
 __global__ __launch_bounds__(256) void ssim_fwd_kernel(const float* __restrict__ pred,
                                                        const float* __restrict__ target, float lo,
                                                        float range, GaussK gk, int H, int W,
@@ -36,8 +62,10 @@
                                                        float* __restrict__ dC,
                                                        float* __restrict__ partial) {
   chain_priority();
-  __shared__ float tx[SS_IN * SS_LD], ty[SS_IN * SS_LD];
-  __shared__ float vv[5][SS_T * SS_LD];
+  __shared__ ss2 txy[SS_IN * SS_LD];
+  __shared__ ss2 v01[SS_T * SS_LD];
+  __shared__ ss2 v23[SS_T * SS_LD];
+  __shared__ float v4[SS_T * SS_LD];
   __shared__ float wsum[4];
   const int Hv = H - (SS_K - 1), Wv = W - (SS_K - 1);
   const int plane = blockIdx.z;
@@ -45,47 +73,56 @@
   const float* __restrict__ px = pred + (long)plane * H * W;
   const float* __restrict__ py = target + (long)plane * H * W;
   const int tid = threadIdx.x;
-  for (int e = tid; e < SS_IN * SS_IN; e += 256) {
-    const int r = e / SS_IN, c = e - r * SS_IN;
-    const int iy = oy0 + r, ix = ox0 + c;
-    float a = 0.f, b = 0.f;
-    if (iy < H && ix < W) {
-      a = norm01(px[(long)iy * W + ix], lo, range);
-      b = norm01(py[(long)iy * W + ix], lo, range);
-    }
-    tx[r * SS_LD + c] = a;
-    ty[r * SS_LD + c] = b;
-  }
-  __syncthreads();
-  constexpr int RB = 8;
-  if (tid < SS_IN * (SS_T / RB)) {
-    const int c = tid % SS_IN, r0 = (tid / SS_IN) * RB;
-    float a[RB + SS_K - 1], b[RB + SS_K - 1], aa[RB + SS_K - 1], bb[RB + SS_K - 1], ab[RB + SS_K - 1];
-#pragma unroll
-    for (int i = 0; i < RB + SS_K - 1; ++i) {
-      a[i] = tx[(r0 + i) * SS_LD + c];
-      b[i] = ty[(r0 + i) * SS_LD + c];
-      aa[i] = a[i] * a[i];
-      bb[i] = b[i] * b[i];
-      ab[i] = a[i] * b[i];
-    }
-#pragma unroll
-    for (int r = 0; r < RB; ++r) {
-      float s0 = 0.f, s1 = 0.f, s2 = 0.f, s3 = 0.f, s4 = 0.f;
+  constexpr int PCS = (SS_IN + 3) / 4;
+  for (int t = tid; t < SS_IN * PCS; t += 256) {
+    const int r = t / PCS, k = t - r * PCS;
+    const int iy = oy0 + r, ix = ox0 + 4 * k;
+    float a[4] = {0.f, 0.f, 0.f, 0.f}, b[4] = {0.f, 0.f, 0.f, 0.f};
+    if (iy < H) {
+      ss_load4(px + (long)iy * W, ix, W, a);
+      ss_load4(py + (long)iy * W, ix, W, b);
+    }
+#pragma unroll
+    for (int e = 0; e < 4; ++e) {
+      const int c = 4 * k + e;
+      if (c >= SS_IN) continue;
+      ss2 v = {0.f, 0.f};
+      if (iy < H && ix + e < W) {
+        v.x = norm01(a[e], lo, range);
+        v.y = norm01(b[e], lo, range);
+      }
+      txy[r * SS_LD + c] = v;
+    }
+  }
+  __syncthreads();
+  if (tid < SS_IN * SS_RG) {
+    const int c = tid % SS_IN, grp = tid / SS_IN;
+    const int r0 = ss_group_row0(grp), nr = ss_group_rows(grp);
+    ss2 ab[SS_RBMAX + SS_K - 1], sq[SS_RBMAX + SS_K - 1];
+    float xy[SS_RBMAX + SS_K - 1];
+#pragma unroll
+    for (int i = 0; i < SS_RBMAX + SS_K - 1; ++i) {
+      const int row = r0 + i < SS_IN ? r0 + i : SS_IN - 1;
+      ab[i] = txy[row * SS_LD + c];
+      sq[i] = ab[i] * ab[i];
+      xy[i] = ab[i].x * ab[i].y;
+    }
+#pragma unroll
+    for (int r = 0; r < SS_RBMAX; ++r) {
+      if (r >= nr) continue;
+      ss2 s01 = {0.f, 0.f}, s23 = {0.f, 0.f};
+      float s4 = 0.f;
 #pragma unroll
       for (int i = 0; i < SS_K; ++i) {
         const float g = gk.g[i];
-        s0 += g * a[r + i];
-        s1 += g * b[r + i];
-        s2 += g * aa[r + i];
-        s3 += g * bb[r + i];
-        s4 += g * ab[r + i];
+        const ss2 gg = {g, g};
+        s01 += gg * ab[r + i];
+        s23 += gg * sq[r + i];
+        s4 += g * xy[r + i];
       }
-      vv[0][(r0 + r) * SS_LD + c] = s0;
-      vv[1][(r0 + r) * SS_LD + c] = s1;
-      vv[2][(r0 + r) * SS_LD + c] = s2;
-      vv[3][(r0 + r) * SS_LD + c] = s3;
-      vv[4][(r0 + r) * SS_LD + c] = s4;
+      v01[(r0 + r) * SS_LD + c] = s01;
+      v23[(r0 + r) * SS_LD + c] = s23;
+      v4[(r0 + r) * SS_LD + c] = s4;
     }
   }
   __syncthreads();
@@ -93,37 +130,51 @@
   float local = 0.f;
   constexpr int CBk = 4;
   const int rr = tid / (SS_T / CBk), cq = (tid % (SS_T / CBk)) * CBk;
-  float win[5][CBk + SS_K - 1];
-#pragma unroll
-  for (int q = 0; q < 5; ++q)
-#pragma unroll
-    for (int j = 0; j < CBk + SS_K - 1; ++j) win[q][j] = vv[q][rr * SS_LD + cq + j];
+  ss2 w01[CBk + SS_K - 1], w23[CBk + SS_K - 1];
+  float w4[CBk + SS_K - 1];
+#pragma unroll
+  for (int j = 0; j < CBk + SS_K - 1; ++j) {
+    w01[j] = v01[rr * SS_LD + cq + j];
+    w23[j] = v23[rr * SS_LD + cq + j];
+    w4[j] = v4[rr * SS_LD + cq + j];
+  }
+  const int oy = oy0 + rr;
+  float oa[CBk], ob[CBk], oc[CBk];
+  int valid = 0;
 #pragma unroll
   for (int cc = 0; cc < CBk; ++cc) {
-    const int r = rr, c = cq + cc;
-    const int oy = oy0 + r, ox = ox0 + c;
+    const int ox = ox0 + cq + cc;
+    oa[cc] = ob[cc] = oc[cc] = 0.f;
     if (oy >= Hv || ox >= Wv) continue;
-    float m[5];
-#pragma unroll
-    for (int q = 0; q < 5; ++q) {
-      float s = 0.f;
-#pragma unroll
-      for (int j = 0; j < SS_K; ++j) s += gk.g[j] * win[q][cc + j];
-      m[q] = s;
-    }
-    const float mux = m[0], muy = m[1];
-    const float sxx = m[2] - mux * mux, syy = m[3] - muy * muy, sxy = m[4] - mux * muy;
+    ss2 m01 = {0.f, 0.f}, m23 = {0.f, 0.f};
+    float m4 = 0.f;
+#pragma unroll
+    for (int j = 0; j < SS_K; ++j) {
+      const float g = gk.g[j];
+      const ss2 gg = {g, g};
+      m01 += gg * w01[cc + j];
+      m23 += gg * w23[cc + j];
+      m4 += g * w4[cc + j];
+    }
+    const float mux = m01.x, muy = m01.y;
+    const float sxx = m23.x - mux * mux, syy = m23.y - muy * muy, sxy = m4 - mux * muy;
     const float a1 = 2.f * mux * muy + c1, b1 = mux * mux + muy * muy + c1;
     const float a2 = 2.f * sxy + c2, b2 = sxx + syy + c2;
     const float l = a1 / b1, cs = a2 / b2;
     const float ss = l * cs;
     local += ss;
-    const long o = ((long)plane * Hv + oy) * Wv + ox;
     const float dl_dmux = 2.f * (muy - l * mux) / b1;
     const float dcs_dmux = (2.f * mux * cs - 2.f * muy) / b2;
-    dA[o] = cs * dl_dmux + l * dcs_dmux;
-    dB[o] = -l * cs / b2;
-    dC[o] = 2.f * l / b2;
+    oa[cc] = cs * dl_dmux + l * dcs_dmux;
+    ob[cc] = -l * cs / b2;
+    oc[cc] = 2.f * l / b2;
+    valid = cc + 1;
+  }
+  if (valid > 0) {
+    const long o = ((long)plane * Hv + oy) * Wv + ox0 + cq;
+    ss_store4(dA + o, oa, valid);
+    ss_store4(dB + o, ob, valid);
+    ss_store4(dC + o, oc, valid);
   }
 #pragma unroll
   for (int o = 32; o > 0; o >>= 1) local += __shfl_xor(local, o);
@@ -140,51 +191,61 @@
     const float* __restrict__ dC, float ssim_coef, float mse_coef, float* __restrict__ grad,
     float* __restrict__ partial_mse) {
   chain_priority();
-  __shared__ float t3[3][SS_IN * SS_LD];
-  __shared__ float vv[3][SS_T * SS_LD];
+  __shared__ ss2 t01[SS_IN * SS_LD];
+  __shared__ float t2[SS_IN * SS_LD];
+  __shared__ ss2 v01[SS_T * SS_LD];
+  __shared__ float v2[SS_T * SS_LD];
   __shared__ float wsum[4];
   const int Hv = H - (SS_K - 1), Wv = W - (SS_K - 1);
   const int plane = blockIdx.z;
   const int py0 = blockIdx.y * SS_T, px0 = blockIdx.x * SS_T;
   const int tid = threadIdx.x;
-  for (int e = tid; e < SS_IN * SS_IN; e += 256) {
-    const int r = e / SS_IN, c = e - r * SS_IN;
-    const int oy = py0 - (SS_K - 1) + r, ox = px0 - (SS_K - 1) + c;
-    float a = 0.f, b = 0.f, d = 0.f;
-    if (oy >= 0 && oy < Hv && ox >= 0 && ox < Wv) {
-      const long o = ((long)plane * Hv + oy) * Wv + ox;
-      a = dA[o];
-      b = dB[o];
-      d = dC[o];
-    }
-    t3[0][r * SS_LD + c] = a;
-    t3[1][r * SS_LD + c] = b;
-    t3[2][r * SS_LD + c] = d;
-  }
-  __syncthreads();
-  constexpr int RB = 8;
-  if (tid < SS_IN * (SS_T / RB)) {
-    const int c = tid % SS_IN, r0 = (tid / SS_IN) * RB;
-    float v0[RB + SS_K - 1], v1[RB + SS_K - 1], v2[RB + SS_K - 1];
-#pragma unroll
-    for (int i = 0; i < RB + SS_K - 1; ++i) {
-      v0[i] = t3[0][(r0 + i) * SS_LD + c];
-      v1[i] = t3[1][(r0 + i) * SS_LD + c];
-      v2[i] = t3[2][(r0 + i) * SS_LD + c];
-    }
-#pragma unroll
-    for (int r = 0; r < RB; ++r) {
-      float s0 = 0.f, s1 = 0.f, s2 = 0.f;
+  constexpr int PCS = 12;
+  for (int t = tid; t < SS_IN * PCS; t += 256) {
+    const int r = t / PCS, k = t - r * PCS;
+    const int oy = py0 - (SS_K - 1) + r, ox = px0 - 12 + 4 * k;
+    float a[4] = {0.f, 0.f, 0.f, 0.f}, b[4] = {0.f, 0.f, 0.f, 0.f}, d[4] = {0.f, 0.f, 0.f, 0.f};
+    if (oy >= 0 && oy < Hv) {
+      const long o = ((long)plane * Hv + oy) * Wv;
+      ss_load4(dA + o, ox, Wv, a);
+      ss_load4(dB + o, ox, Wv, b);
+      ss_load4(dC + o, ox, Wv, d);
+    }
+#pragma unroll
+    for (int e = 0; e < 4; ++e) {
+      const int c = 4 * k + e - 2;
+      if (c < 0 || c >= SS_IN) continue;
+      const ss2 v = {a[e], b[e]};
+      t01[r * SS_LD + c] = v;
+      t2[r * SS_LD + c] = d[e];
+    }
+  }
+  __syncthreads();
+  if (tid < SS_IN * SS_RG) {
+    const int c = tid % SS_IN, grp = tid / SS_IN;
+    const int r0 = ss_group_row0(grp), nr = ss_group_rows(grp);
+    ss2 u01[SS_RBMAX + SS_K - 1];
+    float u2[SS_RBMAX + SS_K - 1];
+#pragma unroll
+    for (int i = 0; i < SS_RBMAX + SS_K - 1; ++i) {
+      const int row = r0 + i < SS_IN ? r0 + i : SS_IN - 1;
+      u01[i] = t01[row * SS_LD + c];
+      u2[i] = t2[row * SS_LD + c];
+    }
+#pragma unroll
+    for (int r = 0; r < SS_RBMAX; ++r) {
+      if (r >= nr) continue;
+      ss2 s01 = {0.f, 0.f};
+      float s2 = 0.f;
 #pragma unroll
       for (int i = 0; i < SS_K; ++i) {
         const float g = gk.g[SS_K - 1 - i];
-        s0 += g * v0[r + i];
-        s1 += g * v1[r + i];
-        s2 += g * v2[r + i];
+        const ss2 gg = {g, g};
+        s01 += gg * u01[r + i];
+        s2 += g * u2[r + i];
       }
-      vv[0][(r0 + r) * SS_LD + c] = s0;
-      vv[1][(r0 + r) * SS_LD + c] = s1;
-      vv[2][(r0 + r) * SS_LD + c] = s2;
+      v01[(r0 + r) * SS_LD + c] = s01;
+      v2[(r0 + r) * SS_LD + c] = s2;
     }
   }
   __syncthreads();
@@ -192,34 +253,45 @@
   float local = 0.f;
   constexpr int CBk = 4;
   const int rr = tid / (SS_T / CBk), cq = (tid % (SS_T / CBk)) * CBk;
-  float win[3][CBk + SS_K - 1];
-#pragma unroll
-  for (int q = 0; q < 3; ++q)
-#pragma unroll
-    for (int j = 0; j < CBk + SS_K - 1; ++j) win[q][j] = vv[q][rr * SS_LD + cq + j];
-#pragma unroll
-  for (int cc = 0; cc < CBk; ++cc) {
-    const int r = rr, c = cq + cc;
-    const int iy = py0 + r, ix = px0 + c;
-    if (iy >= H || ix >= W) continue;
-    float ga = 0.f, gb = 0.f, gc = 0.f;
-#pragma unroll
-    for (int j = 0; j < SS_K; ++j) {
-      const float g = gk.g[SS_K - 1 - j];
-      ga += g * win[0][cc + j];
-      gb += g * win[1][cc + j];
-      gc += g * win[2][cc + j];
-    }
-    const long p = (long)plane * H * W + (long)iy * W + ix;
-    const float pv = pred[p], tv = target[p];
-    const float rawx = (pv - lo) / range;
-    const float xh = fminf(fmaxf(rawx, 0.f), 1.f);
-    const float yh = norm01(tv, lo, range);
-    float gx = ga + 2.f * xh * gb + yh * gc;
-    gx = (rawx >= 0.f && rawx <= 1.f) ? gx * inv_range : 0.f;
-    const float diff = pv - tv;
-    local += diff * diff;
-    grad[p] = ssim_coef * gx + mse_coef * diff;
+  ss2 w01[CBk + SS_K - 1];
+  float w2[CBk + SS_K - 1];
+#pragma unroll
+  for (int j = 0; j < CBk + SS_K - 1; ++j) {
+    w01[j] = v01[rr * SS_LD + cq + j];
+    w2[j] = v2[rr * SS_LD + cq + j];
+  }
+  const int iy = py0 + rr, ix0 = px0 + cq;
+  if (iy < H && ix0 < W) {
+    const long p0 = (long)plane * H * W + (long)iy * W;
+    float pv4[4], tv4[4], go[4] = {0.f, 0.f, 0.f, 0.f};
+    ss_load4(pred + p0, ix0, W, pv4);
+    ss_load4(target + p0, ix0, W, tv4);
+    int valid = 0;
+#pragma unroll
+    for (int cc = 0; cc < CBk; ++cc) {
+      if (ix0 + cc >= W) continue;
+      ss2 gab = {0.f, 0.f};
+      float gc = 0.f;
+#pragma unroll
+      for (int j = 0; j < SS_K; ++j) {
+        const float g = gk.g[SS_K - 1 - j];
+        const ss2 gg = {g, g};
+        gab += gg * w01[cc + j];
+        gc += g * w2[cc + j];
+      }
+      const float ga = gab.x, gb = gab.y;
+      const float pv = pv4[cc], tv = tv4[cc];
+      const float rawx = (pv - lo) / range;
+      const float xh = fminf(fmaxf(rawx, 0.f), 1.f);
+      const float yh = norm01(tv, lo, range);
+      float gx = ga + 2.f * xh * gb + yh * gc;
+      gx = (rawx >= 0.f && rawx <= 1.f) ? gx * inv_range : 0.f;
+      const float diff = pv - tv;
+      local += diff * diff;
+      go[cc] = ssim_coef * gx + mse_coef * diff;
+      valid = cc + 1;
+    }
+    ss_store4(grad + p0 + ix0, go, valid);
   }
 #pragma unroll
   for (int o = 32; o > 0; o >>= 1) local += __shfl_xor(local, o);
diff --git a/denoising_diffusion_deep_fake_amd/csrc/pointwise.h b/denoising_diffusion_deep_fake_amd/csrc/pointwise.h
--- a/denoising_diffusion_deep_fake_amd/csrc/pointwise.h
+++ b/denoising_diffusion_deep_fake_amd/csrc/pointwise.h
@@ -60,6 +60,9 @@
   void* dres = nullptr;
   int dres_acc = 0;
   float *dgamma = nullptr, *dbeta = nullptr;
+  void* pool_out = nullptr;
+  uint8_t* pool_idx = nullptr;
+  int pool_H = 0, pool_W = 0;
 };
 struct BnSync {
   int (*fn)(void* ctx, float* data, int64_t count, void* stream);
diff --git a/denoising_diffusion_deep_fake_amd/ops.py b/denoising_diffusion_deep_fake_amd/ops.py
--- a/denoising_diffusion_deep_fake_amd/ops.py
+++ b/denoising_diffusion_deep_fake_amd/ops.py
@@ -183,6 +183,13 @@
                                           stream_ptr()))
 
 
+def bn_layer_forward_pool(d, stats, gamma, beta, coef, y, a, pool_out, pool_idx, H, W, running_mean=None,
+                          running_var=None):
+    check(_lib.lib().d3f_bn_layer_forward_pool(C.byref(d), ptr(stats), ptr(gamma), ptr(beta), ptr(running_mean),
+                                               ptr(running_var), ptr(coef), ptr(y), ptr(a), ptr(pool_out),
+                                               ptr(pool_idx), H, W, stream_ptr()))
+
+
 def bn_layer_backward(d, partial, gamma, coef, y, dA, dy, a=None, dres=None, dres_acc=False, dgamma=None, dbeta=None):
     check(_lib.lib().d3f_bn_layer_backward(C.byref(d), ptr(partial), ptr(gamma), ptr(coef), ptr(y), ptr(a), ptr(dA),
                                            ptr(dy), ptr(dres), int(dres_acc), ptr(dgamma), ptr(dbeta), stream_ptr()))
diff --git a/include/d3f_hip.h b/include/d3f_hip.h
--- a/include/d3f_hip.h
+++ b/include/d3f_hip.h
@@ -147,6 +147,9 @@
 int d3f_bn_layer_forward(const d3f_bn_desc* d, float* stats, const float* gamma, const float* beta, float* running_mean,
                          float* running_var, float* coef, const void* y, const void* res, const float* res_coef, void* a,
                          void* stream);
+int d3f_bn_layer_forward_pool(const d3f_bn_desc* d, float* stats, const float* gamma, const float* beta,
+                              float* running_mean, float* running_var, float* coef, const void* y, void* a, void* pool_out,
+                              uint8_t* pool_idx, int H, int W, void* stream);
 int d3f_bn_layer_backward(const d3f_bn_desc* d, float* partial, const float* gamma, float* coef, const void* y,
                           const void* a, const void* dA, void* dy, void* dres, int dres_acc, float* dgamma, float* dbeta,
                           void* stream);
```

After: 2054 images/sec (median of 6 runs). About the same (+0.6%).
